# fverdoja/Fast-3D-Pointcloud-Segmentation

Hardware: AMD Instinct MI355X
Metric: Mpoints/sec segmented end-to-end, 1M-pt RGB-D frames (higher is better)
Workload: dtype f32

## Files before the change

### fast-3d-pointcloud-segmentation_amd/csrc/f3ds_hip.hip

```cpp
#include <hip/hip_runtime.h>

#include <algorithm>
#include <cmath>
#include <atomic>
#include <map>
#include <chrono>
#include <cstdio>
#include <cstdlib>
#include <cstring>
#include <string>
#include <type_traits>
#include <mutex>
#include <set>
#include <vector>

#include "../../include/f3ds.h"
#include "f3ds_algo.h"
#include "f3ds_glasbey.h"
#include "f3ds_eval.h"
#include "f3ds_dev.h"
#include "f3ds_levels.h"
#include "f3ds_eval_levels.h"
#include "f3ds_rgbd.h"
#include "f3ds_label_image.h"
#include "f3ds_track.h"
#include "f3ds_regions.h"
#include "f3ds_contacts.h"
#include "f3ds_shapes.h"
#include "f3ds_boxes.h"
#include "f3ds_joints.h"
#include "f3ds_components.h"

using namespace f3ds;

#include "f3ds_kernels.inc"
#include "f3ds_levels.inc"
#include "f3ds_eval_levels.inc"
#include "f3ds_track.inc"
#include "f3ds_regions.inc"
#include "f3ds_contacts.inc"
#include "f3ds_shapes.inc"
#include "f3ds_boxes.inc"
#include "f3ds_joints.inc"
#include "f3ds_components.inc"

namespace {

thread_local std::string g_last_hip_error;
#define HIPCHECK(expr) do { hipError_t e_ = (expr); if (e_ != hipSuccess) { g_last_hip_error = std::string(#expr) + ": " + hipGetErrorString(e_); return F3DS_ERR_HIP; } } while (0)

template <class... Ts> struct ArgPack;
template <> struct ArgPack<> {};
template <class T, class... Ts> struct ArgPack<T, Ts...> { T head; ArgPack<Ts...> tail; };

template <class K, class... Done>
__device__ __forceinline__ void unpack_call(const ArgPack<>&, Done... d) { K{}(d...); }
template <class K, class T, class... Ts, class... Done>
__device__ __forceinline__ void unpack_call(const ArgPack<T, Ts...>& p, Done... d) { unpack_call<K>(p.tail, d..., p.head); }

template <class K, class = void> struct waves_per_simd { static constexpr int v = 1; };
template <class K> struct waves_per_simd<K, std::void_t<decltype(K::WAVES_PER_SIMD)>> { static constexpr int v = K::WAVES_PER_SIMD; };
template <class K, class = void> struct is_latency_kernel { static constexpr bool v = false; };
template <class K> struct is_latency_kernel<K, std::void_t<decltype(K::LATENCY_KERNEL)>> { static constexpr bool v = K::LATENCY_KERNEL; };
template <class K, class Pack>
__global__ __launch_bounds__(K::BLOCK, waves_per_simd<K>::v) void k_batched(const Pack* frames) {
#ifndef F3DS_EXP_NO_LATENCY_PRIO
    if constexpr (is_latency_kernel<K>::v) __builtin_amdgcn_s_setprio(3);
#endif
    const Pack p = frames[f3ds_frame()];
    unpack_call<K>(p);
}

template <class F> struct op_traits;
template <class C, class... Ps> struct op_traits<void (C::*)(Ps...) const> { using pack = ArgPack<std::decay_t<Ps>...>; };
template <class K> using pack_of = typename op_traits<decltype(&K::operator())>::pack;

inline void fill_pack(ArgPack<>&) {}
template <class T, class... Ts, class A, class... As>
inline void fill_pack(ArgPack<T, Ts...>& p, A a, As... as) {
    static_assert(std::is_convertible<A, T>::value && !(std::is_pointer<T>::value && std::is_integral<A>::value),
                  "rec<K>(): an argument does not convert implicitly to the kernel's parameter type (wrong element type, swapped arguments?)");
    p.head = a; fill_pack(p.tail, as...);
}

typedef hipError_t (*LaunchFn)(uint32_t gx, uint32_t nf, uint32_t lds, hipStream_t st, const void* dargs);
template <class K>
hipError_t launch_fn(uint32_t gx, uint32_t nf, uint32_t lds, hipStream_t st, const void* dargs) {
    using Pack = pack_of<K>;
    if (lds > 48u * 1024u) {
        hipError_t e = hipFuncSetAttribute(reinterpret_cast<const void*>(k_batched<K, Pack>), hipFuncAttributeMaxDynamicSharedMemorySize, (int)lds);
        if (e != hipSuccess) return e;
    }
    hipLaunchKernelGGL((k_batched<K, Pack>), dim3(gx ? gx : 1u, nf), dim3(K::BLOCK), lds, st, static_cast<const Pack*>(dargs));
    return hipGetLastError();
}
struct Cmd { LaunchFn fn; uint32_t gx, lds, bytes, off; };

const int g_inc_shift = [] { const char* e = dev_getenv("F3DS_INC_SHIFT"); return e ? atoi(e) : 6; }();

struct Switches {
    bool direct_labels = false, copy_stream = true, copy_duplex = false, split_voxel_accum = false, sweep_tiles = true, merge_spec = true, force_global_merge = false, no_stream_pool = false, sort_pairs = false, host_prof = false, trace_err = false, vox_hash = true, vox_tiles_forced = false, levels_global = false;
    int normals_threads = 0, merge_nw = 0, merge_keys = -1; uint32_t tile_holes = 0, ilist_slack = 32, r_rounds = F3DS_R_ROUNDS, grid_cap = 0, rgc_first_cap = 0, rgj_first_cap = 0; long relabel_lds_cap = -1;
    void read() {
        auto on = [](const char* n) { return dev_getenv(n) != nullptr; };
        auto num = [](const char* n, long dflt) { const char* e = dev_getenv(n); return e ? atol(e) : dflt; };
        direct_labels = num("F3DS_DIRECT_LABELS", 0) != 0; copy_stream = num("F3DS_COPY_STREAM", 1) != 0; copy_duplex = num("F3DS_COPY_STREAM", 1) == 2; split_voxel_accum = on("F3DS_SPLIT_VOXEL_ACCUM"); sweep_tiles = num("F3DS_SWEEP_TILES", 1) != 0; merge_spec = num("F3DS_MERGE_SPEC", 1) != 0;
        force_global_merge = on("F3DS_FORCE_GLOBAL_MERGE"); no_stream_pool = on("F3DS_NO_STREAM_POOL"); sort_pairs = on("F3DS_SORT_PAIRS");
        host_prof = on("F3DS_HOST_PROF"); trace_err = on("F3DS_TRACE_ERR");
        vox_tiles_forced = num("F3DS_VOX_TILES", 1) == 2;
        vox_hash = num("F3DS_VOX_TILES", 1) != 0 && !sort_pairs && !split_voxel_accum;
        normals_threads = (int)num("F3DS_NORMALS_THREADS", 0); tile_holes = (uint32_t)num("F3DS_SWEEP_TILE_HOLES", 0);
        { const long v = num("F3DS_MERGE_NW", 0); merge_nw = v == 4 ? 4 : (v ? 8 : 0); }
        { const char* e = dev_getenv("F3DS_MERGE_KEYS"); merge_keys = !e ? -1 : (!strcmp(e, "lds") ? 2 : (!strcmp(e, "global") ? 1 : 0)); }
        relabel_lds_cap = num("F3DS_RELABEL_LDS_CAP", -1);
        levels_global = num("F3DS_LEVELS_GLOBAL", 0) != 0;
        { const long v = num("F3DS_R_ROUNDS_RUN", F3DS_R_ROUNDS); r_rounds = v >= 1 && v <= F3DS_R_ROUNDS ? (uint32_t)v : (uint32_t)F3DS_R_ROUNDS; }
        { const long v = num("F3DS_ILIST_SLACK", 32); ilist_slack = v >= 1 && v <= 32 ? (uint32_t)v : 32u; }
        { const long v = num("F3DS_GRID_CAP", 0); grid_cap = v >= 1 && v <= 2048 ? (uint32_t)v : 0u; }
        { const long v = num("F3DS_RGC_FIRST_CAP", 0); rgc_first_cap = v >= 1 && v <= 0x7fffffffl ? (uint32_t)v : 0u; }
        { const long v = num("F3DS_RGJ_FIRST_CAP", 0); rgj_first_cap = v >= 1 && v <= 0x7fffffffl ? (uint32_t)v : 0u; }
    }
};
thread_local Switches g_sw;
const int g_merge_shared_res = [] { const char* e = dev_getenv("F3DS_MERGE_SHARED_RES"); return e && atoi(e) == 2 ? 2 : 0; }();

#define F3DS_SCRATCH(X) \
    X(P16, pts)  X(unsigned char, img_depth) X(unsigned char, img_color) X(P16, spts) X(uint64_t, keys0) X(uint64_t, keys1) X(uint32_t, vals0) X(uint32_t, vals1) X(uint32_t, flags) X(uint32_t, incl) X(uint32_t, tiles) X(uint32_t, hist) X(uint32_t, seg_start) X(int, pt_voxel) X(uint32_t, labels) \
    X(uint32_t, vkey) X(uint32_t, vcount) X(float, vf) X(int, nbr) X(int, nbrT) X(uint64_t, hkeys) X(uint32_t, hvals) X(float, boxes) X(uint32_t, ckey) X(uint32_t, cell_start) X(uint64_t, chk) X(uint32_t, chv) X(uint32_t, chvals) X(int, seed_orig) X(uint32_t, keep) X(int, seed_kept) \
    X(uint32_t, owner0) X(uint32_t, ownR) X(float, dist0) X(unsigned char, R) X(float, hc) X(uint32_t, hcount) X(uint32_t, hlo) X(uint32_t, hhi) X(int, ghost_vox) X(unsigned char, ghost_active) X(unsigned char, ghost_done) X(uint32_t, ghost_head) X(uint32_t, ghost_next) \
    X(uint32_t, loff) X(float, rows) X(int, row_voxel) X(float, racc0) X(uint32_t, rcnt0) X(float, rrec0) X(unsigned char, ralive0) X(uint64_t, ehk) X(uint64_t, ekeys0) X(uint64_t, ekeys1) X(uint32_t, evals0) X(uint32_t, evals1) X(uint32_t, ea0) X(uint32_t, eb0) \
    X(uint32_t, ea) X(uint32_t, eb) X(float, ew) X(uint32_t, eku) X(int, ehist) X(unsigned char, ealive) X(uint32_t, ev_epoch) X(uint32_t, ev_key) X(int, ev_prev) X(float, racc) X(uint32_t, rcnt) X(float, rrec) X(unsigned char, ralive) X(uint32_t, rhead) X(uint32_t, rtail) X(uint32_t, lnext) X(uint32_t, parent) X(uint32_t, markA) X(uint32_t, markB) X(uint32_t, tl) X(uint32_t, merges) \
     X(float, r_vf) X(uint32_t, r_owner) X(float, r_dist) X(float, r_hc) X(uint32_t, r_hcount) X(uint32_t, r_hlo) X(uint32_t, r_hhi) X(int, r_gvox) X(unsigned char, r_gact) X(unsigned char, r_gdone) X(uint32_t, r_ghead) X(uint32_t, r_gnext) X(uint32_t, r_tl) X(uint32_t, r_tcnt) X(int, r_seed) X(uint32_t, r_L) \
    X(uint32_t, tstamp) X(uint32_t, tround) X(uint32_t, hdirty) X(uint32_t, htiles) X(uint32_t, htcnt) X(uint32_t, vwl) X(uint32_t, vwl2) X(uint32_t, vtmask) \
     X(uint32_t, glut) X(uint32_t, truth_pts) X(uint32_t, tsum) X(uint32_t, tcol) X(uint32_t, tlab) X(uint32_t, ctab) X(uint32_t, csize) X(uint32_t, eroot) X(uint32_t, eincl) \
     X(uint32_t, hcnt) X(uint32_t, pslot) X(uint32_t, vlist) \
     X(uint32_t, u_src) X(uint32_t, u_voff) X(float, u_xyz) X(uint32_t, u_rgba) X(float, u_cent) X(float, u_nrm) \
    X(float, deltas) X(uint64_t, skeys0) X(uint64_t, skeys1) X(uint32_t, svals0) X(uint32_t, svals1) X(uint32_t, cdf_hist) X(float, cdf) X(uint32_t, root) X(uint32_t, rincl) X(uint32_t, rrank) X(uint2, pool) X(uint32_t, rstart) X(uint32_t, rnleaf) X(uint32_t, rcap) X(uint32_t, tile_n1) X(uint32_t, tile_ord) X(uint32_t, tile_slots) X(uint32_t, ilist) X(uint32_t, istart) X(uint32_t, ilen) X(uint32_t, icap) \
     X(uint32_t, lv_into) X(uint32_t, lv_at) X(uint32_t, lv_pfx) X(float, lv_thr) X(uint32_t, lv_tab) X(uint32_t, lv_nreg) X(uint32_t, lv_out) \
     \
    X(uint64_t, evl_k0) X(uint64_t, evl_k1) X(uint32_t, evl_v0) X(uint32_t, evl_v1) X(uint32_t, evl_flag) X(uint64_t, evl_bkey) X(uint32_t, evl_bcnt) X(uint64_t, evl_ukey) X(uint32_t, evl_ucnt) X(uint32_t, evl_glist) \
    X(uint32_t, evl_ssize) X(unsigned char, evl_used) X(float, evl_hterm) X(float, evl_mterm) X(float, evl_tterm) X(uint32_t, evl_tsize) X(uint32_t, evl_order) X(uint32_t, evl_slot) X(uint32_t, evl_counts) X(uint32_t, evl_out) \
     \
    X(unsigned char, li_depth) X(unsigned char, li_color) X(uint32_t, li_lab) X(unsigned char, li_out) \
     \
     \
    X(uint32_t, trk_end) X(uint32_t, trk_out) X(uint32_t, trk_id) X(uint32_t, trk_tid) \
     \
    X(RgAcc, rgt_acc) \
     \
    X(uint64_t, rgc_k0) X(uint64_t, rgc_k1) X(uint32_t, rgc_v0) X(uint32_t, rgc_v1) X(uint32_t, rgc_rec) X(uint32_t, rgc_flag) X(uint64_t, rgc_ukey) X(uint32_t, rgc_ustart) X(uint32_t, rgc_uend) X(uint32_t, rgc_cnt) \
     \
    X(ShAcc, rgs_acc) \
     \
    X(BxFrame, rgx_frame) X(BxAcc, rgx_acc) X(uint32_t, rgx_head) X(f3ds_region_shape, rgx_shape) \
     \
    X(ShAcc, rgj_sacc) X(uint32_t, rgj_shead) X(f3ds_region_shape, rgj_shape) X(uint64_t, rgj_k0) X(uint64_t, rgj_k1) X(uint32_t, rgj_v0) X(uint32_t, rgj_v1) X(uint32_t, rgj_rec) X(uint32_t, rgj_flag) X(uint64_t, rgj_ukey) X(uint32_t, rgj_ustart) X(uint32_t, rgj_uend) X(uint32_t, rgj_cnt) \
     \
    X(uint32_t, rgk_parent) X(uint32_t, rgk_cnt) X(uint32_t, rgk_flag)
template <class T> struct Scratch { T* p = nullptr; size_t cap = 0; int slot = -1; };
#define F3DS_SCRATCH_SLOT(T, name) S_##name,
#define F3DS_SCRATCH_MEMBER(T, name) Scratch<T> name{nullptr, 0, S_##name};
#define F3DS_SCRATCH_VISIT(T, name) if (const int rc_ = f(name)) return rc_;
enum ScratchSlot { F3DS_SCRATCH(F3DS_SCRATCH_SLOT) N_SCRATCH };

}

struct f3ds_ctx {
    int device = 0;
    hipStream_t own_stream = nullptr;
    hipStream_t stream = nullptr;
    hipEvent_t ev[11] = {};
    DevCounters* d_dc = nullptr;
    DevCounters* h_dc = nullptr;
    GridInfo* d_grid = nullptr;
    GridInfo* h_grid = nullptr;
    SeedGrid* d_sgrid = nullptr;
    std::vector<Cmd> cmds;
    std::vector<unsigned char> blob;
    std::vector<uintptr_t> pend;
    MultiOp ops = {}; uint32_t ops_grid = 0;
    unsigned char* h_args[2] = {nullptr, nullptr}; unsigned char* d_args[2] = {nullptr, nullptr}; size_t args_cap = 0;
    hipEvent_t ev_args[2] = {nullptr, nullptr}; bool args_used[2] = {false, false}; int args_flip = 0;
    hipEvent_t ev_copy[3] = {nullptr, nullptr, nullptr};
    DevCounters* d_dcblk = nullptr; DevCounters* h_dcblk = nullptr; size_t dcblk_cap = 0;
    unsigned char* h_li = nullptr; size_t h_li_cap = 0;
    bool have_frame = false;
    bool live = false;
    int rc = 0;
    f3ds_params prm;
    FrameArgs fa;
    const P16* d_pts = nullptr;
    uint32_t n = 0, V = 0, C = 0, S0 = 0, E = 0, hmask = 0;
    uint64_t *ks = nullptr; uint32_t *vs = nullptr;
    uint64_t *cks = nullptr; uint32_t *cvs = nullptr;
    uint64_t *eks = nullptr;
    f3ds_result res;
    bool merge_in_lds = false;
    int merge_kind = 0;
    uint32_t ev_mult = 64;
    uint32_t pool_mult = 1;
    uint32_t vox_cap = 0;
    bool vox_hashed = false;
    bool vox_dense = false;
    uint32_t vox_dense_wait = 0, vox_dense_penalty = 8;
    uint32_t ilist_mult = 1;
    uint32_t edge_mult = 32;
    bool relabel_lds = true;
    int refined_itr = -1;
    int idxbits = -1;
    uint32_t* user_labels = nullptr;
    MergeDev mdev; MergeLds mlds; float host_lambda = 0.5f;
    F3DS_SCRATCH(F3DS_SCRATCH_MEMBER)
    template <class F> int each_scratch(F&& f) { F3DS_SCRATCH(F3DS_SCRATCH_VISIT) return 0; }
    uint32_t launch_shape[3] = {0, 0, 0};
    std::vector<uint32_t> tsize;
    float cluster_T = 0.0f;
    bool user_mode = false;
    std::vector<uint32_t> user_label, user_row;
};

namespace {

bool referenced_by_pending_calls(const f3ds_ctx* c, const void* mem, size_t cap) {
    const uintptr_t lo = (uintptr_t)mem, hi = lo + cap;
    for (const uintptr_t w : c->pend) if (w >= lo && w < hi) return true;
    for (uint32_t k = 0; k < c->ops.n; ++k) {
        const uintptr_t d = (uintptr_t)c->ops.dst[k], sp = (uintptr_t)c->ops.src[k];
        if ((d >= lo && d < hi) || (sp >= lo && sp < hi)) return true;
    }
    return false;
}
template <class A> inline void note_arg(f3ds_ctx* c, const A& a) {
    if constexpr (std::is_pointer<A>::value) { if (a) c->pend.push_back((uintptr_t)a); }
    else if constexpr (std::is_class<A>::value) {
        static_assert(std::is_trivially_copyable<A>::value, "kernel arguments must be plain data");
        for (size_t off = 0; off + 8 <= sizeof(A); off += 8) { uintptr_t w; memcpy(&w, reinterpret_cast<const unsigned char*>(&a) + off, 8); if (w) c->pend.push_back(w); }
    }
}
std::atomic<size_t> g_scratch_hwm[16][N_SCRATCH];
std::atomic<unsigned long long> g_scratch_allocs{0};
template <class T>
int regrow(Scratch<T>& b, size_t mark) {
    g_scratch_allocs.fetch_add(1, std::memory_order_relaxed);
    if (b.p) { HIPCHECK(hipFree(b.p)); b.p = nullptr; b.cap = 0; }
    const size_t want = mark + mark / 4 + 64;
    HIPCHECK(hipMalloc(&b.p, want));
    b.cap = want;
    return F3DS_OK;
}
template <class T>
int ensure(f3ds_ctx* c, Scratch<T>& b, size_t count, T** out) {
    size_t bytes = count * sizeof(T);
    if (bytes < 256) bytes = 256;
    size_t target = bytes;
    std::atomic<size_t>& hwm = g_scratch_hwm[c->device & 15][b.slot];
    size_t seen = hwm.load(std::memory_order_relaxed);
    while (seen < bytes && !hwm.compare_exchange_weak(seen, bytes, std::memory_order_relaxed)) {}
    if (seen > target && seen <= 4 * bytes) target = seen;
    if (b.cap < bytes) {
        if (b.p && (!c->cmds.empty() || c->ops.n) && referenced_by_pending_calls(c, b.p, b.cap)) {
            fprintf(stderr, "f3ds: internal error: regrowing a buffer that a recorded kernel call refers to\n");
            return F3DS_ERR_LOGIC;
        }
        static const bool trace = dev_getenv("F3DS_TRACE_ALLOC") != nullptr;
        if (trace && b.p) fprintf(stderr, "f3ds: regrow slot %d: cap %zu, request %zu, mark %zu, pending calls %zu\n", b.slot, b.cap, bytes, target, c->cmds.size());
        if (const int rc = regrow(b, target)) return rc;
    }
    *out = b.p;
    return F3DS_OK;
}
int pregrow_scratch(f3ds_ctx* c) {
    return c->each_scratch([c](auto& b) -> int {
        if (!b.p) return F3DS_OK;
        const size_t mark = g_scratch_hwm[c->device & 15][b.slot].load(std::memory_order_relaxed);
        if (b.cap >= mark || mark > 4 * b.cap) return F3DS_OK;
        return regrow(b, mark);
    });
}
#define ENSURE(buf, count, ptr) do { int rc_ = ensure(c, buf, (size_t)(count), &ptr); if (rc_) return rc_; } while (0)

thread_local size_t g_grid_cap = 2048;
thread_local size_t g_wide_cap = 2048;
thread_local int g_batch_frames = 1;
std::atomic<int> g_batch_calls[16];
struct BatchCallCount { int d; explicit BatchCallCount(int dev) : d(dev & 15) { g_batch_calls[d].fetch_add(1, std::memory_order_relaxed); } ~BatchCallCount() { g_batch_calls[d].fetch_sub(1, std::memory_order_relaxed); } };
size_t grid_cap_for_batch(int frames) {
    static const size_t target = dev_getenv("F3DS_GRID_TARGET") ? (size_t)atol(dev_getenv("F3DS_GRID_TARGET")) : 3072;
    if (!target) return 2048;
    size_t cap = target / (size_t)(frames > 0 ? frames : 1);
    return cap < 8 ? 8 : (cap > 2048 ? 2048 : cap);
}
inline void set_launch_shape(f3ds_ctx* const* frames, int nframes) {
    g_grid_cap = g_sw.grid_cap ? (size_t)g_sw.grid_cap : grid_cap_for_batch(nframes);
    g_wide_cap = g_sw.grid_cap ? (size_t)g_sw.grid_cap : 2048;
    g_batch_frames = nframes;
    for (int i = 0; i < nframes; ++i) { frames[i]->launch_shape[0] = (uint32_t)g_grid_cap; frames[i]->launch_shape[1] = (uint32_t)g_wide_cap; frames[i]->launch_shape[2] = (uint32_t)nframes; }
}
inline uint32_t grid_wide(size_t work, int block) {
    size_t g = (work + block - 1) / block;
    return (uint32_t)(g < 1 ? 1 : (g > g_wide_cap ? g_wide_cap : g));
}
inline uint32_t grid_for(size_t work, int block) {
    size_t g = (work + block - 1) / block;
    if (g < 1) g = 1;
    if (g > g_grid_cap) g = g_grid_cap;
    return (uint32_t)g;
}
inline uint32_t pow2_ge(size_t x) { uint32_t p = 1; while (p < x) p <<= 1; return p; }
int bits_for(uint64_t max_value) { int b = 0; while (b < 64 && (max_value >> b)) ++b; return b; }

template <class K, class... As> void rec(f3ds_ctx* c, uint32_t gx, uint32_t lds, As... as);
inline void flush_ops(f3ds_ctx* c) {
    if (!c->ops.n) return;
    const MultiOp m = c->ops; const uint32_t g = c->ops_grid;
    c->ops.n = 0; c->ops_grid = 0;
    rec<d_multi_op>(c, g, 0u, m);
}
template <class K, class... As>
void rec(f3ds_ctx* c, uint32_t gx, uint32_t lds, As... as) {
    if constexpr (!std::is_same<K, d_multi_op>::value) flush_ops(c);
    using Pack = pack_of<K>;
    static_assert(std::is_trivially_copyable<Pack>::value, "kernel arguments must be plain data");
    Pack p;
    memset(&p, 0, sizeof p);
    fill_pack(p, as...);
    (note_arg(c, as), ...);
    Cmd cmd; cmd.fn = &launch_fn<K>; cmd.gx = gx; cmd.lds = lds; cmd.bytes = (uint32_t)sizeof(Pack); cmd.off = (uint32_t)c->blob.size();
    c->blob.resize(c->blob.size() + sizeof(Pack));
    memcpy(c->blob.data() + cmd.off, &p, sizeof(Pack));
    c->cmds.push_back(cmd);
}
inline void rec_op(f3ds_ctx* c, void* dst, const void* src, uint32_t value, size_t bytes) {
    const uint32_t words = (uint32_t)((bytes + 3) / 4);
    if (c->ops.n == (uint32_t)MULTI_OPS) flush_ops(c);
    MultiOp& m = c->ops;
    if (m.n == 0) memset(&m, 0, sizeof m);
    m.dst[m.n] = static_cast<uint32_t*>(dst); m.src[m.n] = static_cast<const uint32_t*>(src); m.val[m.n] = value; m.words[m.n] = words; m.n++;
    const uint32_t g = grid_for(words, 256);
    if (g > c->ops_grid) c->ops_grid = g;
}
inline void rec_fill(f3ds_ctx* c, void* dst, uint32_t value, size_t bytes) { rec_op(c, dst, nullptr, value, bytes); }
inline void rec_copy(f3ds_ctx* c, void* dst, const void* src, size_t bytes) { rec_op(c, dst, src, 0u, bytes); }
inline void reset_recording(f3ds_ctx* c) { c->cmds.clear(); c->blob.clear(); c->pend.clear(); c->ops.n = 0; c->ops_grid = 0; }

struct Batch {
    std::vector<f3ds_ctx*> fr;
    hipStream_t st = nullptr;
    f3ds_ctx* owner = nullptr;
};
inline Batch batch_of(f3ds_ctx* c) {
    Batch b; b.owner = c; b.st = c->stream;
    set_launch_shape(&c, 1); reset_recording(c);
    b.fr.push_back(c);
    return b;
}
int batch_of(f3ds_ctx** ctxs, int nctx, Batch& b) {
    b.owner = ctxs[0]; b.st = ctxs[0]->stream;
    set_launch_shape(ctxs, nctx);
    for (int i = 0; i < nctx; ++i) {
        if (ctxs[i]->stream != b.st) HIPCHECK(hipStreamSynchronize(ctxs[i]->stream));
        reset_recording(ctxs[i]);
        b.fr.push_back(ctxs[i]);
    }
    return F3DS_OK;
}

thread_local double g_t_wait = 0, g_t_launch = 0;
static int trace_err(int code, const char* where, const f3ds_ctx* c) {
    if (code && g_sw.trace_err)
        fprintf(stderr, "f3ds: error %d after %s (V %u, seeds %u, edges %u, chain overflow %d, capacity flag %d)\n", code, where, c->V, c->S0, c->h_dc->n_edges,
                c->h_dc->r_overflow, c->h_dc->ev_overflow);
    return code;
}
static inline double now_ms() { return std::chrono::duration<double, std::milli>(std::chrono::steady_clock::now().time_since_epoch()).count(); }
inline hipError_t timed_sync(hipEvent_t e) { const double t0 = now_ms(); const hipError_t r = hipEventSynchronize(e); g_t_wait += now_ms() - t0; return r; }
inline hipError_t timed_sync(hipStream_t st) { const double t0 = now_ms(); const hipError_t r = hipStreamSynchronize(st); g_t_wait += now_ms() - t0; return r; }
template <class F> int clear_counter(f3ds_ctx* c, hipStream_t st, F DevCounters::*f) { c->h_dc->*f = 0; HIPCHECK(hipMemsetAsync(&(c->d_dc->*f), 0, sizeof(F), st)); return F3DS_OK; }
template <class... Fs> int clear_counters(f3ds_ctx* c, hipStream_t st, Fs DevCounters::*... f) { int rc = F3DS_OK; (void)((rc = clear_counter(c, st, f)) || ...); return rc; }
int flush(Batch& b, hipEvent_t before_launch = nullptr) {
    if (b.fr.empty()) return F3DS_OK;
    for (f3ds_ctx* c : b.fr) flush_ops(c);
    const size_t ncmd = b.fr[0]->cmds.size();
    for (f3ds_ctx* c : b.fr) if (c->cmds.size() != ncmd) return F3DS_ERR_UNSUPPORTED;
    if (ncmd == 0) return F3DS_OK;
    const uint32_t nf = (uint32_t)b.fr.size();
    size_t total = 0;
    std::vector<size_t> off(ncmd);
    for (size_t j = 0; j < ncmd; ++j) { off[j] = total; total += (((size_t)b.fr[0]->cmds[j].bytes * nf) + 63u) & ~(size_t)63u; }
    f3ds_ctx* o = b.owner;
    if (o->args_cap < total) {
        HIPCHECK(hipStreamSynchronize(b.st));
        for (int k = 0; k < 2; ++k) {
            if (o->h_args[k]) HIPCHECK(hipHostFree(o->h_args[k]));
            if (o->d_args[k]) HIPCHECK(hipFree(o->d_args[k]));
            o->h_args[k] = o->d_args[k] = nullptr; o->args_used[k] = false;
        }
        o->args_cap = total * 2;
        for (int k = 0; k < 2; ++k) {
            HIPCHECK(hipHostMalloc(&o->h_args[k], o->args_cap, hipHostMallocDefault));
            HIPCHECK(hipMalloc(&o->d_args[k], o->args_cap));
            if (!o->ev_args[k]) HIPCHECK(hipEventCreateWithFlags(&o->ev_args[k], hipEventDisableTiming));
        }
    }
    const int fl = o->args_flip; o->args_flip ^= 1;
    if (o->args_used[fl]) HIPCHECK(timed_sync(o->ev_args[fl]));
    unsigned char* const h_args = o->h_args[fl]; unsigned char* const d_args = o->d_args[fl];
    const double tl0 = now_ms();
    for (size_t j = 0; j < ncmd; ++j)
        for (uint32_t i = 0; i < nf; ++i) {
            const Cmd& cm = b.fr[i]->cmds[j];
            if (cm.fn != b.fr[0]->cmds[j].fn) return F3DS_ERR_UNSUPPORTED;
            memcpy(h_args + off[j] + (size_t)i * cm.bytes, b.fr[i]->blob.data() + cm.off, cm.bytes);
        }
    HIPCHECK(hipMemcpyAsync(d_args, h_args, total, hipMemcpyHostToDevice, b.st));
    if (before_launch) HIPCHECK(hipEventRecord(before_launch, b.st));
    for (size_t j = 0; j < ncmd; ++j) {
        uint32_t gx = 1, lds = 0;
        for (uint32_t i = 0; i < nf; ++i) { const Cmd& cm = b.fr[i]->cmds[j]; if (cm.gx > gx) gx = cm.gx; if (cm.lds > lds) lds = cm.lds; }
        HIPCHECK(b.fr[0]->cmds[j].fn(gx, nf, lds, b.st, d_args + off[j]));
    }
    HIPCHECK(hipEventRecord(o->ev_args[fl], b.st)); o->args_used[fl] = true;
    for (f3ds_ctx* c : b.fr) reset_recording(c);
    g_t_launch += now_ms() - tl0;
    return F3DS_OK;
}
int flush_sync(Batch& b) {
    int rc = flush(b);
    if (rc) return rc;
    const size_t nf = b.fr.size();
    if (nf == 1) HIPCHECK(hipMemcpyAsync(b.fr[0]->h_dc, b.fr[0]->d_dc, sizeof(DevCounters), hipMemcpyDeviceToHost, b.st));
    else if (nf > 1) {
        f3ds_ctx* o = b.owner;
        if (o->dcblk_cap < nf) {
            HIPCHECK(hipStreamSynchronize(b.st));
            if (o->d_dcblk) HIPCHECK(hipFree(o->d_dcblk));
            if (o->h_dcblk) HIPCHECK(hipHostFree(o->h_dcblk));
            o->dcblk_cap = nf * 2;
            HIPCHECK(hipMalloc(&o->d_dcblk, o->dcblk_cap * sizeof(DevCounters)));
            HIPCHECK(hipHostMalloc(&o->h_dcblk, o->dcblk_cap * sizeof(DevCounters), hipHostMallocDefault));
        }
        for (size_t i = 0; i < nf; ++i) rec<d_dc_gather>(b.fr[i], 1u, 0u, b.fr[i]->d_dc, o->d_dcblk + i);
        if ((rc = flush(b))) return rc;
        HIPCHECK(hipMemcpyAsync(o->h_dcblk, o->d_dcblk, nf * sizeof(DevCounters), hipMemcpyDeviceToHost, b.st));
    }
    HIPCHECK(timed_sync(b.st));
    HIPCHECK(hipGetLastError());
    if (nf > 1) for (size_t i = 0; i < nf; ++i) *b.fr[i]->h_dc = b.owner->h_dcblk[i];
    return F3DS_OK;
}

int scan_u32(f3ds_ctx* c, const uint32_t* in, uint32_t* out, uint32_t n) {
    const uint32_t nt = n ? (n + SCAN_TILE - 1) / SCAN_TILE : 1u;
    uint32_t* tiles;
    ENSURE(c->tiles, nt, tiles);
    rec<d_scan_tiles>(c, nt, 0u, in, out, tiles, n);
    rec<d_scan_single>(c, 1u, 0u, tiles, nt);
    rec<d_scan_add>(c, nt, 0u, out, tiles, n);
    return F3DS_OK;
}
int radix_sort(f3ds_ctx* c, uint64_t* k0, uint32_t* v0, uint64_t* k1, uint32_t* v1, uint32_t n, int total_bits, uint64_t** keys_out, uint32_t** vals_out, int base_shift = 0, const uint32_t* n_dev = nullptr) {
    *keys_out = k0; if (vals_out) *vals_out = v0;
    if (total_bits <= 0) return F3DS_OK;
    const int passes = (total_bits + RS_MAXBITS - 1) / RS_MAXBITS;
    const int per = (total_bits + passes - 1) / passes;
    const uint32_t nb = n ? (n + RS_TILE - 1) / RS_TILE : 1u;
    uint32_t* hist;
    ENSURE(c->hist, (size_t)RS_BINS * nb, hist);
    int shift = 0;
    for (int p = 0; p < passes; ++p) {
        const int bits = (total_bits - shift) < per ? (total_bits - shift) : per;
        rec<d_radix_hist>(c, nb, 0u, k0, n, base_shift + shift, bits, hist, nb, n_dev);
        rec<d_scan_single>(c, 1u, 0u, hist, (uint32_t)((1u << bits) * nb));
        if (v0) rec<d_radix_scatter>(c, nb, 0u, k0, v0, k1, v1, n, base_shift + shift, bits, hist, nb, n_dev);
        else rec<d_radix_scatter_k>(c, nb, 0u, k0, k1, n, base_shift + shift, bits, hist, nb);
        std::swap(k0, k1); std::swap(v0, v1);
        shift += bits;
    }
    *keys_out = k0; if (vals_out) *vals_out = v0;
    return F3DS_OK;
}

int seg_bbox(f3ds_ctx* c) {
    rec<d_init_counters>(c, 1u, 0u, c->d_dc);
    rec<d_bbox>(c, grid_for(c->n, 256 * 8) < 512 ? grid_for(c->n, 256 * 8) : 512u, 0u, c->d_pts, c->n, c->fa, c->d_dc);
    rec<d_grid>(c, 1u, 0u, c->d_dc, c->prm.voxel_res, c->d_grid);
    return F3DS_OK;
}
int seg_sort(f3ds_ctx* c, int sort_bits, int idxbits) {
    const uint32_t n = c->n;
    uint64_t *k0, *k1; uint32_t *v0 = nullptr, *v1 = nullptr, *flags, *incl, *seg_start; int* pt_voxel;
    ENSURE(c->keys0, n, k0); ENSURE(c->keys1, n, k1);
    if (idxbits < 0) { ENSURE(c->vals0, n, v0); ENSURE(c->vals1, n, v1); }
    ENSURE(c->flags, n, flags); ENSURE(c->incl, n, incl); ENSURE(c->seg_start, (size_t)n + 1, seg_start);
    ENSURE(c->pt_voxel, n, pt_voxel);
    c->idxbits = idxbits;
    const int ks = idxbits < 0 ? 0 : idxbits;
    rec<d_keys>(c, grid_for(n, 256), 0u, c->d_pts, n, c->fa, c->d_grid, k0, v0, ks);
    c->vs = nullptr;
    int rc = radix_sort(c, k0, v0, k1, v1, n, sort_bits, &c->ks, &c->vs, ks);
    if (rc) return rc;
    const uint64_t invalid = 1ull << (3 * c->h_dc->depth);
    if (g_sw.split_voxel_accum) {
        rec<d_heads>(c, grid_for(n, 256), 0u, c->ks, n, invalid, flags, ks);
        if ((rc = scan_u32(c, flags, incl, n))) return rc;
        rec<d_segstart>(c, grid_for(n, 256), 0u, c->ks, flags, incl, n, invalid, seg_start, &c->d_dc->n_voxels, &c->d_dc->n_valid, ks);
        return F3DS_OK;
    }
    const uint32_t nt = n ? (n + SCAN_TILE - 1) / SCAN_TILE : 1u;
    uint32_t* tiles; ENSURE(c->tiles, nt, tiles);
    rec<d_seg_count>(c, nt, 0u, c->ks, n, invalid, ks, tiles);
    rec<d_scan_single>(c, 1u, 0u, tiles, nt);
    rec<d_seg_write>(c, nt, 0u, c->ks, n, invalid, ks, tiles, seg_start, &c->d_dc->n_voxels, &c->d_dc->n_valid);
    return F3DS_OK;
}
int seg_vox_tiles(f3ds_ctx* c, int code_bits, int tile_bits) {
    const uint32_t n = c->n;
    const uint32_t ntiles = (n + VT_TILE - 1u) / VT_TILE;
    const uint64_t dcap64 = (uint64_t)ntiles * VT_ENT_MAX;
    if (code_bits + tile_bits + VT_CNT_BITS > 64 || dcap64 > 0x7fffffffull || (uint64_t)ntiles * VT_TAB > 0x7fffffffull) return F3DS_ERR_UNSUPPORTED;
    const uint32_t dcap = (uint32_t)dcap64;
    const uint64_t fin = c->h_dc->n_finite;
    const uint32_t capV = (uint32_t)std::max<uint64_t>(256u, std::min<uint64_t>(fin, dcap));
    c->vox_cap = capV;
    uint64_t *k0, *k1; uint32_t *ploc, *v0, *v1, *part, *vkey, *vcount, *seg_start, *list; uint2* bo_te; float* vf; int* pt_voxel;
    const uint32_t nchunks = (dcap + DS_CHUNK - 1u) / DS_CHUNK;
    ENSURE(c->pslot, n, ploc); ENSURE(c->keys0, dcap, k0); ENSURE(c->keys1, dcap, k1); ENSURE(c->vals0, dcap, v0); ENSURE(c->vals1, dcap, v1);
    { uint32_t* w; ENSURE(c->hcnt, (size_t)ntiles * VT_TAB * 2 + 2u * nchunks, w); bo_te = reinterpret_cast<uint2*>(w); part = w + (size_t)ntiles * VT_TAB * 2; }
    ENSURE(c->vkey, (size_t)capV * 3, vkey); ENSURE(c->vcount, capV, vcount); ENSURE(c->vf, (size_t)capV * 12, vf);
    ENSURE(c->seg_start, (size_t)capV + 1, seg_start); ENSURE(c->vlist, n, list); ENSURE(c->pt_voxel, n, pt_voxel);
    { uint32_t *f, *incl; ENSURE(c->flags, capV, f); ENSURE(c->incl, capV, incl); }
    c->idxbits = -1; c->ks = nullptr; c->vs = nullptr;
    rec<d_tile_keys>(c, std::min<uint32_t>(ntiles, (uint32_t)g_grid_cap * 16u), 0u, c->d_pts, n, c->fa, c->d_grid, ploc, k0, v0, dcap, tile_bits, c->d_dc);
    uint64_t* ks; uint32_t* vs;
    int rc = radix_sort(c, k0, v0, k1, v1, dcap, code_bits + tile_bits, &ks, &vs, VT_CNT_BITS, &c->d_dc->seg_count);
    if (rc) return rc;
    rec<d_desc_part>(c, nchunks, 0u, ks, dcap, tile_bits, part, c->d_dc);
    rec<d_desc_offsets>(c, 1u, 0u, part, dcap, capV, seg_start, c->d_dc);
    rec<d_desc_apply>(c, nchunks, 0u, ks, vs, dcap, capV, tile_bits, c->fa, c->d_grid, part, bo_te, seg_start, vkey, c->d_dc);
    rec<d_tile_place>(c, std::min<uint32_t>(ntiles, (uint32_t)g_grid_cap * 16u), 0u, ploc, n, bo_te, list, pt_voxel, c->d_dc);
    rec<d_voxel_list_accum>(c, std::min<uint32_t>(grid_wide(capV, 256), std::max<uint32_t>(64u, grid_wide(n / 8u, 256))), 0u, c->d_pts, list, seg_start, c->fa, vf, vcount, c->d_dc, capV);
    c->vox_hashed = true;
    return F3DS_OK;
}
int seg_neighbors(f3ds_ctx* c, uint32_t wgs) {
    const uint32_t V = c->V;
    const bool blocks = c->h_dc->depth <= N_BLOCK_DEPTH_MAX;
    const uint32_t cap = blocks ? pow2_ge((size_t)V + 16) : pow2_ge((size_t)V * 2 + 16);
    const size_t words = blocks ? (size_t)cap * 2 : cap;
    uint32_t* hvals = nullptr; int *nbr, *nbrT; uint64_t* hkeys;
    c->hmask = cap - 1;
    ENSURE(c->nbr, (size_t)V * 27, nbr); ENSURE(c->nbrT, (size_t)V * 27, nbrT); ENSURE(c->hkeys, words, hkeys);
    if (!blocks) ENSURE(c->hvals, cap, hvals);
    rec_fill(c, hkeys, 0xFFFFFFFFu, words * 8);
    rec<d_vox_table>(c, wgs, 0u, c->vkey.p, V, c->d_grid, hkeys, hvals, c->hmask);
    rec<d_neighbors>(c, grid_wide((size_t)V * 27, 256), 0u, c->vkey.p, c->d_dc, c->d_grid, c->fa.leaf_order, hkeys, hvals, c->hmask, nbr, nbrT);
    return F3DS_OK;
}
int seg_voxels(f3ds_ctx* c) {
    const uint32_t V = c->V, n = c->n;
    if (c->vox_hashed) return seg_neighbors(c, 1u);
    uint32_t *vkey, *vcount; float *vf;
    ENSURE(c->vkey, (size_t)V * 3, vkey); ENSURE(c->vcount, V, vcount); ENSURE(c->vf, (size_t)V * 12, vf);
    if (g_sw.split_voxel_accum) {
        P16* spts; ENSURE(c->spts, n, spts);
        rec<d_point_gather>(c, grid_wide(n, 256), 0u, c->d_pts, c->vs, c->ks, c->idxbits < 0 ? 0 : c->idxbits, c->incl.p, n, c->d_dc, spts, c->pt_voxel.p);
        rec<d_voxel_accum>(c, grid_wide(V, 256), 0u, spts, c->ks, c->idxbits < 0 ? 0 : c->idxbits, c->seg_start.p, c->d_dc, c->fa, c->d_grid, vkey, vcount, vf);
    } else
        rec<d_voxel_gather_accum>(c, grid_wide(V, 256), 0u, c->d_pts, c->vs, c->ks, c->idxbits < 0 ? 0 : c->idxbits, c->seg_start.p, n, c->d_dc, c->fa, c->d_grid, vkey, vcount, vf, c->pt_voxel.p);
    return seg_neighbors(c, grid_for(V, 4096));
}
int seg_normals(f3ds_ctx* c) {
    const uint32_t nt = (c->V + NT_TILE - 1) / NT_TILE;
    uint32_t *tn1, *tord, *tslots;
    ENSURE(c->tile_n1, nt, tn1); ENSURE(c->tile_ord, (size_t)nt * NT_RING1, tord); ENSURE(c->tile_slots, (size_t)nt * SW_SLOT_WORDS * NT_TILE, tslots);
#ifdef F3DS_NORMALS_LOOP
    static const uint32_t budget = dev_getenv("F3DS_NORMALS_WGS") ? (uint32_t)atoi(dev_getenv("F3DS_NORMALS_WGS")) : 0u;
#else
    static const uint32_t budget = 0u;
#endif
    const uint32_t share = budget ? std::max(2u, budget / (uint32_t)g_batch_frames) : nt;
    const int nthr_env = g_sw.normals_threads;
    const uint32_t holes = g_sw.tile_holes;
    if (nthr_env ? nthr_env == 256 : g_batch_frames >= 16)
        rec<d_normals_t<256>>(c, std::min(nt, share), 0u, c->vf.p, c->nbr.p, c->d_dc, tn1, tord, tslots, holes);
    else
        rec<d_normals_t<384>>(c, std::min(nt, share), 0u, c->vf.p, c->nbr.p, c->d_dc, tn1, tord, tslots, holes);
    return F3DS_OK;
}
int seg_seed_grid(f3ds_ctx* c) {
    const uint32_t V = c->V;
    float* boxes; const float* vf = c->vf.p;
    const uint32_t nchunks = (V + SEED_CHUNK - 1) / SEED_CHUNK;
    ENSURE(c->boxes, (size_t)nchunks * 6, boxes);
    rec<d_chunkbox>(c, nchunks, 0u, vf, c->d_dc, boxes);
    rec<d_seed_grow>(c, 1u, 0u, vf, boxes, c->d_dc, c->prm.seed_res, c->d_sgrid);
    return F3DS_OK;
}
int seg_seed_cells(f3ds_ctx* c, int sort_bits, int max_sdepth) {
    const uint32_t V = c->V;
    uint32_t *ckey, *cell_start, *v0, *v1; uint64_t *k0 = c->keys0.p, *k1 = c->keys1.p;
    ENSURE(c->vals0, V, v0); ENSURE(c->vals1, V, v1);
    ENSURE(c->ckey, (size_t)V * 3, ckey); ENSURE(c->cell_start, (size_t)V + 1, cell_start);
    rec<d_seed_keys>(c, grid_for(V, 256), 0u, c->vf.p, c->d_dc, c->d_sgrid, ckey, k0, v0);
    int rc = radix_sort(c, k0, v0, k1, v1, V, sort_bits, &c->cks, &c->cvs);
    if (rc) return rc;
    const uint64_t climit = max_sdepth >= 21 ? 0xFFFFFFFFFFFFFFFFull : (1ull << (3 * max_sdepth));
    rec<d_heads>(c, grid_for(V, 256), 0u, c->cks, V, climit, c->flags.p, 0);
    if ((rc = scan_u32(c, c->flags.p, c->incl.p, V))) return rc;
    rec<d_segstart>(c, grid_for(V, 256), 0u, c->cks, c->flags.p, c->incl.p, V, climit, cell_start, &c->d_dc->n_cells, &c->d_dc->seg_count, 0);
    return F3DS_OK;
}
int seg_seeds(f3ds_ctx* c) {
    const uint32_t V = c->V, C = c->C;
    uint32_t *sorted_vox, *chvals, *keep; uint64_t* chk; int *seed_orig, *seed_kept;
    const uint32_t ccap = pow2_ge((size_t)C * 2 + 16);
    ENSURE(c->chv, V, sorted_vox); ENSURE(c->chk, ccap, chk); ENSURE(c->chvals, ccap, chvals);
    ENSURE(c->seed_orig, C, seed_orig); ENSURE(c->seed_kept, C, seed_kept); ENSURE(c->keep, C, keep);
    rec_copy(c, sorted_vox, c->cvs, (size_t)V * 4);
    rec_fill(c, chk, 0xFFFFFFFFu, (size_t)ccap * 8);
    const uint32_t* ckey = c->ckey.p; const uint32_t* cell_start = c->cell_start.p; const float* vf = c->vf.p;
    rec<d_cell_hash>(c, grid_for(C, 256), 0u, ckey, sorted_vox, cell_start, c->d_dc, chk, chvals, ccap - 1);
    rec<d_seed_nn>(c, (C + 3u) / 4u, 0u, vf, ckey, sorted_vox, cell_start, c->d_dc, c->d_sgrid, chk, chvals, ccap - 1, seed_orig);
    rec<d_seed_filter>(c, (C + 3u) / 4u, 0u, vf, ckey, sorted_vox, cell_start, c->d_dc, c->d_sgrid, chk, chvals, ccap - 1, seed_orig, a_radius_sq(c->prm.seed_res), a_min_points(c->prm.seed_res, c->prm.voxel_res), keep);
    int rc = scan_u32(c, keep, c->incl.p, C);
    if (rc) return rc;
    rec<d_seed_compact>(c, grid_for(C, 256), 0u, seed_orig, keep, c->incl.p, c->d_dc, seed_kept);
    return F3DS_OK;
}
struct SweepBufs {
    Scratch<uint32_t> *owner; Scratch<float> *dist, *hc; Scratch<uint32_t> *hcount, *hlo, *hhi; Scratch<int>* ghost_vox; Scratch<unsigned char> *ghost_active, *ghost_done; Scratch<uint32_t> *ghost_head, *ghost_next, *htiles, *htcnt;
    const float* vf;
    const int* seeds;
    bool reseed;
};
int seg_sweeps_on(f3ds_ctx* c, const SweepBufs& sb) {
    const uint32_t V = c->V, S0 = c->S0;
    const f3ds_params& prm = c->prm;
    uint32_t *owner0, *ownR, *hcount, *hlo, *hhi, *ghost_head, *ghost_next; float *dist0, *hc; unsigned char *R, *ghost_active, *ghost_done; int* ghost_vox;
    ENSURE(*sb.owner, V, owner0); ENSURE(c->ownR, V, ownR); ENSURE(*sb.dist, V, dist0);
    ENSURE(c->R, V, R); ENSURE(*sb.hc, (size_t)(S0 + 1) * 12, hc); ENSURE(*sb.hcount, S0 + 1, hcount);
    ENSURE(*sb.hlo, S0 + 1, hlo); ENSURE(*sb.hhi, S0 + 1, hhi); ENSURE(*sb.ghost_vox, S0 + 1, ghost_vox);
    ENSURE(*sb.ghost_active, S0 + 1, ghost_active); ENSURE(*sb.ghost_done, S0 + 1, ghost_done);
    ENSURE(*sb.ghost_head, V, ghost_head); ENSURE(*sb.ghost_next, S0 + 1, ghost_next);
    const uint32_t T = (V + 63u) / 64u;
    uint32_t *tiles4, *trr, *hD;
    ENSURE(c->tstamp, (size_t)4 * T, tiles4); ENSURE(c->tround, (size_t)(F3DS_R_ROUNDS - 1) * T, trr); ENSURE(c->hdirty, S0 + 1, hD);
    uint32_t *tl, *tcnt; ENSURE(*sb.htiles, (size_t)(S0 + 1) * HT_CAP, tl); ENSURE(*sb.htcnt, S0 + 1, tcnt);
    uint32_t *wl, *wl2, *tmask; ENSURE(c->vwl, V, wl); ENSURE(c->vwl2, V, wl2); ENSURE(c->vtmask, V, tmask);
    rec_fill(c, tiles4, 0u, (size_t)4 * T * 4);
    rec_fill(c, trr, 0u, (size_t)(F3DS_R_ROUNDS - 1) * T * 4);
    rec_fill(c, hD, 0u, (size_t)(S0 + 1) * 4);
    rec_fill(c, owner0, 0u, (size_t)V * 4);
    rec_fill(c, ghost_head, 0u, (size_t)V * 4);
    rec_fill(c, ghost_next, 0u, (size_t)(S0 + 1) * 4);
    { const float fmax = F3DS_FLT_MAX; uint32_t bits; memcpy(&bits, &fmax, 4); rec_fill(c, dist0, bits, (size_t)V * 4); }
    if (sb.reseed) {
        rec<d_reseed_own>(c, grid_for(S0, 256), 0u, sb.seeds, S0, owner0);
        rec<d_reseed_init>(c, grid_for(S0 + 1, 256), 0u, sb.seeds, S0, owner0, ghost_vox, ghost_active, ghost_done, hlo, hhi, hcount, tl, tcnt);
    } else {
        rec<d_helper_own>(c, grid_for(S0, 256), 0u, sb.seeds, S0, owner0);
        rec<d_helper_init>(c, grid_for(S0 + 1, 256), 0u, sb.seeds, S0, owner0, ghost_vox, ghost_active, ghost_done, hlo, hhi, hcount, hc, tl, tcnt);
    }
    const int* nbrT = c->nbrT.p; const float* vf = sb.vf;
    SweepFrame a;
    a.sv = SweepView{(int)V, nbrT, vf, owner0, dist0, hc, ghost_head, ghost_next, &c->d_dc->n_ghosts, prm.seed_res, prm.w_normal, prm.w_color, prm.w_spatial, c->nbr.p};
    a.R = R; a.ownR = ownR; a.owner_out = owner0; a.dist_out = dist0;
    a.ghost_done = ghost_done; a.ghost_active = ghost_active; a.ghost_vox = ghost_vox; a.ghost_head = ghost_head; a.ghost_next = ghost_next;
    a.hlo = hlo; a.hhi = hhi; a.hcount = hcount; a.hc = hc; a.dc = c->d_dc; a.S0 = S0;
    a.tR0 = tiles4; a.tR1 = tiles4 + T; a.tC0 = tiles4 + 2 * (size_t)T; a.tC1 = tiles4 + 3 * (size_t)T; a.tRr = trr; a.hD = hD; a.T = T; a.tl = tl; a.tcnt = tcnt; a.wl = wl; a.wl2 = wl2; a.tmask = tmask;
    a.thr = a_sweep_thr(V, g_inc_shift);
    if (!g_sw.sweep_tiles) a.tile_n1 = nullptr;
    else a.tile_n1 = c->tile_n1.p;
    a.tile_ord = c->tile_ord.p; a.tile_slots = c->tile_slots.p;
    for (uint32_t t = 0; t < c->res.sweeps; ++t) {
        if (a_sweep_needs_clear(t)) rec_fill(c, R, 0u, V);
        rec<d_sweep_begin>(c, 1u, 0u, a, t);
        const bool can_skip = t >= 2u;
        const bool rounds = g_inc_shift >= 0 && can_skip;
        const uint32_t nrounds = rounds ? g_sw.r_rounds : 0u;
        rec<d_sweep_R_first>(c, grid_for(V, 256), 0u, a, a_sweep_tag(t), t, nrounds);
        for (uint32_t r = 1; r < nrounds; ++r) rec<d_sweep_R_round>(c, grid_for(V, 256), 0u, a, t, r, nrounds);
        for (uint32_t pass = 0; pass < F3DS_R_PASSES; ++pass) rec<d_sweep_R>(c, pass == 0 ? grid_for(V, 256) : 64u, 0u, a, a_sweep_tag(t), t, pass);
        rec<d_sweep_R_tail>(c, 1u, 0u, a, a_sweep_tag(t), t);
        rec<d_sweep_claim>(c, grid_for(V, 256), 0u, a, t);
        rec<d_centroid>(c, grid_for((size_t)S0 * 64u, 256), 0u, a, t);
    }
    return F3DS_OK;
}
int seg_sweeps(f3ds_ctx* c) {
    SweepBufs sb{&c->owner0, &c->dist0, &c->hc, &c->hcount, &c->hlo, &c->hhi, &c->ghost_vox, &c->ghost_active, &c->ghost_done, &c->ghost_head, &c->ghost_next, &c->htiles, &c->htcnt, c->vf.p, c->seed_kept.p, false};
    return seg_sweeps_on(c, sb);
}
int seg_supervoxels(f3ds_ctx* c) {
    const uint32_t V = c->V, S0 = c->S0;
    uint32_t *loff, *rcnt0, *ev0, *ev1; float *rows, *racc0, *rrec0; int* row_voxel; unsigned char* ralive0; uint64_t *ehk, *ek0, *ek1;
    ENSURE(c->loff, S0 + 2, loff);
    int rc = scan_u32(c, c->hcount.p, loff + 1, S0 + 1);
    if (rc) return rc;
    rec_fill(c, loff, 0u, 4);
    ENSURE(c->rows, ((size_t)V + S0 + 1) * 12, rows); ENSURE(c->row_voxel, (size_t)V + S0 + 1, row_voxel);
    ENSURE(c->racc0, (size_t)(S0 + 1) * 12, racc0); ENSURE(c->rcnt0, S0 + 1, rcnt0); ENSURE(c->rrec0, (size_t)(S0 + 1) * 16, rrec0);
    ENSURE(c->ralive0, S0 + 1, ralive0);
    rec_fill(c, ralive0, 0u, S0 + 1);
    rec_fill(c, rcnt0, 0u, (size_t)(S0 + 1) * 4);
    rec<d_sv_fill>(c, S0 ? (S0 + 3u) / 4u : 1u, 0u,
                   c->vf.p, c->owner0.p, S0, c->hlo.p, c->hhi.p, c->ghost_vox.p, c->ghost_active.p, c->hcount.p, loff, c->hc.p, rows, row_voxel, racc0, rcnt0, rrec0, ralive0, c->d_dc, c->htiles.p, c->htcnt.p, V);
    const uint32_t ecap = (uint32_t)std::min<uint64_t>((uint64_t)S0 * c->edge_mult + 1024u, 0x7fffffffu);
    const uint32_t ehcap = pow2_ge((size_t)ecap * 2);
    ENSURE(c->ehk, ehcap, ehk);
    ENSURE(c->ekeys0, ecap, ek0); ENSURE(c->ekeys1, ecap, ek1); ENSURE(c->evals0, ecap, ev0); ENSURE(c->evals1, ecap, ev1);
    rec_fill(c, ehk, 0xFFFFFFFFu, (size_t)ehcap * 8);
    rec<d_edges>(c, grid_for(V, 256), 0u, V, S0, c->nbrT.p, c->owner0.p, ehk, ehcap - 1, ek0, ecap, c->d_dc);
    rec<d_edges_ghost>(c, grid_for(S0, 256), 0u, V, S0, c->ghost_vox.p, c->ghost_active.p, c->nbrT.p, c->owner0.p, ehk, ehcap - 1, ek0, ecap, c->d_dc);
    return F3DS_OK;
}
int seg_edge_sort(f3ds_ctx* c, int sort_bits) {
    const uint32_t E = c->E, S0 = c->S0;
    uint32_t *ea0, *eb0; ENSURE(c->ea0, E, ea0); ENSURE(c->eb0, E, eb0);
    uint32_t* evs;
    { uint32_t* h; ENSURE(c->hist, (size_t)RS_BINS * (((size_t)E * 2 + RS_TILE - 1) / RS_TILE + 1), h); }
    rec<d_iota>(c, grid_for(E, 256), 0u, c->evals0.p, E);
    int rc = radix_sort(c, c->ekeys0.p, c->evals0.p, c->ekeys1.p, c->evals1.p, E, sort_bits, &c->eks, &evs);
    if (rc) return rc;
    rec<d_edge_init>(c, grid_for(E, 256), 0u, c->eks, E, S0, ea0, eb0);
    return F3DS_OK;
}
bool merge_il_layout(uint32_t E, uint32_t S0, int nw, int res, MergeLds* xl) {
    memset(xl, 0, sizeof *xl);
    if ((uint64_t)E * (res == 2 ? 10u : 2u) > (1u << 22)) return false;
    const MergeIlLayout L = merge_il_offsets(E, nw, res);
    xl->Ecap = L.Ecap; xl->NGcap = L.NGcap; xl->lds_bytes = L.total; xl->keys_in_lds = res;
    xl->spec = g_sw.merge_spec ? 1 : 0;
    return L.total <= MC_LDS_LIMIT && S0 <= 65534u;
}
enum MergeKind { MK_GLOBAL = 0, MK_IL = 1 };
inline int mk_waves(int kind) { return (kind - MK_IL) >= 2 ? 4 : 8; }
inline int mk_res(int kind) { return (kind - MK_IL) % 2 ? 0 : 2; }
int choose_merge_kind(const std::vector<f3ds_ctx*>& fr, bool force_global) {
    if (force_global || g_sw.force_global_merge) return MK_GLOBAL;
    const bool e_keys = g_sw.merge_keys >= 0;
    const bool shared = fr.size() >= 16 && g_batch_calls[fr[0]->device & 15].load(std::memory_order_relaxed) >= 2;
    const int nw = g_sw.merge_nw ? (g_sw.merge_nw == 8 ? 8 : 4) : (shared ? 4 : 8);
    const int first = e_keys ? (g_sw.merge_keys == 2 ? 2 : 0) : (shared ? g_merge_shared_res : 2);
    for (int res = first; res >= (e_keys ? first : 0); res -= 2) {
        bool ok = true;
        for (f3ds_ctx* c : fr) { MergeLds t; if (!merge_il_layout(c->E, c->S0, nw, res, &t)) { ok = false; break; } }
        if (ok) return MK_IL + (nw == 8 ? 0 : 2) + (res == 2 ? 0 : 1);
    }
    return MK_GLOBAL;
}
int seg_cluster_front(f3ds_ctx* c, const f3ds_params* prm, int kind) {
    const bool use_lds = kind != MK_GLOBAL;
    const uint32_t S0 = c->S0, E = c->E;
    float lambda = 0.5f; int bins = 500;
    if (prm->merging == F3DS_MANUAL_LAMBDA && prm->lambda != 0) { if (prm->lambda < 0 || prm->lambda > 1) return F3DS_ERR_RANGE; lambda = prm->lambda; }
    if (prm->merging == F3DS_EQUALIZATION && prm->bins != 0) { if (prm->bins < 0) return F3DS_ERR_RANGE; bins = (short)prm->bins; }
    if (prm->merging < 0 || prm->merging > 2 || prm->color_metric < 0 || prm->color_metric > 1 || prm->geom_metric < 0 || prm->geom_metric > 1) return F3DS_ERR_ARG;
    MergeDev m;
    memset(&m, 0, sizeof m);
    m.E = E; m.S0 = S0; m.threshold = prm->threshold; m.dc = c->d_dc;
    { const uint64_t cap = (uint64_t)E * c->ev_mult + 4096u; m.ev_cap = cap > 0x7fffffffull ? 0x7fffffffu : (uint32_t)cap; }
    ENSURE(c->ea, E, m.ea); ENSURE(c->eb, E, m.eb); ENSURE(c->ew, ((size_t)E + 2047) & ~(size_t)2047, m.ew);  ENSURE(c->eku, ((size_t)E + 2047) & ~(size_t)2047, m.eku);
    ENSURE(c->ehist, E, m.ehist); ENSURE(c->ealive, E, m.ealive);
    ENSURE(c->ev_epoch, m.ev_cap, m.ev_epoch); ENSURE(c->ev_key, m.ev_cap, m.ev_key); ENSURE(c->ev_prev, m.ev_cap, m.ev_prev);
    ENSURE(c->racc, (size_t)(S0 + 1) * 12, m.racc); ENSURE(c->rrec, (size_t)(S0 + 1) * 16, m.rrec);
    ENSURE(c->rcnt, S0 + 1, m.rcnt); ENSURE(c->ralive, S0 + 1, m.ralive);
    ENSURE(c->rhead, S0 + 1, m.rhead); ENSURE(c->rtail, S0 + 1, m.rtail); ENSURE(c->lnext, S0 + 1, m.lnext);
    ENSURE(c->parent, S0 + 1, m.parent); ENSURE(c->markA, S0 + 1, m.markA); ENSURE(c->markB, S0 + 1, m.markB);
    ENSURE(c->tl, E, m.tl); ENSURE(c->merges, (size_t)(S0 + 1) * 3, m.merges);
    m.loff = c->loff.p; m.llen = c->hcount.p; m.rows = c->rows.p;
    float* deltas; ENSURE(c->deltas, (size_t)E * 2, deltas);
    rec_copy(c, m.racc, c->racc0.p, (size_t)(S0 + 1) * 12 * 4);
    rec_copy(c, m.rrec, c->rrec0.p, (size_t)(S0 + 1) * 16 * 4);
    rec_copy(c, m.rcnt, c->rcnt0.p, (size_t)(S0 + 1) * 4);
    rec_copy(c, m.ralive, c->ralive0.p, (size_t)(S0 + 1));
    rec_copy(c, m.ea, c->ea0.p, (size_t)E * 4);
    rec_copy(c, m.eb, c->eb0.p, (size_t)E * 4);
    MergeLds xl;
    merge_il_layout(E, S0, use_lds ? mk_waves(kind) : 8, use_lds ? mk_res(kind) : 0, &xl);
    uint32_t logS = 1; while ((1u << logS) < S0 + 2u) ++logS;
    xl.pool_cap = (S0 + 1u) * (4u * logS + 8u) * c->pool_mult;
    ENSURE(c->pool, xl.pool_cap, xl.pool); ENSURE(c->rstart, S0 + 1, xl.rstart); ENSURE(c->rnleaf, S0 + 1, xl.rnleaf);
    ENSURE(c->rcap, S0 + 1, xl.rcap);
    if (use_lds) {
        const uint64_t bound = 2ull * E + (uint64_t)(S0 ? S0 - 1u : 0u) * (MC_TL_CAP + MC_TL_CAP / 2u + 4u) + 1024u;
        uint64_t cap = 2ull * E + (uint64_t)g_sw.ilist_slack * E * c->ilist_mult + (g_sw.ilist_slack < 32u ? 16u : 1024u);
        if (cap > bound) cap = bound;
        xl.ilist_cap = cap > 0x7fffffffull ? 0x7fffffffu : (uint32_t)cap;
        ENSURE(c->ilist, xl.ilist_cap, xl.ilist); ENSURE(c->istart, S0 + 1, xl.istart); ENSURE(c->ilen, S0 + 1, xl.ilen); ENSURE(c->icap, S0 + 1, xl.icap);
    }
    if (use_lds) rec<d_inc_build>(c, 1u, 0u, E, S0, m.ea, m.eb, xl.istart, xl.ilen, xl.icap, xl.ilist);
    xl.stop_key = (prm->threshold != prm->threshold) ? 0u : n_weight_key(prm->threshold);
    c->merge_in_lds = use_lds; c->merge_kind = kind;
    rec<d_region_reset>(c, grid_for(S0 + 1, 256), 0u, S0, c->hcount.p, m.rhead, m.rtail, m.lnext, m.parent, m.markA, m.markB, xl.pool, xl.rstart, xl.rnleaf, xl.rcap, c->loff.p);
    m.mp.color_metric = prm->color_metric; m.mp.geom_metric = prm->geom_metric; m.mp.merging = prm->merging; m.mp.lambda = lambda; m.mp.bins = bins;
    uint64_t *sk0 = nullptr, *sk1 = nullptr; uint32_t *sv0 = nullptr, *sv1 = nullptr;
    if (prm->merging == F3DS_ADAPTIVE_LAMBDA) {
        ENSURE(c->skeys0, (size_t)E * 2, sk0); ENSURE(c->skeys1, (size_t)E * 2, sk1);
        ENSURE(c->svals0, (size_t)E * 2, sv0); ENSURE(c->svals1, (size_t)E * 2, sv1);
    }
    rec<d_edge_deltas>(c, grid_for(E, 256), 0u, E, m.ea, m.eb, m.rrec, prm->color_metric, prm->geom_metric, deltas, sk0, sv0);
    if (prm->merging == F3DS_ADAPTIVE_LAMBDA) {
        uint64_t* ks; uint32_t* vs;
        int rc = radix_sort(c, sk0, sv0, sk1, sv1, E * 2u, 33, &ks, &vs);
        if (rc) return rc;
        rec<d_lambda>(c, 1u, 0u, E, deltas, vs, c->d_dc);
    } else if (prm->merging == F3DS_EQUALIZATION) {
        uint32_t* hist; float* cdf;
        ENSURE(c->cdf_hist, (size_t)2 * (bins > 0 ? bins : 1), hist); ENSURE(c->cdf, (size_t)2 * (bins > 0 ? bins : 1), cdf);
        rec_fill(c, hist, 0u, (size_t)2 * (bins > 0 ? bins : 1) * 4);
        rec<d_cdf_hist>(c, grid_for((size_t)E * 2, 256), 0u, E, deltas, bins, hist, c->d_dc);
        rec<d_cdf_scan>(c, 1u, 0u, E, bins, hist, cdf);
        m.mp.cdf_c = cdf; m.mp.cdf_g = cdf + bins;
    }
    rec<d_edge_weights>(c, grid_for(E, 256), 0u, m, deltas);
    c->mdev = m; c->mlds = xl; c->host_lambda = lambda;
    return F3DS_OK;
}
int seg_merge(f3ds_ctx* c) {
#ifdef F3DS_WHATIF
    if (const char* e = dev_getenv("F3DS_FAKE_MERGE")) {
        unsigned us = 30000, waves = 1; sscanf(e, "%u,%u", &us, &waves);
        const char* l = dev_getenv("F3DS_FAKE_MERGE_LDS");
        rec<d_fake_merge>(c, 1u, l ? (uint32_t)atoi(l) * 1024u : c->mlds.lds_bytes, c->mdev, (uint32_t)us, (uint32_t)waves);
        return F3DS_OK;
    }
#endif
    switch (c->merge_kind) {
        case MK_IL + 0: rec<d_merge_il_t<8, 2>>(c, 1u, c->mlds.lds_bytes, c->mdev, c->mlds); break;
        case MK_IL + 1: rec<d_merge_il_t<8, 0>>(c, 1u, c->mlds.lds_bytes, c->mdev, c->mlds); break;
        case MK_IL + 2: rec<d_merge_il_t<4, 2>>(c, 1u, c->mlds.lds_bytes, c->mdev, c->mlds); break;
        case MK_IL + 3: rec<d_merge_il_t<4, 0>>(c, 1u, c->mlds.lds_bytes, c->mdev, c->mlds); break;
        default: rec<d_merge>(c, 1u, 0u, c->mdev);
    }
    return F3DS_OK;
}
int seg_labels(f3ds_ctx* c) {
    const uint32_t S0 = c->S0, n = c->n;
    const MergeDev& m = c->mdev;
    uint32_t *root, *rincl, *d_labels;
    ENSURE(c->root, S0 + 1, root); ENSURE(c->rincl, S0 + 1, rincl);
    if (c->user_labels) d_labels = c->user_labels;
    else ENSURE(c->labels, n, d_labels);
// ... 79 lines not shown
int li_begin(f3ds_ctx** ctxs, int nctx, Batch* b) {
    g_sw.read();
    HIPCHECK(hipSetDevice(ctxs[0]->device));
    return batch_of(ctxs, nctx, *b);
}
struct LiImages { const unsigned char* depth; const unsigned char* color; const uint32_t* labels; };
int li_upload(f3ds_ctx* const* ctxs, int nctx, Batch& b, const RgbdLayout& lay, const void* const* depth, const void* const* color, const uint32_t* const* labels, int inputs_on_device,
              LiImages* im) {
    for (int i = 0; i < nctx; ++i) im[i] = LiImages{static_cast<const unsigned char*>(depth[i]), color ? static_cast<const unsigned char*>(color[i]) : nullptr, labels[i]};
    if (inputs_on_device) return F3DS_OK;
    hipStream_t up = g_sw.copy_stream ? copy_stream_of(b.owner->device) : nullptr;
    for (int i = 0; i < nctx; ++i) {
        f3ds_ctx* c = ctxs[i];
        unsigned char *ud, *uc = nullptr; uint32_t* ul;
        ENSURE(c->li_depth, lay.depth_bytes, ud); ENSURE(c->li_lab, lay.n, ul);
        if (color) ENSURE(c->li_color, lay.color_bytes, uc);
        HIPCHECK(hipMemcpyAsync(ud, depth[i], lay.depth_bytes, hipMemcpyHostToDevice, up ? up : b.st));
        if (color) HIPCHECK(hipMemcpyAsync(uc, color[i], lay.color_bytes, hipMemcpyHostToDevice, up ? up : b.st));
        HIPCHECK(hipMemcpyAsync(ul, labels[i], lay.n * 4, hipMemcpyHostToDevice, up ? up : b.st));
        im[i] = LiImages{ud, uc, ul};
    }
    if (up) { if (const int urc = await_uploads(b, up)) return urc; }
    return F3DS_OK;
}
int li_upload(f3ds_ctx* c, Batch& b, const RgbdLayout& lay, const void* depth, const void* color, const uint32_t* labels, int inputs_on_device, LiImages* im) {
    return li_upload(&c, 1, b, lay, &depth, color ? &color : nullptr, &labels, inputs_on_device, im);
}
struct LiStage {
    f3ds_ctx* o = nullptr; unsigned char* out = nullptr; std::vector<LiSlot> slot; size_t first_bytes = 0, total = 0;
    uint32_t* head(int i) const { return reinterpret_cast<uint32_t*>(out + (size_t)i * LI_HEAD_BYTES); }
    const uint32_t* h_head(int i) const { return reinterpret_cast<const uint32_t*>(o->h_li + (size_t)i * LI_HEAD_BYTES); }
};
int li_out_buffers(f3ds_ctx* c, int nctx, const size_t* fixed, const size_t* stage_rows, size_t row_bytes, size_t first_rows, LiStage* s) {
    s->o = c; s->slot.resize((size_t)nctx);
    s->total = li_stage_layout((size_t)nctx, fixed, stage_rows, row_bytes, first_rows, s->slot.data(), &s->first_bytes);
    ENSURE(c->li_out, s->total, s->out);
    if (c->h_li_cap < s->total) {
        if (c->h_li) { HIPCHECK(hipHostFree(c->h_li)); c->h_li = nullptr; c->h_li_cap = 0; }
        HIPCHECK(hipHostMalloc(&c->h_li, s->total + s->total / 4, hipHostMallocDefault));
        c->h_li_cap = s->total + s->total / 4;
    }
    return F3DS_OK;
}
int li_download_heads(const LiStage& s, Batch& b) {
    HIPCHECK(hipMemcpyAsync(s.o->h_li, s.out, s.first_bytes, hipMemcpyDeviceToHost, b.st));
    HIPCHECK(timed_sync(b.st));
    HIPCHECK(hipGetLastError());
    return F3DS_OK;
}
int li_rows_behind(const LiStage& s, Batch& b, int nctx, size_t row_bytes, const size_t* count, void* const* rows) {
    bool more = false;
    for (int i = 0; i < nctx; ++i) {
        const LiSlot& sl = s.slot[(size_t)i];
        if (count[i] <= sl.first) continue;
        const size_t off = sl.rows_at + sl.first * row_bytes;
        HIPCHECK(hipMemcpyAsync(s.o->h_li + off, s.out + off, (count[i] - sl.first) * row_bytes, hipMemcpyDeviceToHost, b.st));
        more = true;
    }
    if (more) HIPCHECK(timed_sync(b.st));
    for (int i = 0; i < nctx; ++i) if (count[i]) memcpy(rows[i], s.o->h_li + s.slot[(size_t)i].rows_at, count[i] * row_bytes);
    return F3DS_OK;
}
enum FrameNeed { NEED_NOTHING = 0, NEED_FRAME = 1, NEED_VOXEL_GRID = 2 , NEED_REFINED = 4 };
int on_frame(f3ds_ctx* c, int need = NEED_FRAME) {
    if (!c) return F3DS_ERR_ARG;
    if (((need & NEED_FRAME) && !c->have_frame) || ((need & NEED_VOXEL_GRID) && c->user_mode) || ((need & NEED_REFINED) && c->refined_itr < 0)) return F3DS_ERR_LOGIC;
    HIPCHECK(hipSetDevice(c->device));
    HIPCHECK(hipStreamSynchronize(c->stream));
    return F3DS_OK;
}
struct Capped {
    size_t cap; bool any; size_t k = 0;
    bool room() const { return k < cap; }
    void next() { ++k; }
    int finish(size_t* n_out) const { if (n_out) *n_out = k; return (k > cap && any) ? F3DS_ERR_CAPACITY : F3DS_OK; }
};
inline bool all_fit(size_t n, size_t cap, bool any, size_t* n_out, int* rc) {
    if (n_out) *n_out = n;
    *rc = (any && cap < n) ? F3DS_ERR_CAPACITY : F3DS_OK;
    return any && cap >= n;
}
inline void put3(float* dst, size_t k, const float* src) { if (dst) { dst[3 * k] = src[0]; dst[3 * k + 1] = src[1]; dst[3 * k + 2] = src[2]; } }

static uint32_t* pinned_device_alias(uint32_t* host) {
    hipPointerAttribute_t at;
    memset(&at, 0, sizeof at);
    if (hipPointerGetAttributes(&at, host) != hipSuccess) { (void)hipGetLastError(); return nullptr; }
    if (at.type != hipMemoryTypeHost || !at.devicePointer) return nullptr;
    return static_cast<uint32_t*>(at.devicePointer);
}

int run_cluster(Batch& b, const f3ds_params* prm, uint32_t* const* labels_of, const std::vector<int>& index_of, int labels_on_device, bool force_global = false) {
    const int kind = choose_merge_kind(b.fr, force_global);
    const bool all_lds = kind != MK_GLOBAL;
    int rc = for_frames(b, [&](f3ds_ctx* c) { return seg_cluster_front(c, prm, kind); });
    if (rc || (rc = flush(b))) return rc;
    stage_mark(b, 5);
    if ((rc = for_frames(b, seg_merge)) || (rc = flush(b))) return rc;
    stage_mark(b, 6);
    for (size_t i = 0; i < b.fr.size(); ++i) {
        uint32_t* out = labels_of ? labels_of[index_of[i]] : nullptr;
        if (out && !labels_on_device && g_sw.direct_labels) out = pinned_device_alias(out);
        else if (!labels_on_device) out = nullptr;
        b.fr[i]->user_labels = out;
    }
    {
        const uint32_t cap = g_sw.relabel_lds_cap >= 0 ? (uint32_t)g_sw.relabel_lds_cap : RL_LDS_CAP;
        bool fits = true;
        for (f3ds_ctx* c : b.fr) if (c->S0 + 1u > cap) fits = false;
        for (f3ds_ctx* c : b.fr) c->relabel_lds = fits;
    }
    if ((rc = for_frames(b, seg_labels)) || (rc = flush(b))) return rc;
    stage_mark(b, 7);
    {
        bool want = false;
        for (size_t i = 0; i < b.fr.size(); ++i) if (labels_of && labels_of[index_of[i]] && !b.fr[i]->user_labels && b.fr[i]->n) want = true;
        hipStream_t dl = nullptr;
        if (want && !labels_on_device && (rc = download_begin(b, &dl))) return rc;
        for (size_t i = 0; i < b.fr.size(); ++i) {
            f3ds_ctx* c = b.fr[i];
            uint32_t* out = labels_of ? labels_of[index_of[i]] : nullptr;
            if (out && !c->user_labels && c->n) HIPCHECK(hipMemcpyAsync(out, c->labels.p, (size_t)c->n * 4, hipMemcpyDeviceToHost, dl ? dl : b.st));
            c->user_labels = nullptr;
        }
        if ((rc = download_queued(b, dl)) || (rc = flush_sync(b)) || (rc = download_wait(b, dl))) return rc;
    }
    {
        bool again = false;
        for (f3ds_ctx* c : b.fr) {
            if (c->h_dc->ev_overflow == 1 && c->ev_mult < 16384u) { c->ev_mult *= 4u; again = true; }
            if (c->h_dc->ev_overflow == 2 && c->pool_mult < 64u) { c->pool_mult *= 4u; again = true; }
            if (c->h_dc->ev_overflow == 4 && c->ilist_mult < 4096u) { c->ilist_mult *= 4u; again = true; }
        }
        if (again) {
            if (g_sw.trace_err) fprintf(stderr, "f3ds: merge stage of %zu frames runs again with more history / leaf-pool room\n", b.fr.size());
            for (f3ds_ctx* c : b.fr) if ((rc = clear_counters(c, b.st, &DevCounters::error, &DevCounters::ev_overflow))) return rc;
            return run_cluster(b, prm, labels_of, index_of, labels_on_device, force_global);
        }
    }
    if (all_lds) {
        bool again = false;
        for (f3ds_ctx* c : b.fr) if (c->h_dc->error == F3DS_ERR_UNSUPPORTED) again = true;
        if (again) {
            if (g_sw.trace_err) fprintf(stderr, "f3ds: merge stage of %zu frames runs again with the global-memory kernel\n", b.fr.size());
            for (f3ds_ctx* c : b.fr) if ((rc = clear_counters(c, b.st, &DevCounters::error))) return rc;
            return run_cluster(b, prm, labels_of, index_of, labels_on_device, true);
        }
    }
    for (f3ds_ctx* c : b.fr) {
        if (c->h_dc->error) return trace_err(c->h_dc->error, "merge", c);
        c->res.n_merges = c->h_dc->n_merges; c->res.n_regions = c->h_dc->n_regions;
        c->res.lambda = prm->merging == F3DS_ADAPTIVE_LAMBDA ? (c->E ? c->h_dc->lambda : __builtin_nanf("")) : c->host_lambda;
        c->prm.color_metric = prm->color_metric; c->prm.geom_metric = prm->geom_metric; c->prm.merging = prm->merging;
        c->prm.lambda = prm->lambda; c->prm.bins = prm->bins; c->prm.threshold = prm->threshold;
        c->cluster_T = prm->threshold;
        c->have_frame = true;
    }
    return F3DS_OK;
}

}

extern "C" {

const char* f3ds_last_hip_error(void) { return g_last_hip_error.c_str(); }

int f3ds_device_count(void) {
    int n = 0;
    if (hipGetDeviceCount(&n) != hipSuccess) return 0;
    return n;
}

int f3ds_create(int device, f3ds_ctx** out) {
    if (!out) return F3DS_ERR_ARG;
    *out = nullptr;
    int n = 0;
    if (hipGetDeviceCount(&n) != hipSuccess || n <= 0) return F3DS_ERR_NO_DEVICE;
    if (device < 0 || device >= n) return F3DS_ERR_ARG;
    HIPCHECK(hipSetDevice(device));
    f3ds_ctx* c = new f3ds_ctx;
    c->device = device;
    if (const char* e = dev_getenv("F3DS_EDGE_MULT")) { const int v = atoi(e); if (v >= 1 && v <= 32) c->edge_mult = (uint32_t)v; }
    const int rc = [c]() -> int {
        HIPCHECK(hipStreamCreateWithFlags(&c->own_stream, hipStreamNonBlocking));
        c->stream = c->own_stream;
        for (auto& e : c->ev) HIPCHECK(hipEventCreate(&e));
        HIPCHECK(hipMalloc(&c->d_dc, sizeof(DevCounters)));
        HIPCHECK(hipHostMalloc(&c->h_dc, sizeof(DevCounters), hipHostMallocDefault));
        HIPCHECK(hipMalloc(&c->d_grid, sizeof(GridInfo)));
        HIPCHECK(hipHostMalloc(&c->h_grid, sizeof(GridInfo), hipHostMallocDefault));
        HIPCHECK(hipMalloc(&c->d_sgrid, sizeof(SeedGrid)));
        return F3DS_OK;
    }();
    if (rc) { c->stream = c->own_stream; f3ds_destroy(c); return rc; }
    memset(c->h_grid, 0, sizeof(GridInfo));
    memset(&c->res, 0, sizeof c->res);
    *out = c;
    return F3DS_OK;
}

void f3ds_destroy(f3ds_ctx* c) {
    if (!c) return;
    (void)hipSetDevice(c->device);
    if (c->stream) (void)hipStreamSynchronize(c->stream);
    c->each_scratch([](auto& b) { if (b.p) (void)hipFree(b.p); return 0; });
    if (c->d_dc) (void)hipFree(c->d_dc);
    if (c->h_dc) (void)hipHostFree(c->h_dc);
    if (c->d_grid) (void)hipFree(c->d_grid);
    if (c->h_grid) (void)hipHostFree(c->h_grid);
    if (c->d_sgrid) (void)hipFree(c->d_sgrid);
    for (int k = 0; k < 2; ++k) { if (c->h_args[k]) (void)hipHostFree(c->h_args[k]); if (c->d_args[k]) (void)hipFree(c->d_args[k]); if (c->ev_args[k]) (void)hipEventDestroy(c->ev_args[k]); }
    for (auto& e : c->ev_copy) if (e) (void)hipEventDestroy(e);
    if (c->d_dcblk) (void)hipFree(c->d_dcblk);
    if (c->h_dcblk) (void)hipHostFree(c->h_dcblk);
    if (c->h_li) (void)hipHostFree(c->h_li);
    for (auto& e : c->ev) if (e) (void)hipEventDestroy(e);
    if (c->own_stream) (void)hipStreamDestroy(c->own_stream);
    delete c;
}

int f3ds_set_stream(f3ds_ctx* c, void* hip_stream) {
    if (!c) return F3DS_ERR_ARG;
    c->stream = hip_stream ? (hipStream_t)hip_stream : c->own_stream;
    return F3DS_OK;
}

int f3ds_segment(f3ds_ctx* c, const void* points, size_t n_, int points_on_device, const f3ds_params* prm, uint32_t* point_labels,
                 int labels_on_device, f3ds_result* result) {
    const void* pp[1] = {points}; const size_t cnt[1] = {n_}; uint32_t* lp[1] = {point_labels};
    return f3ds_segment_batch(&c, 1, pp, cnt, points_on_device, prm, lp, labels_on_device, result);
}

}
namespace {
template <class Source>
int segment_batch_from(f3ds_ctx** ctxs, int nctx, Source&& source, int sources_on_device, const f3ds_params* prm, uint32_t* const* point_labels, int labels_on_device,
                              f3ds_result* results) {
    const int points_on_device = sources_on_device;
    const auto t0 = std::chrono::steady_clock::now();
    g_t_wait = 0; g_t_launch = 0;
    g_sw.read();
    HIPCHECK(hipSetDevice(ctxs[0]->device));
    BatchCallCount in_flight(ctxs[0]->device);
    Batch b;
    b.owner = ctxs[0]; b.st = ctxs[0]->stream;
    BatchStreamLease lease;
    if (nctx > 1 && ctxs[0]->stream == ctxs[0]->own_stream && !g_sw.no_stream_pool) { hipStream_t ps = lease.acquire(ctxs[0]->device); if (ps) b.st = ps; }
    set_launch_shape(ctxs, nctx);
    std::vector<int> index_of;
    const int max_depth = (int)(1.8f * prm->seed_res / prm->voxel_res);
    const uint32_t sweeps = max_depth > 1 ? (uint32_t)(max_depth - 1) : 0u;
    stage_mark(b, 0);
    hipStream_t up_stream = (!points_on_device && g_sw.copy_stream) ? copy_stream_of(ctxs[0]->device) : nullptr;
    bool uploaded = false;
    for (int i = 0; i < nctx; ++i) {
        f3ds_ctx* c = ctxs[i];
        reset_recording(c);
        c->have_frame = false; c->live = true; c->rc = 0; c->refined_itr = -1;
        c->user_mode = false; c->user_label.clear(); c->user_row.clear();
        { const int prc = pregrow_scratch(c); if (prc) return prc; }
        c->prm = *prm; c->V = c->C = c->S0 = c->E = 0;
        c->fa = FrameArgs{prm->use_transform, prm->fold_negative_z, prm->leaf_order, prm->voxel_res, prm->seed_res, prm->w_color, prm->w_spatial, prm->w_normal};
        { const int src_rc = source(c, i, up_stream ? up_stream : b.st, uploaded); if (src_rc) return src_rc; }
        memset(&c->res, 0, sizeof c->res);
        c->res.n_points = c->n; c->res.sweeps = sweeps;
        b.fr.push_back(c); index_of.push_back(i);
    }
    if (up_stream && uploaded) { const int urc = await_uploads(b, up_stream); if (urc) return urc; }
    auto drop_dead = [&](auto&& dead) -> int {
        std::vector<f3ds_ctx*> keep; std::vector<int> keep_idx;
        for (size_t i = 0; i < b.fr.size(); ++i) {
            f3ds_ctx* c = b.fr[i];
            if (dead(c)) { int rc = finish_empty(c, b.st, point_labels ? point_labels[index_of[i]] : nullptr, labels_on_device); if (rc) return rc; }
            else { keep.push_back(c); keep_idx.push_back(index_of[i]); }
        }
        b.fr.swap(keep); index_of.swap(keep_idx);
        return F3DS_OK;
    };
    int rc;
    if ((rc = for_frames(b, seg_bbox)) || (rc = flush_sync(b))) return rc;
    for (f3ds_ctx* c : b.fr) {
        c->res.n_finite = c->h_dc->n_finite;
        if (c->h_dc->error) return c->h_dc->error;
        c->res.octree_depth = (uint32_t)c->h_dc->depth;
    }
    if ((rc = drop_dead([](f3ds_ctx* c) { return c->h_dc->grid_empty || c->n == 0; }))) return rc;
    int maxd = 0;
    for (f3ds_ctx* c : b.fr) if (c->h_dc->depth > maxd) maxd = c->h_dc->depth;
    bool hashed = g_sw.vox_hash && (nctx >= 4 || g_sw.vox_tiles_forced);
    for (f3ds_ctx* c : b.fr) {
        c->vox_hashed = false;
        if (c->vox_dense && hashed) { if (c->vox_dense_wait) c->vox_dense_wait--; else c->vox_dense = false; }
    }
    for (f3ds_ctx* c : b.fr) if (c->vox_dense) hashed = false;
    if (hashed) {
        uint32_t maxtiles = 1;
        for (f3ds_ctx* c : b.fr) maxtiles = std::max(maxtiles, (c->n + VT_TILE - 1u) / VT_TILE);
        const int tile_bits = bits_for((uint64_t)maxtiles - 1u);
        rc = for_frames(b, [&](f3ds_ctx* c) { return seg_vox_tiles(c, 3 * maxd, tile_bits); });
        if (rc == F3DS_ERR_UNSUPPORTED) {
            for (f3ds_ctx* c : b.fr) { reset_recording(c); c->vox_hashed = false; }
            hashed = false;
        } else if (rc || (rc = flush_sync(b))) return rc;
        if (hashed && g_sw.trace_err) for (f3ds_ctx* c : b.fr) fprintf(stderr, "f3ds: tile path: most voxels in a tile %u, descriptors %u, leaves %u, lists sorted %u\n", c->h_dc->vox_max_tile, c->h_dc->seg_count, c->h_dc->n_voxels, c->h_dc->vox_disorder);
        if (hashed) for (f3ds_ctx* c : b.fr) if (c->h_dc->ev_overflow == 6 || c->h_dc->ev_overflow == 7) {
            if (g_sw.trace_err) fprintf(stderr, "f3ds: tile path refused a frame: %s (descriptors %u, leaves %u)\n", c->h_dc->ev_overflow == 6 ? "a voxel with too many points" : "a tile with too many voxels", c->h_dc->seg_count, c->h_dc->n_voxels);
            c->vox_dense = true; c->vox_dense_wait = c->vox_dense_penalty; c->vox_dense_penalty = std::min(2u * c->vox_dense_penalty, 1024u); hashed = false;
        }
        if (!hashed) {
            if (g_sw.trace_err) fprintf(stderr, "f3ds: voxelisation of %zu frames runs again on the sort path (an unorganised cloud or dense voxels)\n", b.fr.size());
            for (f3ds_ctx* c : b.fr) {
                c->vox_hashed = false;
                if ((rc = clear_counters(c, b.st, &DevCounters::error, &DevCounters::ev_overflow, &DevCounters::n_voxels, &DevCounters::seg_count))) return rc;
            }
        }
    }
    if (!hashed) {
        uint32_t maxn = 1;
        for (f3ds_ctx* c : b.fr) if (c->n > maxn) maxn = c->n;
        int idxbits = bits_for((uint64_t)maxn - 1u);
        if (3 * maxd + 1 + idxbits > 64 || g_sw.sort_pairs) idxbits = -1;
        if ((rc = for_frames(b, [&](f3ds_ctx* c) { return seg_sort(c, 3 * maxd + 1, idxbits); })) || (rc = flush_sync(b))) return rc;
    }
    for (f3ds_ctx* c : b.fr) { if (c->h_dc->error) return trace_err(c->h_dc->error, "voxelisation", c); c->V = c->h_dc->n_voxels; c->res.n_voxels = c->V; }
    if ((rc = drop_dead([](f3ds_ctx* c) { return c->V == 0; }))) return rc;
    stage_mark(b, 1);
    if ((rc = for_frames(b, seg_voxels)) || (rc = flush(b))) return rc;
    if ((rc = for_frames(b, seg_normals)) || (rc = flush(b, b.owner->ev[9]))) return rc;
    stage_mark(b, 10);
    if ((rc = for_frames(b, seg_seed_grid)) || (rc = flush(b))) return rc;
    stage_mark(b, 2);
    if ((rc = flush_sync(b))) return rc;
    int maxsd = 0;
    for (f3ds_ctx* c : b.fr) { if (c->h_dc->error) return c->h_dc->error; if (c->h_dc->sdepth > maxsd) maxsd = c->h_dc->sdepth; }
    if ((rc = for_frames(b, [&](f3ds_ctx* c) { return seg_seed_cells(c, 3 * maxsd, maxsd); })) || (rc = flush_sync(b))) return rc;
    for (f3ds_ctx* c : b.fr) { c->C = c->h_dc->n_cells; c->res.n_seed_cells = c->C; }
    if ((rc = for_frames(b, seg_seeds)) || (rc = flush_sync(b))) return rc;
    for (f3ds_ctx* c : b.fr) { c->S0 = c->h_dc->n_seeds; c->res.n_seeds = c->S0; if (c->S0 >= 0x3FFFFFFFu) return F3DS_ERR_UNSUPPORTED; }
    stage_mark(b, 3);
    if ((rc = for_frames(b, seg_sweeps)) || (rc = flush(b))) return rc;
    stage_mark(b, 4);
    if ((rc = for_frames(b, seg_supervoxels)) || (rc = flush_sync(b))) return rc;
    for (int attempt = 0; attempt < 6; ++attempt) {
        bool again = false;
        for (f3ds_ctx* c : b.fr) if (c->h_dc->ev_overflow == 3 && c->edge_mult < (1u << 14)) { c->edge_mult *= 4u; again = true; }
        if (!again) break;
        if (g_sw.trace_err) fprintf(stderr, "f3ds: adjacency pass of %zu frames runs again with more list room\n", b.fr.size());
        for (f3ds_ctx* c : b.fr) if ((rc = clear_counters(c, b.st, &DevCounters::error, &DevCounters::ev_overflow, &DevCounters::n_edges, &DevCounters::n_alive))) return rc;
        if ((rc = for_frames(b, seg_supervoxels)) || (rc = flush_sync(b))) return rc;
    }
    uint64_t maxkey = 1;
    for (f3ds_ctx* c : b.fr) {
        if (c->h_dc->error) return trace_err(c->h_dc->error, "supervoxels/adjacency", c);
        if (c->h_dc->r_overflow) return trace_err(F3DS_ERR_UNSUPPORTED, "sweeps (R chain)", c);
        c->E = c->h_dc->n_edges; c->res.n_edges = c->E; c->res.n_supervoxels = c->h_dc->n_alive;
        const uint64_t k = (uint64_t)(c->S0 + 1) * (c->S0 + 1);
        if (k > maxkey) maxkey = k;
    }
    if ((rc = for_frames(b, [&](f3ds_ctx* c) { return seg_edge_sort(c, bits_for(maxkey)); }))) return rc;
    if ((rc = run_cluster(b, prm, point_labels, index_of, labels_on_device))) return rc;
    HIPCHECK(hipStreamSynchronize(b.st));
    float stage[8] = {0, 0, 0, 0, 0, 0, 0, 0};
    stage_times(b.owner, 0, 7, stage);
    if (!b.fr.empty()) { float ms = 0; if (hipEventElapsedTime(&ms, b.owner->ev[9], b.owner->ev[10]) == hipSuccess) stage[7] = ms; }
    const float ms = (float)std::chrono::duration<double, std::milli>(std::chrono::steady_clock::now() - t0).count();
    if (g_sw.host_prof) fprintf(stderr, "batch of %d: %.1f ms total, %.1f waiting for the GPU, %.1f packing + launching, %.1f recording / host logic; stages %.0f %.0f %.0f %.0f %.0f %.0f %.0f ms; %llu scratch allocations so far\n", nctx, ms, g_t_wait, g_t_launch, ms - g_t_wait - g_t_launch, stage[0], stage[1], stage[2], stage[3], stage[4], stage[5], stage[6], g_scratch_allocs.load());
    for (int i = 0; i < nctx; ++i) {
        f3ds_ctx* c = ctxs[i];
        for (int k = 0; k < 8; ++k) c->res.ms_stage[k] = stage[k];
        c->res.ms_total = ms;
        if (results) results[i] = c->res;
    }
    return F3DS_OK;
}

}
extern "C" {

int f3ds_segment_batch(f3ds_ctx** ctxs, int nctx, const void* const* points, const size_t* counts, int points_on_device, const f3ds_params* prm,
                       uint32_t* const* point_labels, int labels_on_device, f3ds_result* results) {
    if (!ctxs || nctx <= 0 || !points || !counts || !prm) return F3DS_ERR_ARG;
    if (!(prm->voxel_res > 0) || !(prm->seed_res > 0)) return F3DS_ERR_ARG;
    for (int i = 0; i < nctx; ++i) if (!ctxs[i] || (!points[i] && counts[i]) || counts[i] > 0x7fffffffull || ctxs[i]->device != ctxs[0]->device) return F3DS_ERR_ARG;
    auto source = [&](f3ds_ctx* c, int i, hipStream_t copy, bool& uploaded) -> int {
        c->n = (uint32_t)counts[i];
        if (points_on_device) c->d_pts = static_cast<const P16*>(points[i]);
        else {
            P16* up; ENSURE(c->pts, c->n ? c->n : 1, up);
            if (c->n) { HIPCHECK(hipMemcpyAsync(up, points[i], (size_t)c->n * 16, hipMemcpyHostToDevice, copy)); uploaded = true; }
            c->d_pts = up;
        }
        return F3DS_OK;
    };
    return segment_batch_from(ctxs, nctx, source, points_on_device, prm, point_labels, labels_on_device, results);
}

int f3ds_segment_rgbd_batch(f3ds_ctx** ctxs, int nctx, const f3ds_rgbd_format* fmt, const void* const* depth, const void* const* color, int images_on_device,
                            const f3ds_params* prm, uint32_t* const* point_labels, int labels_on_device, f3ds_result* results) {
    if (!ctxs || nctx <= 0 || !fmt || !depth || !color || !prm) return F3DS_ERR_ARG;
    if (!(prm->voxel_res > 0) || !(prm->seed_res > 0)) return F3DS_ERR_ARG;
    f3ds::RgbdLayout lay;
    if (const int rc = f3ds::rgbd_layout(fmt, &lay)) return rc;
    for (int i = 0; i < nctx; ++i) if (!ctxs[i] || !depth[i] || !color[i] || ctxs[i]->device != ctxs[0]->device) return F3DS_ERR_ARG;
    const RgbdArgs args{fmt->width, (uint32_t)lay.n, lay.depth_pitch, lay.color_pitch, fmt->depth_type == F3DS_DEPTH_F32 ? 1 : 0, fmt->color_format, fmt->depth_scale, fmt->fx, fmt->fy, fmt->cx, fmt->cy};
    auto source = [&](f3ds_ctx* c, int i, hipStream_t copy, bool& uploaded) -> int {
        c->n = (uint32_t)lay.n;
        P16* records; ENSURE(c->pts, c->n, records);
        const unsigned char* d_depth = static_cast<const unsigned char*>(depth[i]);
        const unsigned char* d_color = static_cast<const unsigned char*>(color[i]);
        if (!images_on_device) {
            unsigned char *ud, *uc; ENSURE(c->img_depth, lay.depth_bytes, ud); ENSURE(c->img_color, lay.color_bytes, uc);
            HIPCHECK(hipMemcpyAsync(ud, depth[i], lay.depth_bytes, hipMemcpyHostToDevice, copy));
            HIPCHECK(hipMemcpyAsync(uc, color[i], lay.color_bytes, hipMemcpyHostToDevice, copy));
            uploaded = true; d_depth = ud; d_color = uc;
        }
        rec<d_deproject>(c, grid_for(c->n, 256), 0u, d_depth, d_color, args, records);
        c->d_pts = records;
        return F3DS_OK;
    };
    return segment_batch_from(ctxs, nctx, source, images_on_device, prm, point_labels, labels_on_device, results);
}
int f3ds_segment_rgbd(f3ds_ctx* c, const f3ds_rgbd_format* fmt, const void* depth, const void* color, int images_on_device, const f3ds_params* prm, uint32_t* point_labels,
                      int labels_on_device, f3ds_result* result) {
    const void* dp[1] = {depth}; const void* cp[1] = {color}; uint32_t* lp[1] = {point_labels};
    return f3ds_segment_rgbd_batch(&c, 1, fmt, dp, cp, images_on_device, prm, lp, labels_on_device, result);
}

int f3ds_get_points(f3ds_ctx* c, void* points16, size_t cap, int dst_on_device, size_t* n_out) {
    if (!c || (!points16 && !n_out)) return F3DS_ERR_ARG;
    if (!c->d_pts || c->d_pts != c->pts.p) return F3DS_ERR_LOGIC;
    int rc;
    if (!all_fit(c->n, cap, points16 != nullptr, n_out, &rc)) return rc;
    HIPCHECK(hipSetDevice(c->device));
    if (c->n) HIPCHECK(hipMemcpy(points16, c->pts.p, (size_t)c->n * 16, dst_on_device ? hipMemcpyDeviceToDevice : hipMemcpyDeviceToHost));
    return F3DS_OK;
}

int f3ds_recluster(f3ds_ctx* c, const f3ds_params* prm, uint32_t* point_labels, int labels_on_device, f3ds_result* result) {
    if (!c || !prm) return F3DS_ERR_ARG;
    if (!c->have_frame) return F3DS_ERR_LOGIC;
    const auto t0 = std::chrono::steady_clock::now();
    g_sw.read();
    HIPCHECK(hipSetDevice(c->device));
    Batch b = batch_of(c);
    { const int crc = clear_counters(c, c->stream, &DevCounters::error); if (crc) return crc; }
    stage_mark(b, 4);
    std::vector<int> idx{0}; uint32_t* lp[1] = {point_labels};
    int rc = run_cluster(b, prm, lp, idx, labels_on_device);
    if (rc) return rc;
    HIPCHECK(hipStreamSynchronize(b.st));
    stage_times(c, 4, 7, c->res.ms_stage);
    c->res.ms_total = (float)std::chrono::duration<double, std::milli>(std::chrono::steady_clock::now() - t0).count();
    if (result) *result = c->res;
    return F3DS_OK;
}

int f3ds_cluster_supervoxels(f3ds_ctx* c, const f3ds_supervoxel_set* sv, const uint32_t* pairs, size_t n_pairs, const f3ds_params* prm, uint32_t* region_of_sv,
                             uint32_t* voxel_labels, f3ds_result* result) {
    if (!c || !sv || !prm || (n_pairs && !pairs)) return F3DS_ERR_ARG;
    const uint32_t S = sv->n_supervoxels;
    if (S && (!sv->label || !sv->voxel_offset || !sv->voxel_xyz || !sv->voxel_rgba || !sv->centroid_xyz || !sv->normal)) return F3DS_ERR_ARG;
    if (S >= 0x3FFFFFFFu) return F3DS_ERR_UNSUPPORTED;
    const auto t0 = std::chrono::steady_clock::now();
    g_sw.read();
    HIPCHECK(hipSetDevice(c->device));
    std::vector<uint32_t> row(S + 1u, 0u), lab(S + 1u, 0u), hof(S, 0u);
    {
        std::vector<uint32_t> order(S);
        for (uint32_t i = 0; i < S; ++i) order[i] = i;
        std::sort(order.begin(), order.end(), [&](uint32_t a, uint32_t b) { return sv->label[a] < sv->label[b]; });
        for (uint32_t r = 0; r < S; ++r) {
            if (r && sv->label[order[r]] == sv->label[order[r - 1]]) return F3DS_ERR_ARG;
            row[r + 1] = order[r]; lab[r + 1] = sv->label[order[r]]; hof[order[r]] = r + 1u;
        }
    }
    if (S && sv->voxel_offset[0] != 0u) return F3DS_ERR_ARG;
    for (uint32_t i = 0; i < S; ++i) if (sv->voxel_offset[i + 1] <= sv->voxel_offset[i]) return F3DS_ERR_ARG;
    const uint32_t Vt = S ? sv->voxel_offset[S] : 0u;
    if ((uint64_t)Vt + S + 1u > 0x7fffffffull) return F3DS_ERR_UNSUPPORTED;
    std::vector<uint32_t> ea, eb;
    {
        std::vector<std::pair<uint32_t, uint32_t>> ed;
        std::set<std::pair<uint32_t, uint32_t>> seen;
        for (size_t k = 0; k < n_pairs; ++k) {
            const uint32_t p = pairs[2 * k], q = pairs[2 * k + 1];
            if (p > q) continue;
            uint32_t hh[2];
            for (int w = 0; w < 2; ++w) {
                const uint32_t l = w ? q : p;
                const auto it = std::lower_bound(lab.begin() + 1, lab.end(), l);
                if (it == lab.end() || *it != l) return F3DS_ERR_OUT_OF_RANGE;
                hh[w] = (uint32_t)(it - lab.begin());
            }
            if (hh[0] == hh[1] || !seen.insert({hh[0], hh[1]}).second) return F3DS_ERR_ARG;
            ed.push_back({hh[0], hh[1]});
        }
        std::stable_sort(ed.begin(), ed.end(), [](const std::pair<uint32_t, uint32_t>& a, const std::pair<uint32_t, uint32_t>& b) { return a.first < b.first; });
        if (ed.size() > 0x7fffffffull) return F3DS_ERR_UNSUPPORTED;
        ea.resize(ed.size()); eb.resize(ed.size());
        for (size_t k = 0; k < ed.size(); ++k) { ea[k] = ed[k].first; eb[k] = ed[k].second; }
    }
    const uint32_t E = (uint32_t)ea.size();
    reset_recording(c);
    c->have_frame = false; c->live = true; c->rc = 0; c->refined_itr = -1;
    { const int prc = pregrow_scratch(c); if (prc) return prc; }
    c->prm = *prm; c->n = Vt; c->V = c->C = 0; c->S0 = S; c->E = E; c->d_pts = nullptr;
    memset(&c->res, 0, sizeof c->res);
    c->res.n_voxels = Vt; c->res.n_seeds = S; c->res.n_supervoxels = S; c->res.n_edges = E;
    c->user_mode = true; c->user_label = lab; c->user_row = row;
    if (S == 0) {
        c->user_mode = false; c->user_label.clear(); c->user_row.clear(); c->live = false;
        if (result) *result = c->res;
        return F3DS_OK;
    }
    Batch b = batch_of(c);
    uint32_t *d_src, *d_voff, *d_rgba, *loff, *hcount, *owner, *rcnt0, *ea0, *eb0; float *d_xyz, *d_cent, *d_nrm, *rows, *racc0, *rrec0, *hc; int *row_voxel, *pt_voxel; unsigned char* ralive0;
    ENSURE(c->u_src, S + 1u, d_src); ENSURE(c->u_voff, S + 1u, d_voff); ENSURE(c->u_xyz, (size_t)Vt * 3, d_xyz); ENSURE(c->u_rgba, Vt, d_rgba);
    ENSURE(c->u_cent, (size_t)S * 3, d_cent); ENSURE(c->u_nrm, (size_t)S * 3, d_nrm);
    ENSURE(c->loff, S + 2u, loff); ENSURE(c->hcount, S + 1u, hcount); ENSURE(c->owner0, Vt, owner); ENSURE(c->pt_voxel, Vt, pt_voxel);
    ENSURE(c->rows, ((size_t)Vt + S + 1) * 12, rows); ENSURE(c->row_voxel, (size_t)Vt + S + 1, row_voxel);
    ENSURE(c->racc0, (size_t)(S + 1) * 12, racc0); ENSURE(c->rcnt0, S + 1u, rcnt0); ENSURE(c->rrec0, (size_t)(S + 1) * 16, rrec0);
    ENSURE(c->ralive0, S + 1u, ralive0); ENSURE(c->hc, (size_t)(S + 1) * 12, hc);
    ENSURE(c->ea0, E, ea0); ENSURE(c->eb0, E, eb0);
    std::vector<uint32_t> h_loff(S + 2u, 0u), h_cnt(S + 1u, 0u);
    for (uint32_t h = 1; h <= S; ++h) { h_loff[h] = sv->voxel_offset[row[h]]; h_cnt[h] = sv->voxel_offset[row[h] + 1] - sv->voxel_offset[row[h]]; }
    h_loff[S + 1] = Vt;
    const hipStream_t st = b.st;
    HIPCHECK(hipMemcpyAsync(d_src, row.data(), (size_t)(S + 1) * 4, hipMemcpyHostToDevice, st));
    HIPCHECK(hipMemcpyAsync(d_voff, sv->voxel_offset, (size_t)(S + 1) * 4, hipMemcpyHostToDevice, st));
    HIPCHECK(hipMemcpyAsync(d_xyz, sv->voxel_xyz, (size_t)Vt * 12, hipMemcpyHostToDevice, st));
    HIPCHECK(hipMemcpyAsync(d_rgba, sv->voxel_rgba, (size_t)Vt * 4, hipMemcpyHostToDevice, st));
    HIPCHECK(hipMemcpyAsync(d_cent, sv->centroid_xyz, (size_t)S * 12, hipMemcpyHostToDevice, st));
    HIPCHECK(hipMemcpyAsync(d_nrm, sv->normal, (size_t)S * 12, hipMemcpyHostToDevice, st));
    HIPCHECK(hipMemcpyAsync(loff, h_loff.data(), (size_t)(S + 2) * 4, hipMemcpyHostToDevice, st));
    HIPCHECK(hipMemcpyAsync(hcount, h_cnt.data(), (size_t)(S + 1) * 4, hipMemcpyHostToDevice, st));
    if (E) { HIPCHECK(hipMemcpyAsync(ea0, ea.data(), (size_t)E * 4, hipMemcpyHostToDevice, st)); HIPCHECK(hipMemcpyAsync(eb0, eb.data(), (size_t)E * 4, hipMemcpyHostToDevice, st)); }
    stage_mark(b, 4);
    rec<d_init_counters>(c, 1u, 0u, c->d_dc);
    rec_fill(c, ralive0, 0u, S + 1u);
    rec_fill(c, rcnt0, 0u, (size_t)(S + 1) * 4);
    rec_fill(c, racc0, 0u, 48); rec_fill(c, rrec0, 0u, 64); rec_fill(c, hc, 0u, 48);
    rec<d_iota>(c, grid_for(Vt, 256), 0u, reinterpret_cast<uint32_t*>(pt_voxel), Vt);
    rec<d_sv_user_fill>(c, S, 0u, S, d_src, d_voff, d_xyz, d_rgba, d_cent, d_nrm, rows, row_voxel, owner, racc0, rcnt0, rrec0, ralive0, hc, c->d_dc);
    int rc = flush(b);
    if (rc) return rc;
    uint32_t* lp[1] = {voxel_labels}; std::vector<int> idx{0};
    if ((rc = run_cluster(b, prm, lp, idx, 0))) return rc;
    HIPCHECK(hipStreamSynchronize(b.st));
    stage_times(c, 4, 7, c->res.ms_stage);
    if (region_of_sv) {
        std::vector<uint32_t> root(S + 1u);
        HIPCHECK(hipMemcpy(root.data(), c->root.p, (size_t)(S + 1) * 4, hipMemcpyDeviceToHost));
        for (uint32_t i = 0; i < S; ++i) region_of_sv[i] = lab[root[hof[i]]];
    }
    c->live = false;
    c->res.ms_total = (float)std::chrono::duration<double, std::milli>(std::chrono::steady_clock::now() - t0).count();
    if (result) *result = c->res;
    return F3DS_OK;
}

}

namespace {
template <class T>
int fetch(f3ds_ctx* c, const Scratch<T>& b, size_t count, std::vector<T>& out) {
    out.resize(count);
    if (count) HIPCHECK(hipMemcpy(out.data(), b.p, count * sizeof(T), hipMemcpyDeviceToHost));
    return F3DS_OK;
}
inline uint32_t label_out(const f3ds_ctx* c, uint32_t h) { return c->user_mode && h < c->user_label.size() ? c->user_label[h] : h; }
int region_leaves(f3ds_ctx* c, std::vector<unsigned char>& ralive, std::vector<std::vector<uint2>>& leaves) {
    const uint32_t S0 = c->S0;
    std::vector<uint32_t> rhead, lnext, loff, llen, rstart, rnleaf; std::vector<uint2> pool;
    int rc;
    if ((rc = fetch(c, c->ralive, S0 + 1, ralive)) || (rc = fetch(c, c->rhead, S0 + 1, rhead)) || (rc = fetch(c, c->lnext, S0 + 1, lnext)) ||
        (rc = fetch(c, c->loff, S0 + 2, loff)) || (rc = fetch(c, c->hcount, S0 + 1, llen)))
        return rc;
    if (c->merge_in_lds && ((rc = fetch(c, c->pool, c->pool.cap / 8, pool)) || (rc = fetch(c, c->rstart, S0 + 1, rstart)) || (rc = fetch(c, c->rnleaf, S0 + 1, rnleaf)))) return rc;
    leaves.assign(S0 + 1, {});
    for (uint32_t h = 1; h <= S0; ++h) {
        if (!ralive[h]) continue;
        if (c->merge_in_lds) leaves[h].assign(pool.begin() + rstart[h], pool.begin() + rstart[h] + rnleaf[h]);
        else for (uint32_t leaf = rhead[h]; leaf; leaf = lnext[leaf]) leaves[h].push_back(make_uint2(loff[leaf], llen[leaf]));
    }
    return F3DS_OK;
}
inline size_t rows_in_use(const f3ds_ctx* c, const std::vector<uint32_t>& loff) { return c->user_mode ? c->n : loff[c->S0 + 1]; }
}

extern "C" int f3ds_get_regions(f3ds_ctx* c, uint32_t* label, uint32_t* n_voxels, float* centroid_xyz, float* normal, float* mean_rgb, size_t cap, size_t* n_out) {
    if (const int frc = on_frame(c)) return frc;
    const uint32_t S0 = c->S0;
    std::vector<unsigned char> ralive; std::vector<uint32_t> rcnt; std::vector<float> rrec;
    int rc;
    if ((rc = fetch(c, c->ralive, S0 + 1, ralive)) || (rc = fetch(c, c->rcnt, S0 + 1, rcnt)) || (rc = fetch(c, c->rrec, (size_t)(S0 + 1) * 16, rrec))) return rc;
    Capped out{cap, label || n_voxels || centroid_xyz || normal || mean_rgb};
    for (uint32_t h = 1; h <= S0; ++h) {
        if (!ralive[h]) continue;
        if (out.room()) {
            const float* r = &rrec[(size_t)h * 16];
            if (label) label[out.k] = label_out(c, h);
            if (n_voxels) n_voxels[out.k] = rcnt[h];
            put3(centroid_xyz, out.k, r); put3(normal, out.k, r + 3); put3(mean_rgb, out.k, r + 6);
        }
        out.next();
    }
    return out.finish(n_out);
// ... 1270 lines not shown
```

### fast-3d-pointcloud-segmentation_amd/csrc/f3ds_kernels.inc

```


namespace {

struct P16 { float x, y, z; uint32_t rgba; };

struct DevCounters {
    unsigned long long n_finite;
    uint32_t bbox[6];
    uint32_t bbox_any;
    uint32_t n_valid;
    uint32_t n_voxels;
    uint32_t n_cells;
    uint32_t n_seeds;
    uint32_t n_edges;
    uint32_t n_alive;
    uint32_t n_merges;
    uint32_t n_regions;
    uint32_t n_events;
    int error;
    int r_overflow;
    float lambda;
    uint32_t seg_count;
    uint32_t n_ghosts;
    int depth;
    int grid_empty;
    int sdepth;
    uint32_t n_changed;
    uint32_t sweep_full;
    uint32_t sweep_marks;
    int ev_overflow;
    uint32_t sweep_pre;
    uint32_t pad_to_line_[1];
    uint32_t rq[F3DS_R_PASSES + 1];
    uint32_t vox_disorder;
    uint32_t vox_max_tile;
#ifdef F3DS_CEN_STATS
    uint32_t cen_stats[8];
#endif
    uint32_t sweep_stats[4];
    uint32_t sweep_idle;
};

static_assert(offsetof(DevCounters, rq) == 128, "rq[] on a 128-byte line of its own");
__device__ inline SweepCtl sweep_ctl(DevCounters* dc) { return SweepCtl{&dc->n_changed, &dc->sweep_full, &dc->sweep_pre, &dc->sweep_marks, &dc->sweep_idle}; }
constexpr uint64_t HASH_EMPTY = 0xFFFFFFFFFFFFFFFFull;

__host__ __device__ inline uint64_t hash64(uint64_t x) {
    x ^= x >> 33; x *= 0xff51afd7ed558ccdULL; x ^= x >> 33; x *= 0xc4ceb9fe1a85ec53ULL; x ^= x >> 33;
    return x;
}
__device__ inline uint32_t enc_f32(float f) {
    uint32_t b = __float_as_uint(f);
    return (b & 0x80000000u) ? ~b : (b | 0x80000000u);
}
__host__ __device__ inline float dec_f32(uint32_t e) {
    uint32_t b = (e & 0x80000000u) ? (e & 0x7fffffffu) : ~e;
    float f; memcpy(&f, &b, 4); return f;
}

__device__ __forceinline__ void f3ds_vblock(uint32_t* frame, uint32_t* vbx) {
    const uint32_t gx = gridDim.x, nf = gridDim.y;
    const uint32_t full = nf & ~7u;
    if (blockIdx.y < full) {
        const uint32_t lin = blockIdx.y * gx + blockIdx.x;
        const uint32_t g = lin / (8u * gx), r = lin - g * 8u * gx;
        *frame = g * 8u + (r & 7u); *vbx = r >> 3;
    } else { *frame = blockIdx.y; *vbx = blockIdx.x; }
}
__device__ __forceinline__ uint32_t f3ds_vbx() { uint32_t f, x; f3ds_vblock(&f, &x); return x; }
__device__ __forceinline__ uint32_t f3ds_frame() { uint32_t f, x; f3ds_vblock(&f, &x); return f; }
#define BIX (f3ds_vbx())

__device__ inline int lane_id() { return (int)(threadIdx.x & 63u); }
__device__ inline uint64_t lanemask_lt() { return (1ull << lane_id()) - 1ull; }
__device__ inline void wave_lds_sync() {
    __builtin_amdgcn_fence(__ATOMIC_RELEASE, "wavefront");
    __builtin_amdgcn_wave_barrier();
    __builtin_amdgcn_fence(__ATOMIC_ACQUIRE, "wavefront");
}

constexpr int SCAN_THREADS = 256;
constexpr int SCAN_ITEMS = 8;
constexpr int SCAN_TILE = SCAN_THREADS * SCAN_ITEMS;

__device__ inline uint32_t wave_incl_scan(uint32_t v) {
#pragma unroll
    for (int d = 1; d < 64; d <<= 1) {
        uint32_t t = __shfl_up(v, d, 64);
        if (lane_id() >= d) v += t;
    }
    return v;
}
template <int BLOCK>
__device__ inline uint32_t block_incl_scan(uint32_t v, uint32_t* total) {
    __shared__ uint32_t wsum[BLOCK / 64];
    __shared__ uint32_t wtot;
    uint32_t inc = wave_incl_scan(v);
    const int w = threadIdx.x >> 6;
    __syncthreads();
    if (lane_id() == 63) wsum[w] = inc;
    __syncthreads();
    if (threadIdx.x == 0) {
        uint32_t run = 0;
        for (int i = 0; i < BLOCK / 64; ++i) { uint32_t t = wsum[i]; wsum[i] = run; run += t; }
        wtot = run;
    }
    __syncthreads();
    *total = wtot;
    return inc + wsum[w];
}

struct d_scan_single {
    static constexpr bool LATENCY_KERNEL = true;
    static constexpr int BLOCK = 256;
    __device__ void operator()(uint32_t* data, uint32_t m) const {
        uint32_t carry = 0;
        for (uint32_t base = 0; base < m; base += 4096u) {
            const uint32_t i0 = base + threadIdx.x * 16u;
            uint32_t v[16];
            if (i0 + 15u < m) {
#pragma unroll
                for (int q = 0; q < 4; ++q) { const uint4 x = *reinterpret_cast<const uint4*>(data + i0 + 4 * q); v[4 * q] = x.x; v[4 * q + 1] = x.y; v[4 * q + 2] = x.z; v[4 * q + 3] = x.w; }
            } else {
#pragma unroll
                for (int k = 0; k < 16; ++k) v[k] = i0 + k < m ? data[i0 + k] : 0u;
            }
            uint32_t sum = 0;
#pragma unroll
            for (int k = 0; k < 16; ++k) sum += v[k];
            uint32_t tot;
            const uint32_t inc = block_incl_scan<256>(sum, &tot);
            uint32_t run = carry + inc - sum;
            if (i0 + 15u < m) {
#pragma unroll
                for (int q = 0; q < 4; ++q) {
                    uint4 x; x.x = run; x.y = run + v[4 * q]; x.z = x.y + v[4 * q + 1]; x.w = x.z + v[4 * q + 2]; run = x.w + v[4 * q + 3];
                    *reinterpret_cast<uint4*>(data + i0 + 4 * q) = x;
                }
            } else {
#pragma unroll
                for (int k = 0; k < 16; ++k) if (i0 + k < m) { data[i0 + k] = run; run += v[k]; }
            }
            carry += tot;
        }
    }
};
struct d_scan_tiles {
    static constexpr int BLOCK = SCAN_THREADS;
    __device__ void operator()(const uint32_t* in, uint32_t* out, uint32_t* tile_sums, uint32_t n) const {
        if (BIX > 0 && BIX * SCAN_TILE >= n) return;
        const uint32_t base = BIX * SCAN_TILE + threadIdx.x * SCAN_ITEMS;
        uint32_t v[SCAN_ITEMS];
        uint32_t s = 0;
    #pragma unroll
        for (int i = 0; i < SCAN_ITEMS; ++i) { v[i] = (base + i < n) ? in[base + i] : 0u; s += v[i]; }
        uint32_t tot;
        uint32_t inc = block_incl_scan<SCAN_THREADS>(s, &tot);
        uint32_t run = inc - s;
    #pragma unroll
        for (int i = 0; i < SCAN_ITEMS; ++i) { run += v[i]; if (base + i < n) out[base + i] = run; }
        if (threadIdx.x == 0) tile_sums[BIX] = tot;
    }
};
struct d_scan_add {
    static constexpr int BLOCK = SCAN_THREADS;
    __device__ void operator()(uint32_t* out, const uint32_t* tile_offsets, uint32_t n) const {
        if (BIX > 0 && BIX * SCAN_TILE >= n) return;
        const uint32_t base = BIX * SCAN_TILE + threadIdx.x * SCAN_ITEMS;
        const uint32_t off = tile_offsets[BIX];
    #pragma unroll
        for (int i = 0; i < SCAN_ITEMS; ++i) if (base + i < n) out[base + i] += off;
    }
};

constexpr int RS_THREADS = 256;
constexpr int RS_WAVES = RS_THREADS / 64;
constexpr int RS_STRIPS = 16;
constexpr int RS_TILE = RS_THREADS * RS_STRIPS;
constexpr int RS_MAXBITS = 9;
constexpr int RS_BINS = 1 << RS_MAXBITS;

struct d_radix_hist {
    static constexpr int BLOCK = RS_THREADS;
    __device__ void operator()(const uint64_t* keys, uint32_t n, int shift, int bits, uint32_t* hist,
                                                         uint32_t nblocks, const uint32_t* n_dev) const {
        if (BIX >= nblocks) return;
        if (n_dev) { const uint32_t nd = *n_dev; n = nd < n ? nd : n; }
        __shared__ uint32_t lh[RS_BINS];
        for (int i = threadIdx.x; i < RS_BINS; i += RS_THREADS) lh[i] = 0;
        __syncthreads();
        const uint32_t mask = (1u << bits) - 1u;
        const uint32_t wbase = BIX * RS_TILE + (threadIdx.x >> 6) * (64 * RS_STRIPS);
    #pragma unroll
        for (int s = 0; s < RS_STRIPS; ++s) {
            uint32_t i = wbase + s * 64 + lane_id();
            if (i < n) atomicAdd(&lh[(uint32_t)(keys[i] >> shift) & mask], 1u);
        }
        __syncthreads();
        for (uint32_t d = threadIdx.x; d < (1u << bits); d += RS_THREADS) hist[d * nblocks + BIX] = lh[d];
    }
};
struct d_radix_scatter {
    static constexpr int BLOCK = RS_THREADS;
    __device__ void operator()(const uint64_t* keys, const uint32_t* vals, uint64_t* keys_out,
                                                            uint32_t* vals_out, uint32_t n, int shift, int bits,
                                                            const uint32_t* hist_scanned, uint32_t nblocks, const uint32_t* n_dev) const {
        if (BIX >= nblocks) return;
        if (n_dev) { const uint32_t nd = *n_dev; n = nd < n ? nd : n; }
        __shared__ uint32_t wcount[RS_WAVES][RS_BINS];
        const uint32_t mask = (1u << bits) - 1u;
        const int w = threadIdx.x >> 6;
        for (int i = threadIdx.x; i < RS_WAVES * RS_BINS; i += RS_THREADS) (&wcount[0][0])[i] = 0;
        __syncthreads();
        const uint32_t wbase = BIX * RS_TILE + w * (64 * RS_STRIPS);
        uint64_t k[RS_STRIPS];
    #pragma unroll
        for (int s = 0; s < RS_STRIPS; ++s) {
            uint32_t i = wbase + s * 64 + lane_id();
            k[s] = i < n ? keys[i] : 0ull;
            if (i < n) atomicAdd(&wcount[w][(uint32_t)(k[s] >> shift) & mask], 1u);
        }
        __syncthreads();
        for (uint32_t d = threadIdx.x; d < (1u << bits); d += RS_THREADS) {
            uint32_t run = hist_scanned[d * nblocks + BIX];
            for (int ww = 0; ww < RS_WAVES; ++ww) { uint32_t t = wcount[ww][d]; wcount[ww][d] = run; run += t; }
        }
        __syncthreads();
    #pragma unroll
        for (int s = 0; s < RS_STRIPS; ++s) {
            uint32_t i = wbase + s * 64 + lane_id();
            const bool valid = i < n;
            const uint32_t d = (uint32_t)(k[s] >> shift) & mask;
            uint64_t peers = __ballot(valid);
            for (int b = 0; b < bits; ++b) {
                uint64_t m = __ballot(valid && ((d >> b) & 1u));
                peers &= ((d >> b) & 1u) ? m : ~m;
            }
            uint32_t pos = 0;
            if (valid) pos = wcount[w][d] + (uint32_t)__popcll(peers & lanemask_lt());
            __builtin_amdgcn_wave_barrier();
            if (valid && (peers & lanemask_lt()) == 0ull) wcount[w][d] += (uint32_t)__popcll(peers);
            __builtin_amdgcn_wave_barrier();
            if (valid) { keys_out[pos] = k[s]; vals_out[pos] = vals[i]; }
        }
    }
};


struct d_radix_scatter_k {
    static constexpr int BLOCK = RS_THREADS;
    __device__ void operator()(const uint64_t* keys, uint64_t* keys_out, uint32_t n, int shift, int bits, const uint32_t* hist_scanned, uint32_t nblocks) const {
        if (BIX >= nblocks) return;
        __shared__ uint32_t wcount[RS_WAVES][RS_BINS];
        const uint32_t mask = (1u << bits) - 1u;
        const int w = threadIdx.x >> 6;
        for (int i = threadIdx.x; i < RS_WAVES * RS_BINS; i += RS_THREADS) (&wcount[0][0])[i] = 0;
        __syncthreads();
        const uint32_t wbase = BIX * RS_TILE + w * (64 * RS_STRIPS);
        uint64_t k[RS_STRIPS];
    #pragma unroll
        for (int s = 0; s < RS_STRIPS; ++s) {
            uint32_t i = wbase + s * 64 + lane_id();
            k[s] = i < n ? keys[i] : 0ull;
            if (i < n) atomicAdd(&wcount[w][(uint32_t)(k[s] >> shift) & mask], 1u);
        }
        __syncthreads();
        for (uint32_t d = threadIdx.x; d < (1u << bits); d += RS_THREADS) {
            uint32_t run = hist_scanned[d * nblocks + BIX];
            for (int ww = 0; ww < RS_WAVES; ++ww) { uint32_t t = wcount[ww][d]; wcount[ww][d] = run; run += t; }
        }
        __syncthreads();
    #pragma unroll
        for (int s = 0; s < RS_STRIPS; ++s) {
            uint32_t i = wbase + s * 64 + lane_id();
            const bool valid = i < n;
            const uint32_t d = (uint32_t)(k[s] >> shift) & mask;
            uint64_t peers = __ballot(valid);
            for (int b = 0; b < bits; ++b) {
                uint64_t m = __ballot(valid && ((d >> b) & 1u));
                peers &= ((d >> b) & 1u) ? m : ~m;
            }
            uint32_t pos = 0;
            if (valid) pos = wcount[w][d] + (uint32_t)__popcll(peers & lanemask_lt());
            __builtin_amdgcn_wave_barrier();
            if (valid && (peers & lanemask_lt()) == 0ull) wcount[w][d] += (uint32_t)__popcll(peers);
            __builtin_amdgcn_wave_barrier();
            if (valid) keys_out[pos] = k[s];
        }
    }
};

struct FrameArgs {
    int use_transform, fold_negative_z, leaf_order;
    float voxel_res, seed_res, w_color, w_spatial, w_normal;
};

__device__ inline P16 load_point(const P16* pts, size_t i) {
    const uint4 q = reinterpret_cast<const uint4*>(pts)[i];
    P16 p;
    p.x = __uint_as_float(q.x); p.y = __uint_as_float(q.y); p.z = __uint_as_float(q.z); p.rgba = q.w;
    return p;
}

__device__ inline bool vt_blocks(int depth) { return depth <= N_BLOCK_DEPTH_MAX; }
constexpr uint32_t BT_EMPTY = 0xFFFFFFFFu;
struct __attribute__((aligned(16))) BtEntry { uint32_t key, base; unsigned long long vacant; };
static_assert(sizeof(BtEntry) == 16, "one 16-byte load per probe");
template <class T> __device__ inline bool vt_cas(T* p, T* expect, T v, bool agent) {
    return agent ? __hip_atomic_compare_exchange_strong(p, expect, v, __ATOMIC_RELAXED, __ATOMIC_RELAXED, __HIP_MEMORY_SCOPE_AGENT)
                 : __hip_atomic_compare_exchange_strong(p, expect, v, __ATOMIC_RELAXED, __ATOMIC_RELAXED, __HIP_MEMORY_SCOPE_WORKGROUP);
}
__device__ inline void vt_insert(uint64_t* hkeys, uint32_t* hvals, uint32_t hmask, bool agent, unsigned x, unsigned y, unsigned z, uint32_t v) {
    const unsigned long long pk = (unsigned long long)n_pack_key(x, y, z);
    uint32_t h = (uint32_t)hash64((uint64_t)pk) & hmask;
    for (;;) {
        unsigned long long expect = HASH_EMPTY;
        if (vt_cas((unsigned long long*)&hkeys[h], &expect, pk, agent) || expect == pk) { hvals[h] = v; return; }
        h = (h + 1u) & hmask;
    }
}
__device__ inline int vt_find(const uint64_t* hkeys, const uint32_t* hvals, uint32_t hmask, unsigned x, unsigned y, unsigned z) {
    const uint64_t pk = n_pack_key(x, y, z);
    uint32_t h = (uint32_t)hash64(pk) & hmask;
    for (;;) {
        const uint64_t k = hkeys[h];
        if (k == pk) return (int)hvals[h];
        if (k == HASH_EMPTY) return -1;
        h = (h + 1u) & hmask;
    }
}
__device__ inline BtEntry* bt_entry(BtEntry* tab, uint32_t tmask, bool agent, uint32_t bk) {
    uint32_t h = (uint32_t)hash64((uint64_t)bk) & tmask;
    for (;;) {
        uint32_t expect = BT_EMPTY;
        if (vt_cas(&tab[h].key, &expect, bk, agent) || expect == bk) return &tab[h];
        h = (h + 1u) & tmask;
    }
}
__device__ inline int bt_find(const BtEntry* tab, uint32_t tmask, int leaf_order, unsigned x, unsigned y, unsigned z) {
    const uint32_t bk = n_block_key(x, y, z);
    uint32_t h = (uint32_t)hash64((uint64_t)bk) & tmask;
    for (;;) {
        const uint4 e = reinterpret_cast<const uint4*>(tab)[h];
        if (e.x == bk) return n_block_ordinal(e.y, ~(((uint64_t)e.w << 32) | (uint64_t)e.z), n_block_cell(x, y, z), leaf_order);
        if (e.x == BT_EMPTY) return -1;
        h = (h + 1u) & tmask;
    }
}
struct RgbdArgs {
    uint32_t width, n;
    uint32_t depth_pitch, color_pitch;
    int depth_f32, color_format;
    float depth_scale, fx, fy, cx, cy;
};
template <class T> __device__ inline T load_unaligned(const unsigned char* p) { T t; __builtin_memcpy(&t, p, sizeof(T)); return t; }
template <bool DEPTH_F32, int COLOR>
__device__ inline void deproject_loop(const unsigned char* depth, const unsigned char* color, const RgbdArgs& a, P16* out) {
    const uint32_t stride = gridDim.x * blockDim.x;
    const uint32_t sv = stride / a.width, su = stride - sv * a.width;
    uint32_t i = BIX * blockDim.x + threadIdx.x;
    uint32_t v = i / a.width, u = i - v * a.width;
    for (; i < a.n; i += stride) {
        const unsigned char* drow = depth + (size_t)v * a.depth_pitch;
        const unsigned char* crow = color + (size_t)v * a.color_pitch;
        float z = 0.0f;
        bool valid;
        if constexpr (DEPTH_F32) valid = n_depth_to_z(reinterpret_cast<const float*>(drow)[u], a.depth_scale, z);
        else valid = n_depth_to_z(reinterpret_cast<const uint16_t*>(drow)[u], a.depth_scale, z);
        uint32_t rgba;
        if constexpr (COLOR == 0) { const unsigned char* p = crow + 3u * (size_t)u; rgba = n_color_word(p[0], p[1], p[2], 255u); }
        else {
            const uint32_t w = load_unaligned<uint32_t>(crow + 4u * (size_t)u);
            rgba = COLOR == 1 ? n_color_word(w & 255u, (w >> 8) & 255u, (w >> 16) & 255u, w >> 24) : w;
        }
        float x, y, zo;
        n_deproject(u, v, valid, z, a.fx, a.fy, a.cx, a.cy, x, y, zo);
        reinterpret_cast<uint4*>(out)[i] = make_uint4(__float_as_uint(x), __float_as_uint(y), __float_as_uint(zo), rgba);
        u += su; v += sv;
        if (u >= a.width) { u -= a.width; ++v; }
    }
}
struct d_deproject {
    static constexpr int BLOCK = 256;
    __device__ void operator()(const unsigned char* depth, const unsigned char* color, RgbdArgs a, P16* out) const {
        if (a.depth_f32) {
            if (a.color_format == 0) deproject_loop<true, 0>(depth, color, a, out);
            else if (a.color_format == 1) deproject_loop<true, 1>(depth, color, a, out);
            else deproject_loop<true, 2>(depth, color, a, out);
        } else {
            if (a.color_format == 0) deproject_loop<false, 0>(depth, color, a, out);
            else if (a.color_format == 1) deproject_loop<false, 1>(depth, color, a, out);
            else deproject_loop<false, 2>(depth, color, a, out);
        }
    }
};
struct d_bbox {
    static constexpr int BLOCK = 256;
    __device__ void operator()(const P16* pts, uint32_t n, FrameArgs fa, DevCounters* dc) const {
        float mn[3] = {F3DS_FLT_MAX, F3DS_FLT_MAX, F3DS_FLT_MAX}, mx[3] = {-F3DS_FLT_MAX, -F3DS_FLT_MAX, -F3DS_FLT_MAX};
        uint32_t nfin = 0, any = 0;
        for (uint32_t i = BIX * blockDim.x + threadIdx.x; i < n; i += gridDim.x * blockDim.x) {
            P16 p = load_point(pts, i);
            float x = p.x, y = p.y, z = p.z;
            n_prelude(z, fa.fold_negative_z);
            if (n_finite3(x, y, z)) nfin++;
            n_transform(x, y, z, fa.use_transform);
            if (!n_finite3(x, y, z)) continue;
            any = 1;
            if (x < mn[0]) mn[0] = x;
            if (y < mn[1]) mn[1] = y;
            if (z < mn[2]) mn[2] = z;
            if (x > mx[0]) mx[0] = x;
            if (y > mx[1]) mx[1] = y;
            if (z > mx[2]) mx[2] = z;
        }
    #pragma unroll
        for (int d = 32; d >= 1; d >>= 1) {
            for (int a = 0; a < 3; ++a) {
                float t = __shfl_xor(mn[a], d, 64); if (t < mn[a]) mn[a] = t;
                t = __shfl_xor(mx[a], d, 64); if (t > mx[a]) mx[a] = t;
            }
            nfin += __shfl_xor(nfin, d, 64);
            any |= __shfl_xor(any, d, 64);
        }
        __shared__ float smn[4][3], smx[4][3];
        __shared__ uint32_t sfin[4], sany[4];
        const int w = threadIdx.x >> 6;
        if (lane_id() == 0) { for (int a = 0; a < 3; ++a) { smn[w][a] = mn[a]; smx[w][a] = mx[a]; } sfin[w] = nfin; sany[w] = any; }
        __syncthreads();
        if (threadIdx.x == 0) {
            for (int ww = 1; ww < 4; ++ww) {
                for (int a = 0; a < 3; ++a) { if (smn[ww][a] < mn[a]) mn[a] = smn[ww][a]; if (smx[ww][a] > mx[a]) mx[a] = smx[ww][a]; }
                nfin += sfin[ww]; any |= sany[ww];
            }
            if (any) {
                for (int a = 0; a < 3; ++a) { atomicMin(&dc->bbox[a], enc_f32(mn[a])); atomicMax(&dc->bbox[3 + a], enc_f32(mx[a])); }
                atomicOr(&dc->bbox_any, 1u);
            }
            if (nfin) atomicAdd(&dc->n_finite, (unsigned long long)nfin);
        }
    }
};
struct d_grid {
    static constexpr bool LATENCY_KERNEL = true;
    static constexpr int BLOCK = 64;
    __device__ void operator()(DevCounters* dc, float voxel_res, GridInfo* g) const {
        if (threadIdx.x || BIX) return;
        GridInfo t;
        if (!dc->bbox_any) {
            for (int a = 0; a < 3; ++a) { t.min[a] = 0; t.max[a] = 0; }
            t.res = (double)voxel_res; t.depth = 0; t.max_key = 0; t.error = 0; t.empty = 1;
        } else {
            float mn[3], mx[3];
            for (int a = 0; a < 3; ++a) { mn[a] = dec_f32(dc->bbox[a]); mx[a] = dec_f32(dc->bbox[3 + a]); }
            n_grid_from_bbox(mn, mx, voxel_res, t);
            if (t.error) dc->error = t.error;
        }
        *g = t;
        dc->depth = t.depth; dc->grid_empty = t.empty;
    }
};
struct d_keys {
    static constexpr int BLOCK = 256;
    __device__ void operator()(const P16* pts, uint32_t n, FrameArgs fa, const GridInfo* gp, uint64_t* keys, uint32_t* vals, int idxbits) const {
        const GridInfo g = *gp;
        const uint64_t invalid = 1ull << (3 * g.depth);
        for (uint32_t i = BIX * blockDim.x + threadIdx.x; i < n; i += gridDim.x * blockDim.x) {
            P16 p = load_point(pts, i);
            float x = p.x, y = p.y, z = p.z;
            n_prelude(z, fa.fold_negative_z);
            uint64_t key = invalid;
            if (n_finite3(x, y, z) && !g.empty) {
                unsigned k[3];
                n_point_key(g, x, y, z, fa.use_transform, k);
                key = n_morton(k[0], k[1], k[2], g.depth);
                if (fa.leaf_order == 1) key = (~key) & (invalid - 1ull);
            }
            if (vals) { keys[i] = key; vals[i] = i; } else keys[i] = (key << idxbits) | (uint64_t)i;
        }
    }
};
struct d_heads {
    static constexpr int BLOCK = 256;
    __device__ void operator()(const uint64_t* keys, uint32_t n, uint64_t limit, uint32_t* flags, int shift) const {
        for (uint32_t i = BIX * blockDim.x + threadIdx.x; i < n; i += gridDim.x * blockDim.x) {
            uint64_t k = keys[i] >> shift;
            flags[i] = (k < limit && (i == 0 || (keys[i - 1] >> shift) != k)) ? 1u : 0u;
        }
    }
};
struct d_segstart {
    static constexpr int BLOCK = 256;
    __device__ void operator()(const uint64_t* keys, const uint32_t* flags, const uint32_t* incl, uint32_t n, uint64_t limit,
                                                 uint32_t* seg_start, uint32_t* nseg_out, uint32_t* nvalid_out, int shift) const {
        for (uint32_t i = BIX * blockDim.x + threadIdx.x; i < n; i += gridDim.x * blockDim.x) {
            if (flags[i]) seg_start[incl[i] - 1u] = i;
            if ((keys[i] >> shift) < limit && (i + 1 == n || (keys[i + 1] >> shift) >= limit)) { seg_start[incl[i]] = i + 1u; *nseg_out = incl[i]; *nvalid_out = i + 1u; }
        }
    }
};
__device__ inline uint32_t seg_heads_of_thread(const uint64_t* keys, uint32_t n, uint64_t limit, int shift, uint32_t base, uint64_t k[SCAN_ITEMS + 1], uint32_t* head_mask) {
    uint64_t prev = (base > 0u && base - 1u < n) ? keys[base - 1u] >> shift : ~0ull;
    uint32_t cnt = 0, mask = 0;
#pragma unroll
    for (int i = 0; i <= SCAN_ITEMS; ++i) k[i] = base + (uint32_t)i < n ? keys[base + (uint32_t)i] >> shift : ~0ull;
#pragma unroll
    for (int i = 0; i < SCAN_ITEMS; ++i) {
        const bool head = base + (uint32_t)i < n && k[i] < limit && (base + (uint32_t)i == 0u || prev != k[i]);
        if (head) { cnt++; mask |= 1u << i; }
        prev = k[i];
    }
    *head_mask = mask;
    return cnt;
}
struct d_seg_count {
    static constexpr int BLOCK = SCAN_THREADS;
    __device__ void operator()(const uint64_t* keys, uint32_t n, uint64_t limit, int shift, uint32_t* tile_sums) const {
        if (BIX > 0 && BIX * SCAN_TILE >= n) return;
        uint64_t k[SCAN_ITEMS + 1]; uint32_t mask, tot;
        const uint32_t cnt = seg_heads_of_thread(keys, n, limit, shift, BIX * SCAN_TILE + threadIdx.x * SCAN_ITEMS, k, &mask);
        block_incl_scan<SCAN_THREADS>(cnt, &tot);
        if (threadIdx.x == 0) tile_sums[BIX] = tot;
    }
};
struct d_seg_write {
    static constexpr int BLOCK = SCAN_THREADS;
    __device__ void operator()(const uint64_t* keys, uint32_t n, uint64_t limit, int shift, const uint32_t* tile_offsets, uint32_t* seg_start, uint32_t* nseg_out, uint32_t* nvalid_out) const {
        if (BIX > 0 && BIX * SCAN_TILE >= n) return;
        const uint32_t base = BIX * SCAN_TILE + threadIdx.x * SCAN_ITEMS;
        uint64_t k[SCAN_ITEMS + 1]; uint32_t mask, tot;
        const uint32_t cnt = seg_heads_of_thread(keys, n, limit, shift, base, k, &mask);
        uint32_t run = tile_offsets[BIX] + block_incl_scan<SCAN_THREADS>(cnt, &tot) - cnt;
#pragma unroll
        for (int i = 0; i < SCAN_ITEMS; ++i) {
            const uint32_t pos = base + (uint32_t)i;
            if (mask & (1u << i)) seg_start[run++] = pos;
            if (pos < n && k[i] < limit && (pos + 1u == n || k[i + 1] >= limit)) { seg_start[run] = pos + 1u; *nseg_out = run; *nvalid_out = pos + 1u; }
        }
    }
};
struct d_point_gather {
    static constexpr int BLOCK = 256;
    __device__ void operator()(const P16* pts, const uint32_t* vals, const uint64_t* keys, int idxbits, const uint32_t* incl, uint32_t n, const DevCounters* dc, P16* spts,
                               int* pt_voxel) const {
        const uint32_t nv = dc->n_valid;
        for (uint32_t i = BIX * blockDim.x + threadIdx.x; i < n; i += gridDim.x * blockDim.x) {
            const uint32_t idx = vals ? vals[i] : (uint32_t)(keys[i] & ((1ull << idxbits) - 1ull));
            if (i < nv) {
                const P16 p = load_point(pts, idx);
                *reinterpret_cast<float4*>(spts + i) = make_float4(p.x, p.y, p.z, __uint_as_float(p.rgba));
                pt_voxel[idx] = (int)(incl[i] - 1u);
            } else pt_voxel[idx] = -1;
        }
    }
};
struct d_voxel_accum {
    static constexpr int BLOCK = 256;
    __device__ void operator()(const P16* spts, const uint64_t* keys, int keyshift, const uint32_t* seg_start,
                                                    const DevCounters* dc, FrameArgs fa, const GridInfo* gp, uint32_t* vkey, uint32_t* vcount,
                                                    float* vf) const {
        const uint32_t V = dc->n_voxels;
        const int depth = gp->depth;
        for (uint32_t v = BIX * blockDim.x + threadIdx.x; v < V; v += gridDim.x * blockDim.x) {
            const uint32_t s = seg_start[v], e = seg_start[v + 1];
            float sx = 0, sy = 0, sz = 0, sr = 0, sg = 0, sb = 0;
            for (uint32_t i = s; i < e; ++i) {
                P16 p = load_point(spts, i);
                float z = p.z; n_prelude(z, fa.fold_negative_z);
                sx += p.x; sy += p.y; sz += z;
                sr += (float)((p.rgba >> 16) & 255u); sg += (float)((p.rgba >> 8) & 255u); sb += (float)(p.rgba & 255u);
            }
            const uint32_t cnt = e - s;
            const float c = (float)cnt;
            float4* row = reinterpret_cast<float4*>(vf + (size_t)v * 12);
            row[0] = make_float4(sx / c, sy / c, sz / c, sr / c);
            row[1] = make_float4(sg / c, sb / c, 0.0f, 0.0f);
            row[2] = make_float4(0.0f, 0.0f, 0.0f, 0.0f);
            vcount[v] = cnt;
            uint64_t code = keys[s] >> keyshift;
            if (fa.leaf_order == 1) code = (~code) & ((1ull << (3 * depth)) - 1ull);
            unsigned k[3];
            n_demorton(code, depth, k);
            vkey[v * 3] = k[0]; vkey[v * 3 + 1] = k[1]; vkey[v * 3 + 2] = k[2];
        }
    }
};
constexpr uint32_t VG_CHUNK = 1024;
struct d_voxel_gather_accum {
    static constexpr int BLOCK = 256;
    __device__ void operator()(const P16* pts, const uint32_t* vals, const uint64_t* keys, int keyshift, const uint32_t* seg_start, uint32_t n,
                               const DevCounters* dc, FrameArgs fa, const GridInfo* gp, uint32_t* vkey, uint32_t* vcount,
                               float* vf, int* pt_voxel) const {
        __shared__ __attribute__((aligned(16))) uint4 buf[VG_CHUNK];
        __shared__ uint32_t ibuf[VG_CHUNK], vbuf[VG_CHUNK];
        const uint32_t V = dc->n_voxels, nv = dc->n_valid;
        const int depth = gp->depth;
        const uint64_t imask = (1ull << keyshift) - 1ull;
        const uint32_t tid = threadIdx.x;
        for (uint32_t i = nv + BIX * blockDim.x + tid; i < n; i += gridDim.x * blockDim.x) pt_voxel[vals ? vals[i] : (uint32_t)(keys[i] & imask)] = -1;
        for (uint32_t vb = BIX * 256u; vb < V; vb += gridDim.x * 256u) {
            const uint32_t v = vb + tid;
            const bool mine = v < V;
            const uint32_t s = mine ? seg_start[v] : 0u, e = mine ? seg_start[v + 1] : 0u;
            const uint32_t p0 = seg_start[vb], p1 = seg_start[vb + 256u < V ? vb + 256u : V];
            float sx = 0, sy = 0, sz = 0, sr = 0, sg = 0, sb = 0;
            for (uint32_t c0 = p0; c0 < p1; c0 += VG_CHUNK) {
                const uint32_t c1 = p1 - c0 < VG_CHUNK ? p1 : c0 + VG_CHUNK;
                uint32_t idx[VG_CHUNK / 256];
        #pragma unroll
                for (uint32_t j = 0; j < VG_CHUNK / 256; ++j) { const uint32_t i = c0 + j * 256u + tid; const uint32_t ii = i < c1 ? i : c1 - 1u; idx[j] = vals ? vals[ii] : (uint32_t)(keys[ii] & imask); }
                uint4 q[VG_CHUNK / 256];
        #pragma unroll
                for (uint32_t j = 0; j < VG_CHUNK / 256; ++j) q[j] = reinterpret_cast<const uint4*>(pts)[idx[j]];
        #pragma unroll
                for (uint32_t j = 0; j < VG_CHUNK / 256; ++j) { buf[j * 256u + tid] = q[j]; ibuf[j * 256u + tid] = idx[j]; }
                __syncthreads();
                const uint32_t a = s > c0 ? s : c0, b = e < c1 ? e : c1;
                for (uint32_t i = a; i < b; ++i) {
                    const uint4 w = buf[i - c0];
                    float z = __uint_as_float(w.z); n_prelude(z, fa.fold_negative_z);
                    sx += __uint_as_float(w.x); sy += __uint_as_float(w.y); sz += z;
                    sr += (float)((w.w >> 16) & 255u); sg += (float)((w.w >> 8) & 255u); sb += (float)(w.w & 255u);
                    vbuf[i - c0] = v;
                }
                __syncthreads();
        #pragma unroll
                for (uint32_t j = 0; j < VG_CHUNK / 256; ++j) { const uint32_t pp = j * 256u + tid; if (c0 + pp < c1) pt_voxel[ibuf[pp]] = (int)vbuf[pp]; }
                __syncthreads();
            }
            if (!mine) continue;
            const uint32_t cnt = e - s;
            const float c = (float)cnt;
            float4* row = reinterpret_cast<float4*>(vf + (size_t)v * 12);
            row[0] = make_float4(sx / c, sy / c, sz / c, sr / c);
            row[1] = make_float4(sg / c, sb / c, 0.0f, 0.0f);
            row[2] = make_float4(0.0f, 0.0f, 0.0f, 0.0f);
            vcount[v] = cnt;
            uint64_t code = keys[s] >> keyshift;
            if (fa.leaf_order == 1) code = (~code) & ((1ull << (3 * depth)) - 1ull);
            unsigned k[3];
            n_demorton(code, depth, k);
            vkey[v * 3] = k[0]; vkey[v * 3 + 1] = k[1]; vkey[v * 3 + 2] = k[2];
        }
    }
};

#ifndef F3DS_VT_TILE
#define F3DS_VT_TILE 4096
#endif
constexpr uint32_t VT_TILE = F3DS_VT_TILE;
constexpr uint32_t VT_TAB = VT_TILE / 2;
constexpr int VT_CNT_BITS = 14;
static_assert(VT_TILE < (1u << VT_CNT_BITS), "a tile's point count must fit the count field");
constexpr uint32_t VT_ENT_MAX = VT_TAB * 5 / 8;
constexpr uint32_t VL_MAX_RUN = 256;
constexpr uint32_t VOX_NONE = 0xFFFFFFFFu;
__device__ inline void run_of_lane(bool valid, uint32_t w0, uint32_t w1, bool* head, int* head_lane, uint32_t* run_len) {
    const int lane = lane_id();
    const uint32_t p0 = __shfl_up(w0, 1, 64), p1 = __shfl_up(w1, 1, 64);
    const bool pv = __shfl_up((int)valid, 1, 64) != 0;
    const bool h = valid && (lane == 0 || !pv || p0 != w0 || p1 != w1);
    const uint64_t hm = __ballot(h), vm = __ballot(valid);
    const uint64_t le = lane == 63 ? ~0ull : ((2ull << lane) - 1ull);
    const int hl = valid ? 63 - __builtin_clzll(hm & le) : lane;
    const uint64_t above = hl == 63 ? 0ull : ~((2ull << hl) - 1ull);
    const uint64_t stop = (hm | ~vm) & above;
    *head = h; *head_lane = hl; *run_len = (uint32_t)((stop ? __builtin_ctzll(stop) : 64) - hl);
}
struct d_tile_keys {
    static constexpr int BLOCK = 256;
    __device__ void operator()(const P16* pts, uint32_t n, FrameArgs fa, const GridInfo* gp, uint32_t* ploc, uint64_t* dkeys, uint32_t* dvals,
                               uint32_t dcap, int tile_bits, DevCounters* dc) const {
        __shared__ unsigned long long tkey[VT_TAB];
        __shared__ uint32_t tcnt[VT_TAB];
        __shared__ uint32_t tbits[2][VT_TAB / 32];
        __shared__ uint32_t s_ent, s_base, s_over[2], s_dis;
        const GridInfo g = *gp;
        const uint64_t code_mask = (1ull << (3 * g.depth)) - 1ull;
        const int lane = lane_id();
        const uint32_t tid = threadIdx.x;
        const uint32_t ntiles = (n + VT_TILE - 1u) / VT_TILE;
        for (uint32_t tile = BIX; tile < ntiles; tile += gridDim.x) {
            for (uint32_t e = tid; e < VT_TAB; e += 256u) { tkey[e] = HASH_EMPTY; tcnt[e] = 0u; }
            if (tid < VT_TAB / 32u) { tbits[0][tid] = 0u; tbits[1][tid] = 0u; }
            if (tid == 0) { s_ent = 0u; s_over[0] = 0u; s_over[1] = 0u; s_dis = 0u; }
            __syncthreads();
            const uint32_t t0 = tile * VT_TILE, t1 = n - t0 < VT_TILE ? n : t0 + VT_TILE;
            constexpr uint32_t VT_PF = 4;
            uint32_t it4 = 0u;
            for (uint32_t base4 = t0; base4 < t1 && !s_over[(it4 + 1u) & 1u]; base4 += 256u * VT_PF, ++it4) {
              uint4 q[VT_PF];
        #pragma unroll
              for (uint32_t j = 0; j < VT_PF; ++j) { const uint32_t i = base4 + j * 256u + tid; q[j] = reinterpret_cast<const uint4*>(pts)[i < t1 ? i : t1 - 1u]; }
        #pragma unroll
              for (uint32_t j = 0; j < VT_PF; ++j) {
                const uint32_t base = base4 + j * 256u;
                if (base >= t1) break;
                const uint32_t i = base + tid;
                const uint32_t step = (base - t0) >> 8;
                uint64_t pk = HASH_EMPTY;
                if (i < t1) {
                    float x = __uint_as_float(q[j].x), y = __uint_as_float(q[j].y), z = __uint_as_float(q[j].z);
                    n_prelude(z, fa.fold_negative_z);
                    if (n_finite3(x, y, z) && !g.empty) { unsigned k[3]; n_point_key(g, x, y, z, fa.use_transform, k); pk = n_pack_key(k[0], k[1], k[2]); }
                }
                const bool valid = pk != HASH_EMPTY;
                bool head; int hl; uint32_t len;
                run_of_lane(valid, (uint32_t)pk, (uint32_t)(pk >> 32), &head, &hl, &len);
                uint32_t ent = VOX_NONE, roff = 0;
                if (head) {
                    uint32_t e = (uint32_t)hash64(pk) & (VT_TAB - 1u);
                    for (uint32_t probes = 0; probes < VT_TAB; ++probes) {
                        const unsigned long long old = atomicCAS(&tkey[e], (unsigned long long)HASH_EMPTY, (unsigned long long)pk);
                        if (old == HASH_EMPTY) { if (atomicAdd(&s_ent, 1u) >= VT_ENT_MAX) s_over[it4 & 1u] = 1u; ent = e; break; }
                        if (old == pk) { ent = e; break; }
                        e = (e + 1u) & (VT_TAB - 1u);
                    }
                    if (ent != VOX_NONE) {
                        roff = atomicAdd(&tcnt[ent], len);
                        const uint32_t bit = 1u << (ent & 31u);
                        if (atomicOr(&tbits[step & 1u][ent >> 5], bit) & bit) s_dis = 1u;
                    } else s_over[it4 & 1u] = 1u;
                }
                if (tid < VT_TAB / 32u) tbits[(step + 1u) & 1u][tid] = 0u;
                ent = __shfl(ent, hl, 64); roff = __shfl(roff, hl, 64);
                if (i < t1) ploc[i] = (valid && ent != VOX_NONE) ? (ent << 16) | (roff + (uint32_t)(lane - hl)) : VOX_NONE;
                __syncthreads();
              }
            }
            __syncthreads();
            if (tid == 0) { atomicMax(&dc->vox_max_tile, s_ent); if (s_dis) dc->vox_disorder = 1u; }
            if (s_over[0] | s_over[1]) { if (tid == 0) { dc->error = F3DS_ERR_UNSUPPORTED; dc->ev_overflow = 7; } return; }
            if (tid == 0) s_base = s_ent ? atomicAdd(&dc->seg_count, s_ent) : 0u;
            __syncthreads();
            const uint32_t dbase = s_base;
            if (tid == 0) s_ent = 0u;
            __syncthreads();
            for (uint32_t e0 = 0; e0 < VT_TAB; e0 += 256u) {
                const uint32_t e = e0 + tid;
                const unsigned long long pk = tkey[e];
                const bool live = pk != HASH_EMPTY;
                const uint64_t lm = __ballot(live);
                if (!lm) continue;
                uint32_t wb = 0;
                if (lane == __builtin_ctzll(lm)) wb = atomicAdd(&s_ent, (uint32_t)__popcll(lm));
                wb = __shfl(wb, __builtin_ctzll(lm), 64);
                if (live) {
                    const uint32_t d = dbase + wb + (uint32_t)__popcll(lm & lanemask_lt());
                    if (d < dcap) {
                        uint64_t code = n_morton((unsigned)(pk >> 42) & 0x1FFFFFu, (unsigned)(pk >> 21) & 0x1FFFFFu, (unsigned)pk & 0x1FFFFFu, g.depth);
                        if (fa.leaf_order == 1) code = (~code) & code_mask;
                        dkeys[d] = (((code << tile_bits) | (uint64_t)tile) << VT_CNT_BITS) | (uint64_t)tcnt[e];
                        dvals[d] = tile * VT_TAB + e;
                    } else { dc->error = F3DS_ERR_UNSUPPORTED; dc->ev_overflow = 7; }
                }
            }
            __syncthreads();
        }
    }
};
constexpr uint32_t DS_IT = 8;
constexpr uint32_t DS_CHUNK = 256u * DS_IT;
struct DescThread { uint64_t code[DS_IT]; uint32_t te[DS_IT], cnt[DS_IT]; uint32_t headmask, nheads, npts; };
__device__ inline void desc_load(const uint64_t* dkeys, const uint32_t* dvals, uint32_t D, int tile_bits, uint32_t db, DescThread& t, bool want_te) {
    const int sh = tile_bits + VT_CNT_BITS;
    uint64_t prev = (db > 0u && db - 1u < D) ? dkeys[db - 1u] >> sh : ~0ull;
#pragma unroll
    for (uint32_t k = 0; k < DS_IT; ++k) {
        const uint32_t d = db + k;
        const uint64_t key = d < D ? dkeys[d] : 0ull;
        t.code[k] = key >> sh; t.cnt[k] = d < D ? (uint32_t)key & ((1u << VT_CNT_BITS) - 1u) : 0u;
        t.te[k] = (want_te && d < D) ? dvals[d] : 0u;
    }
    t.headmask = 0u; t.nheads = 0u; t.npts = 0u;
#pragma unroll
    for (uint32_t k = 0; k < DS_IT; ++k) {
        const uint32_t d = db + k;
        const bool head = d < D && (d == 0u || prev != t.code[k]);
        prev = t.code[k];
        if (head) { t.headmask |= 1u << k; t.nheads++; }
        t.npts += t.cnt[k];
    }
}
__device__ inline void block_excl_scan2(uint32_t a, uint32_t b, uint32_t* ea, uint32_t* eb, uint32_t* ta, uint32_t* tb) {
    __shared__ uint32_t s_a[4], s_b[4];
    const uint32_t lane = (uint32_t)lane_id(), w = threadIdx.x >> 6;
    uint32_t ia = a, ib = b;
#pragma unroll
    for (int k = 1; k < 64; k <<= 1) { const uint32_t x = __shfl_up(ia, k, 64), y = __shfl_up(ib, k, 64); if ((int)lane >= k) { ia += x; ib += y; } }
    __syncthreads();
    if (lane == 63u) { s_a[w] = ia; s_b[w] = ib; }
    __syncthreads();
    uint32_t ba = 0, bb = 0, sa = 0, sb = 0;
#pragma unroll
    for (uint32_t k = 0; k < 4u; ++k) { if (k < w) { ba += s_a[k]; bb += s_b[k]; } sa += s_a[k]; sb += s_b[k]; }
    *ea = ba + ia - a; *eb = bb + ib - b; *ta = sa; *tb = sb;
}
struct d_desc_part {
    static constexpr int BLOCK = 256;
    __device__ void operator()(const uint64_t* dkeys, uint32_t dcap, int tile_bits, uint32_t* part, const DevCounters* dc) const {
        if (dc->ev_overflow) return;
        const uint32_t D = dc->seg_count < dcap ? dc->seg_count : dcap;
        const uint32_t nchunks = (dcap + DS_CHUNK - 1u) / DS_CHUNK;
        for (uint32_t b = BIX; b < nchunks; b += gridDim.x) {
            DescThread t;
            desc_load(dkeys, nullptr, D, tile_bits, b * DS_CHUNK + threadIdx.x * DS_IT, t, false);
            uint32_t eh, ec, th, tc;
            block_excl_scan2(t.nheads, t.npts, &eh, &ec, &th, &tc);
            if (threadIdx.x == 0) { part[2u * b] = th; part[2u * b + 1u] = tc; }
            __syncthreads();
        }
    }
};
struct d_desc_offsets {
    static constexpr bool LATENCY_KERNEL = true;
    static constexpr int BLOCK = 256;
    __device__ void operator()(uint32_t* part, uint32_t dcap, uint32_t capV, uint32_t* seg_start, DevCounters* dc) const {
        if (BIX || dc->ev_overflow) return;
        const uint32_t nchunks = (dcap + DS_CHUNK - 1u) / DS_CHUNK;
        uint32_t ch = 0, cc = 0;
        for (uint32_t b0 = 0; b0 < nchunks; b0 += 256u) {
            const uint32_t b = b0 + threadIdx.x;
            const uint32_t h = b < nchunks ? part[2u * b] : 0u, c = b < nchunks ? part[2u * b + 1u] : 0u;
            uint32_t eh, ec, th, tc;
            block_excl_scan2(h, c, &eh, &ec, &th, &tc);
            if (b < nchunks) { part[2u * b] = ch + eh; part[2u * b + 1u] = cc + ec; }
            ch += th; cc += tc;
            __syncthreads();
        }
        if (threadIdx.x == 0) {
            dc->n_voxels = ch; dc->n_valid = cc;
            if (ch <= capV) seg_start[ch] = cc; else { dc->error = F3DS_ERR_UNSUPPORTED; dc->ev_overflow = 7; }
        }
    }
};
struct d_desc_apply {
    static constexpr int BLOCK = 256;
    __device__ void operator()(const uint64_t* dkeys, const uint32_t* dvals, uint32_t dcap, uint32_t capV, int tile_bits, FrameArgs fa, const GridInfo* gp,
                               const uint32_t* part, uint2* bo_te, uint32_t* seg_start, uint32_t* vkey, const DevCounters* dc) const {
        if (dc->ev_overflow) return;
        const uint32_t D = dc->seg_count < dcap ? dc->seg_count : dcap;
        const int depth = gp->depth;
        const uint32_t nchunks = (D + DS_CHUNK - 1u) / DS_CHUNK;
        for (uint32_t b = BIX; b < nchunks; b += gridDim.x) {
            const uint32_t db = b * DS_CHUNK + threadIdx.x * DS_IT;
            DescThread t;
            desc_load(dkeys, dvals, D, tile_bits, db, t, true);
            uint32_t eh, ec, th, tc;
            block_excl_scan2(t.nheads, t.npts, &eh, &ec, &th, &tc);
            uint32_t ord = part[2u * b] + eh;
            uint32_t pos = part[2u * b + 1u] + ec;
        #pragma unroll
            for (uint32_t k = 0; k < DS_IT; ++k) {
                if (db + k >= D) break;
                if (t.headmask & (1u << k)) {
                    if (ord < capV) {
                        seg_start[ord] = pos;
                        uint64_t c2 = t.code[k];
                        if (fa.leaf_order == 1) c2 = (~c2) & ((1ull << (3 * depth)) - 1ull);
                        unsigned k3[3];
                        n_demorton(c2, depth, k3);
                        vkey[ord * 3] = k3[0]; vkey[ord * 3 + 1] = k3[1]; vkey[ord * 3 + 2] = k3[2];
                    }
                    ord++;
                }
                bo_te[t.te[k]] = make_uint2(pos, ord - 1u);
                pos += t.cnt[k];
            }
            __syncthreads();
        }
    }
};
struct d_tile_place {
    static constexpr int BLOCK = 256;
    __device__ void operator()(const uint32_t* ploc, uint32_t n, const uint2* bo_te, uint32_t* list, int* pt_voxel, const DevCounters* dc) const {
        __shared__ uint2 tab[VT_TAB];
        if (dc->ev_overflow) return;
        const uint32_t ntiles = (n + VT_TILE - 1u) / VT_TILE;
        for (uint32_t tile = BIX; tile < ntiles; tile += gridDim.x) {
            const uint32_t t0 = tile * VT_TILE, t1 = n - t0 < VT_TILE ? n : t0 + VT_TILE;
            constexpr uint32_t PF = 4;
            uint32_t pl[PF];
    #pragma unroll
            for (uint32_t j = 0; j < PF; ++j) { const uint32_t i = t0 + j * 256u + threadIdx.x; pl[j] = i < t1 ? ploc[i] : VOX_NONE; }
            __syncthreads();
            for (uint32_t e = threadIdx.x; e < VT_TAB; e += 256u) tab[e] = bo_te[(size_t)tile * VT_TAB + e];
            __syncthreads();
            for (uint32_t i0 = t0; i0 < t1; i0 += 256u * PF) {
                uint32_t nx[PF];
    #pragma unroll
                for (uint32_t j = 0; j < PF; ++j) { const uint32_t i = i0 + (PF + j) * 256u + threadIdx.x; nx[j] = i < t1 ? ploc[i] : VOX_NONE; }
    #pragma unroll
                for (uint32_t j = 0; j < PF; ++j) {
                    const uint32_t i = i0 + j * 256u + threadIdx.x;
                    if (i >= t1) continue;
                    if (pl[j] == VOX_NONE) { pt_voxel[i] = -1; continue; }
                    const uint2 bo = tab[pl[j] >> 16];
                    list[bo.x + (pl[j] & 0xFFFFu)] = i;
                    pt_voxel[i] = (int)bo.y;
                }
    #pragma unroll
                for (uint32_t j = 0; j < PF; ++j) pl[j] = nx[j];
            }
        }
    }
};
struct d_vox_table {
    static constexpr bool LATENCY_KERNEL = true;
    static constexpr int BLOCK = 1024;
    __device__ void operator()(const uint32_t* vkey, uint32_t V, const GridInfo* gp, uint64_t* hkeys, uint32_t* hvals, uint32_t hmask) const {
        const bool blocks = vt_blocks(gp->depth);
        const bool agent = gridDim.x > 1u;
        BtEntry* const tab = reinterpret_cast<BtEntry*>(hkeys);
        const uint32_t lane = (uint32_t)lane_id();
        constexpr uint32_t PF = 4;
        for (uint32_t s0 = BIX * (BLOCK * PF); s0 < V; s0 += gridDim.x * (BLOCK * PF)) {
            unsigned k[PF][3]; uint32_t prev[PF];
    #pragma unroll
            for (uint32_t j = 0; j < PF; ++j) { const uint32_t v = s0 + j * BLOCK + threadIdx.x, vv = v < V ? v : 0u; k[j][0] = vkey[vv * 3]; k[j][1] = vkey[vv * 3 + 1]; k[j][2] = vkey[vv * 3 + 2]; }
            if (!blocks) {
    #pragma unroll
                for (uint32_t j = 0; j < PF; ++j) { const uint32_t v = s0 + j * BLOCK + threadIdx.x; if (v < V) vt_insert(hkeys, hvals, hmask, agent, k[j][0], k[j][1], k[j][2], v); }
                continue;
            }
    #pragma unroll
            for (uint32_t j = 0; j < PF; ++j) {
                const uint32_t v = s0 + j * BLOCK + threadIdx.x;
                prev[j] = lane == 0u && v > 0u && v < V ? n_block_key(vkey[(v - 1u) * 3], vkey[(v - 1u) * 3 + 1], vkey[(v - 1u) * 3 + 2]) : BT_EMPTY;
            }
    #pragma unroll
            for (uint32_t j = 0; j < PF; ++j) {
                const uint32_t v = s0 + j * BLOCK + threadIdx.x;
                const bool in = v < V;
                const uint32_t bk = n_block_key(k[j][0], k[j][1], k[j][2]);
                const uint32_t up = __shfl_up(bk, 1, 64);
                const bool head = in && bk != (lane ? up : prev[j]);
                const uint64_t cuts = __ballot(head || !in);
                const uint64_t ahead = (cuts >> 1) >> lane;
                unsigned long long m = in ? 1ull << n_block_cell(k[j][0], k[j][1], k[j][2]) : 0ull;
    #pragma unroll
                for (uint32_t d = 1; d < 64u; d <<= 1) {
                    const unsigned long long o = __shfl_down(m, d, 64);
                    if (lane + d < 64u && !(ahead & ((1ull << d) - 1ull))) m |= o;
                }
                if (in && (head || lane == 0u)) {
                    BtEntry* const e = bt_entry(tab, hmask, agent, bk);
                    if (agent) __hip_atomic_fetch_and(&e->vacant, ~m, __ATOMIC_RELAXED, __HIP_MEMORY_SCOPE_AGENT);
                    else __hip_atomic_fetch_and(&e->vacant, ~m, __ATOMIC_RELAXED, __HIP_MEMORY_SCOPE_WORKGROUP);
                    if (head) e->base = v;
                }
            }
        }
    }
};
struct d_voxel_list_accum {
    static constexpr int BLOCK = 256;
    __device__ void operator()(const P16* pts, uint32_t* list, const uint32_t* seg_start, FrameArgs fa, float* vf, uint32_t* vcount, DevCounters* dc, uint32_t capV) const {
        __shared__ __attribute__((aligned(16))) uint4 buf[VG_CHUNK];
        if (dc->ev_overflow) return;
        const uint32_t V = dc->n_voxels < capV ? dc->n_voxels : capV;
        const bool disorder = dc->vox_disorder != 0u;
        const uint32_t tid = threadIdx.x;
        for (uint32_t vb = BIX * 256u; vb < V; vb += gridDim.x * 256u) {
            const uint32_t v = vb + tid;
            const bool mine = v < V;
            const uint32_t s = mine ? seg_start[v] : 0u, e = mine ? seg_start[v + 1] : 0u;
            const uint32_t p0 = seg_start[vb], p1 = seg_start[vb + 256u < V ? vb + 256u : V];
            if (__syncthreads_or(e - s > VL_MAX_RUN)) { if (tid == 0) { dc->error = F3DS_ERR_UNSUPPORTED; dc->ev_overflow = 6; } return; }
            if (disorder) {
                for (uint32_t a = s + 1u; a < e; ++a) {
                    const uint32_t x = list[a];
                    uint32_t b = a;
                    while (b > s && list[b - 1u] > x) { list[b] = list[b - 1u]; --b; }
                    if (b != a) list[b] = x;
                }
                __threadfence_block();
                __syncthreads();
            }
            float sx = 0, sy = 0, sz = 0, sr = 0, sg = 0, sb = 0;
            for (uint32_t c0 = p0; c0 < p1; c0 += VG_CHUNK) {
                const uint32_t c1 = p1 - c0 < VG_CHUNK ? p1 : c0 + VG_CHUNK;
                uint32_t idx[VG_CHUNK / 256];
        #pragma unroll
                for (uint32_t j = 0; j < VG_CHUNK / 256; ++j) { const uint32_t i = c0 + j * 256u + tid; idx[j] = list[i < c1 ? i : c1 - 1u]; }
                uint4 q[VG_CHUNK / 256];
        #pragma unroll
                for (uint32_t j = 0; j < VG_CHUNK / 256; ++j) q[j] = reinterpret_cast<const uint4*>(pts)[idx[j]];
        #pragma unroll
                for (uint32_t j = 0; j < VG_CHUNK / 256; ++j) buf[j * 256u + tid] = q[j];
                __syncthreads();
                const uint32_t a = s > c0 ? s : c0, b = e < c1 ? e : c1;
                for (uint32_t i = a; i < b; ++i) {
                    const uint4 w = buf[i - c0];
                    float z = __uint_as_float(w.z); n_prelude(z, fa.fold_negative_z);
                    sx += __uint_as_float(w.x); sy += __uint_as_float(w.y); sz += z;
                    sr += (float)((w.w >> 16) & 255u); sg += (float)((w.w >> 8) & 255u); sb += (float)(w.w & 255u);
                }
                __syncthreads();
            }
            if (!mine) continue;
            const float c = (float)(e - s);
            vcount[v] = e - s;
            float4* row = reinterpret_cast<float4*>(vf + (size_t)v * 12);
            row[0] = make_float4(sx / c, sy / c, sz / c, sr / c);
            row[1] = make_float4(sg / c, sb / c, 0.0f, 0.0f);
            row[2] = make_float4(0.0f, 0.0f, 0.0f, 0.0f);
        }
    }
};
__device__ inline int hash_find(const uint64_t* hkeys, const uint32_t* hvals, uint32_t hmask, uint64_t pk) {
    uint32_t h = (uint32_t)hash64(pk) & hmask;
    for (;;) {
        uint64_t k = hkeys[h];
        if (k == pk) return (int)hvals[h];
        if (k == HASH_EMPTY) return -1;
        h = (h + 1u) & hmask;
    }
}

struct d_neighbors {
    static constexpr int BLOCK = 256;
    __device__ void operator()(const uint32_t* vkey, const DevCounters* dc, const GridInfo* gp, int leaf_order, const uint64_t* hkeys,
                                                  const uint32_t* hvals, uint32_t hmask, int* nbr, int* nbrT) const {
        __shared__ int tr[27][65];
        const uint32_t V = dc->n_voxels;
        const unsigned max_key = gp->max_key;
        const bool blocks = vt_blocks(gp->depth);
        const BtEntry* const tab = reinterpret_cast<const BtEntry*>(hkeys);
        for (uint32_t vb = BIX * 64u; vb < V; vb += gridDim.x * 64u) {
            const uint32_t nv = V - vb < 64u ? V - vb : 64u, np = nv * 27u;
            for (uint32_t tl = threadIdx.x; tl < np; tl += 256u) {
                const uint32_t vl = tl / 27u, s = tl - vl * 27u, v = vb + vl;
                const int d[3] = {(int)(s / 9u) - 1, (int)((s / 3u) % 3u) - 1, (int)(s % 3u) - 1};
                bool ok = true; unsigned k[3];
                for (int a = 0; a < 3; ++a) {
                    long long q = (long long)vkey[v * 3 + a] + d[a];
                    if (q < 0 || q > (long long)max_key) ok = false;
                    k[a] = (unsigned)q;
                }
                const int u = !ok ? -1 : blocks ? bt_find(tab, hmask, leaf_order, k[0], k[1], k[2]) : vt_find(hkeys, hvals, hmask, k[0], k[1], k[2]);
                nbr[(size_t)vb * 27u + tl] = u;
                tr[s][vl] = u;
            }
            __syncthreads();
            for (uint32_t r = threadIdx.x; r < 27u * 64u; r += 256u) {
                const uint32_t s = r >> 6, vl = r & 63u;
                if (vl < nv) nbrT[(size_t)s * V + vb + vl] = tr[s][vl];
            }
            __syncthreads();
        }
    }
};
constexpr int NT_TILE = 128;
constexpr int NT_HCAP = 2048;
#ifndef F3DS_NT_SLOTS
#define F3DS_NT_SLOTS 896
#endif
#ifndef F3DS_NT_RING1
#define F3DS_NT_RING1 448
#endif
constexpr int NT_SLOTS = F3DS_NT_SLOTS;
constexpr int NT_RING1 = F3DS_NT_RING1;
constexpr uint16_t NT_NONE = 0xFFFFu;
constexpr uint32_t NT_HNONE = 0x3FFu;
constexpr uint32_t NT_ORD_LIMIT = (1u << 22) - 2u;
static_assert(NT_SLOTS < 1023, "slot numbers share a word with the ordinal");
constexpr uint16_t NT_ZERO = NT_SLOTS;
constexpr uint32_t SW_TILE_NONE = 0xFFFFFFFFu;
constexpr int SW_SLOT_BITS = 9;
constexpr int SW_SLOT_WORDS = (27 * SW_SLOT_BITS + 31) / 32;
static_assert(NT_RING1 < (1 << SW_SLOT_BITS), "a list position must fit its bit field");
__device__ __forceinline__ void sw_slots_pack(const uint32_t pos[27], uint32_t w[SW_SLOT_WORDS]) {
#pragma unroll
    for (int k = 0; k < SW_SLOT_WORDS; ++k) w[k] = 0u;
#pragma unroll
    for (int j = 0; j < 27; ++j) {
        const int bit = j * SW_SLOT_BITS, wi = bit >> 5, sh = bit & 31;
        w[wi] |= pos[j] << sh;
        if (sh + SW_SLOT_BITS > 32) w[wi + 1] |= pos[j] >> (32 - sh);
    }
}
__device__ __forceinline__ uint32_t sw_slot(const uint32_t w[SW_SLOT_WORDS], int j) {
    const int bit = j * SW_SLOT_BITS, wi = bit >> 5, sh = bit & 31;
    uint32_t x = w[wi] >> sh;
    if (sh + SW_SLOT_BITS > 32) x |= w[wi + 1] << (32 - sh);
    return x & ((1u << SW_SLOT_BITS) - 1u);
}
__device__ inline void cov_add(float acc[9], const float4 q) {
    acc[0] += q.x * q.x; acc[1] += q.x * q.y; acc[2] += q.x * q.z;
    acc[3] += q.y * q.y; acc[4] += q.y * q.z; acc[5] += q.z * q.z;
    acc[6] += q.x; acc[7] += q.y; acc[8] += q.z;
}
__device__ __forceinline__ uint32_t lds_addr(const float* p);
typedef float f3ds_f2 __attribute__((ext_vector_type(2)));
typedef float f3ds_f4 __attribute__((ext_vector_type(4)));
struct CovPairs {
    f3ds_f2 a0, a1, a2, a3; float sz;
    __device__ void zero() { a0 = a1 = a2 = a3 = f3ds_f2{0.0f, 0.0f}; sz = 0.0f; }
    __device__ void add(const f3ds_f4 q) {
        const f3ds_f2 xy = q.xy, zy = q.zw;
        a0 += xy * q.xx;
        a1 += xy * q.zz;
        a2 += zy * zy;
        a3 += xy;
        sz += q.z;
    }
    __device__ void store(float acc[9]) const { acc[0] = a0.x; acc[1] = a0.y; acc[2] = a1.x; acc[3] = a2.y; acc[4] = a1.y; acc[5] = a2.x; acc[6] = a3.x; acc[7] = a3.y; acc[8] = sz; }
};
template <int NTT>
struct d_normals_t {
    static constexpr int BLOCK = NTT;
    static constexpr int PT = (NT_RING1 * 27 + NTT - 1) / NTT;
    static constexpr int PR = PT % 9 == 0 ? 9 : (PT % 8 == 0 ? 8 : (PT % 6 == 0 ? 6 : (PT % 4 == 0 ? 4 : (PT % 3 == 0 ? 3 : (PT % 2 == 0 ? 2 : 1)))));
#ifndef F3DS_NORMALS_WPS
#define F3DS_NORMALS_WPS 3
#endif
#ifndef F3DS_NORMALS_WPS256
#define F3DS_NORMALS_WPS256 3
#endif
    static constexpr int WAVES_PER_SIMD = NTT > 256 ? F3DS_NORMALS_WPS : F3DS_NORMALS_WPS256;
    __device__ static uint32_t hslot(uint32_t ord) { return (ord * 2654435761u) >> 21; }
    __device__ void one_tile(const uint32_t bix, float* vf, const int* nbr, const DevCounters* dc, uint32_t* tile_n1, uint32_t* tile_ord, uint32_t* tile_slots, uint32_t holes) const {
        __shared__ uint32_t hw[NT_HCAP];
        __shared__ __attribute__((aligned(16))) float4 xyz[NT_SLOTS + 1];
        __shared__ uint32_t sord[NT_SLOTS];
        __shared__ uint16_t rows[NT_RING1 + 1][28];
        __shared__ uint32_t n_slots, overflow;
        __shared__ uint16_t tme[NT_TILE];
        const uint32_t KB = lds_addr(reinterpret_cast<const float*>(xyz)) >> 4;
        const uint32_t V = dc->n_voxels;
        const uint32_t v0 = bix * NT_TILE;
        if (v0 >= V) return;
        const uint32_t nt = V - v0 < (uint32_t)NT_TILE ? V - v0 : (uint32_t)NT_TILE;
#ifdef F3DS_MERGE_PROF
        unsigned long long tp[8], tq = __builtin_amdgcn_s_memtime(); int tpi = 0;
        unsigned long long tx_[12] = {0, 0, 0, 0, 0, 0, 0, 0, 0, 0, 0, 0}, tq2 = tq;
#define NPH() do { const unsigned long long n_ = __builtin_amdgcn_s_memtime(); tp[tpi++] = n_ - tq; tq = n_; } while (0)
#define NPX(i) do { const unsigned long long n_ = __builtin_amdgcn_s_memtime(); tx_[i] = n_ - tq2; tq2 = n_; } while (0)
#else
#define NPH() do { } while (0)
#define NPX(i) do { } while (0)
#endif
        for (int i = threadIdx.x; i < NT_HCAP; i += NTT) hw[i] = 0u;
        if (threadIdx.x == 0) { n_slots = 0; overflow = V >= NT_ORD_LIMIT ? 1u : 0u; xyz[NT_ZERO] = make_float4(0.0f, 0.0f, 0.0f, 0.0f); }
        __syncthreads();
        auto insert_key_from = [&](uint32_t ord, uint32_t h, uint32_t old) -> uint32_t {
            for (int probes = 0; probes < NT_HCAP; ++probes) {
                if (old == 0u) old = atomicCAS(&hw[h], 0u, ((ord + 1u) << 10) | NT_HNONE);
                if (old == 0u || (old >> 10) == ord + 1u) return h;
                h = (h + 1u) & (NT_HCAP - 1);
                old = hw[h];
            }
            overflow = 1;
            return 0u;
        };
        auto lookup = [&](uint32_t ord) -> uint16_t {
            uint32_t h = hslot(ord);
            for (;;) {
                const uint32_t k = hw[h];
                if ((k >> 10) == ord + 1u) return (k & NT_HNONE) == NT_HNONE ? NT_NONE : (uint16_t)(k & NT_HNONE);
                if (k == 0u) return NT_NONE;
                h = (h + 1u) & (NT_HCAP - 1);
            }
        };
        NPH();
        {
            constexpr int R1 = (NT_TILE * 27 + NTT - 1) / NTT;
            int u1[R1];
#pragma unroll
            for (int j = 0; j < R1; ++j) {
                const uint32_t t = threadIdx.x + (uint32_t)j * NTT;
                const uint32_t tt = t < nt * 27u ? t : 0u;
                u1[j] = nbr[(size_t)v0 * 27 + tt];
            }
            uint32_t h1[R1], o1[R1];
#pragma unroll
            for (int j = 0; j < R1; ++j) { h1[j] = hslot((uint32_t)u1[j]); o1[j] = hw[h1[j]]; }
            NPX(0);
#pragma unroll
            for (int j = 0; j < R1; ++j) {
                const uint32_t t = threadIdx.x + (uint32_t)j * NTT;
                if (t < nt * 27u && u1[j] >= 0 && (o1[j] >> 10) != (uint32_t)u1[j] + 1u) insert_key_from((uint32_t)u1[j], h1[j], o1[j]);
            }
        }
        NPX(1);
        __syncthreads();
        NPX(2);
        constexpr int NI = (NT_HCAP + NTT - 1) / NTT;
        {
            uint32_t key[NI]; uint64_t mask[NI]; uint32_t total = 0;
#pragma unroll
            for (int r = 0; r < NI; ++r) {
                const int i = r * NTT + (int)threadIdx.x;
                key[r] = i < NT_HCAP ? hw[i] : 0u;
                mask[r] = __ballot(key[r] != 0u);
                total += (uint32_t)__popcll(mask[r]);
            }
            uint32_t first = 0;
            if (lane_id() == 0 && total) first = atomicAdd(&n_slots, total);
            first = (uint32_t)__builtin_amdgcn_readfirstlane((int)first);
#pragma unroll
            for (int r = 0; r < NI; ++r) {
                const int i = r * NTT + (int)threadIdx.x;
                if (key[r]) { const uint32_t sl = first + (uint32_t)__popcll(mask[r] & lanemask_lt()); if (sl < NT_RING1) { hw[i] = (key[r] & ~NT_HNONE) | sl; sord[sl] = (key[r] >> 10) - 1u; } else overflow = 1; }
                first += (uint32_t)__popcll(mask[r]);
            }
        }
        NPX(3);
        __syncthreads();
        NPH();
        NPX(4);
        const uint32_t n1 = n_slots < NT_RING1 ? n_slots : NT_RING1;
        if (threadIdx.x < nt && !overflow) tme[threadIdx.x] = lookup(v0 + threadIdx.x);
        if (!overflow) {
            int u2c[PT];
            const uint32_t lim = n1 * 27u;
#pragma unroll
            for (int j = 0; j < PT; ++j) {
                u2c[j] = -1;
                if ((uint32_t)j * NTT < lim) {
                    const uint32_t t = threadIdx.x + (uint32_t)j * NTT;
                    const uint32_t tt = t < lim ? t : lim - 1u;
                    const uint32_t i = tt / 27u, sl = tt - i * 27u;
                    u2c[j] = nbr[(size_t)sord[i] * 27 + sl];
                }
            }
            constexpr int G = PR;
            { int any_ = 0;
#pragma unroll
              for (int j = 0; j < PT; ++j) any_ |= u2c[j];
              asm volatile("" :: "v"(any_)); }
            NPX(5);
#pragma unroll
            for (int j0 = 0; j0 < PT; j0 += G) {
                uint32_t h2[G], o2[G];
#pragma unroll
                for (int g = 0; g < G; ++g) {
                    const uint32_t t = threadIdx.x + (uint32_t)(j0 + g) * NTT;
                    if (t >= lim) u2c[j0 + g] = -1;
                    h2[g] = hslot((uint32_t)u2c[j0 + g]); o2[g] = hw[h2[g]];
                }
#pragma unroll
                for (int g = 0; g < G; ++g) {
                    uint32_t pos = 0xFFFFu;
                    if (u2c[j0 + g] >= 0) pos = (o2[g] >> 10) == (uint32_t)u2c[j0 + g] + 1u ? h2[g] : insert_key_from((uint32_t)u2c[j0 + g], h2[g], o2[g]);
                    const uint32_t t = threadIdx.x + (uint32_t)(j0 + g) * NTT;
                    if (t < lim) { const uint32_t i = t / 27u, sl = t - i * 27u; rows[i][sl] = (uint16_t)pos; }
                }
            }
        }
        NPX(6);
        __syncthreads();
        NPX(7);
        if (!overflow) {
            uint32_t key[NI]; uint64_t mask[NI]; uint32_t total = 0;
#pragma unroll
            for (int r = 0; r < NI; ++r) {
                const int i = r * NTT + (int)threadIdx.x;
                const uint32_t kw = i < NT_HCAP ? hw[i] : 0u;
                key[r] = (kw & NT_HNONE) == NT_HNONE ? kw : 0u;
                mask[r] = __ballot(key[r] != 0u);
                total += (uint32_t)__popcll(mask[r]);
            }
            uint32_t first = 0;
            if (lane_id() == 0 && total) first = atomicAdd(&n_slots, total);
            first = (uint32_t)__builtin_amdgcn_readfirstlane((int)first);
#pragma unroll
            for (int r = 0; r < NI; ++r) {
                const int i = r * NTT + (int)threadIdx.x;
                if (key[r]) { const uint32_t sl = first + (uint32_t)__popcll(mask[r] & lanemask_lt()); if (sl < NT_SLOTS) { hw[i] = (key[r] & ~NT_HNONE) | sl; sord[sl] = (key[r] >> 10) - 1u; } else overflow = 1; }
                first += (uint32_t)__popcll(mask[r]);
            }
        }
        NPX(8);
        __syncthreads();
        NPH();
        NPX(9);
        if (overflow) {
            if (threadIdx.x == 0) tile_n1[bix] = SW_TILE_NONE;
            const uint32_t v = v0 + threadIdx.x;
            if (threadIdx.x < nt) {
                float acc[9] = {0, 0, 0, 0, 0, 0, 0, 0, 0};
                unsigned cnt = 1;
                const float4 self = *reinterpret_cast<const float4*>(vf + (size_t)v * 12);
                cov_add(acc, self);
                for (int s = 0; s < 27; ++s) {
                    const int u = nbr[(size_t)v * 27 + s];
                    if (u < 0) continue;
                    cov_add(acc, *reinterpret_cast<const float4*>(vf + (size_t)u * 12)); cnt++;
                    for (int s2 = 0; s2 < 27; ++s2) {
                        const int u2 = nbr[(size_t)u * 27 + s2];
                        if (u2 >= 0) { cov_add(acc, *reinterpret_cast<const float4*>(vf + (size_t)u2 * 12)); cnt++; }
                    }
                }
                const float vp[3] = {self.x, self.y, self.z};
                float n4[4];
                n_plane_normal(acc, cnt, vp, n4);
                float* nout = vf + (size_t)v * 12 + 6;
                nout[0] = n4[0]; nout[1] = n4[1]; nout[2] = n4[2];
            }
            return;
// ... 2811 lines not shown
```

Baseline: 3703.

## Fuse tile placement into key kernel and sort voxel descriptor keys only

The per-point placement pass moves into the tile-key kernel. Each tile now writes compact 16-bit tile-local point lists built in LDS, in place of a global per-point slot array and a separate placement kernel. The descriptor sort packs the tile list offset into the key so the radix sort moves keys only with no value arrays. The voxel accumulation kernel then finds each point through a binary search over descriptor positions and writes pt_voxel itself. The aim is to cut global traffic and one launch, at the cost of extra LDS work, key bits and search logic.

New measurement: 3695. No clear change (-0.2%).

```diff
diff --git a/fast-3d-pointcloud-segmentation_amd/csrc/f3ds_hip.hip b/fast-3d-pointcloud-segmentation_amd/csrc/f3ds_hip.hip
--- a/fast-3d-pointcloud-segmentation_amd/csrc/f3ds_hip.hip
+++ b/fast-3d-pointcloud-segmentation_amd/csrc/f3ds_hip.hip
@@ -133,7 +133,7 @@
      X(float, r_vf) X(uint32_t, r_owner) X(float, r_dist) X(float, r_hc) X(uint32_t, r_hcount) X(uint32_t, r_hlo) X(uint32_t, r_hhi) X(int, r_gvox) X(unsigned char, r_gact) X(unsigned char, r_gdone) X(uint32_t, r_ghead) X(uint32_t, r_gnext) X(uint32_t, r_tl) X(uint32_t, r_tcnt) X(int, r_seed) X(uint32_t, r_L) \
     X(uint32_t, tstamp) X(uint32_t, tround) X(uint32_t, hdirty) X(uint32_t, htiles) X(uint32_t, htcnt) X(uint32_t, vwl) X(uint32_t, vwl2) X(uint32_t, vtmask) \
      X(uint32_t, glut) X(uint32_t, truth_pts) X(uint32_t, tsum) X(uint32_t, tcol) X(uint32_t, tlab) X(uint32_t, ctab) X(uint32_t, csize) X(uint32_t, eroot) X(uint32_t, eincl) \
-     X(uint32_t, hcnt) X(uint32_t, pslot) X(uint32_t, vlist) \
+     X(uint32_t, hcnt) X(uint32_t, tlist) X(uint32_t, dfirst) X(uint2, dpos) \
      X(uint32_t, u_src) X(uint32_t, u_voff) X(float, u_xyz) X(uint32_t, u_rgba) X(float, u_cent) X(float, u_nrm) \
     X(float, deltas) X(uint64_t, skeys0) X(uint64_t, skeys1) X(uint32_t, svals0) X(uint32_t, svals1) X(uint32_t, cdf_hist) X(float, cdf) X(uint32_t, root) X(uint32_t, rincl) X(uint32_t, rrank) X(uint2, pool) X(uint32_t, rstart) X(uint32_t, rnleaf) X(uint32_t, rcap) X(uint32_t, tile_n1) X(uint32_t, tile_ord) X(uint32_t, tile_slots) X(uint32_t, ilist) X(uint32_t, istart) X(uint32_t, ilen) X(uint32_t, icap) \
      X(uint32_t, lv_into) X(uint32_t, lv_at) X(uint32_t, lv_pfx) X(float, lv_thr) X(uint32_t, lv_tab) X(uint32_t, lv_nreg) X(uint32_t, lv_out) \
@@ -201,6 +201,7 @@
     uint32_t pool_mult = 1;
     uint32_t vox_cap = 0;
     bool vox_hashed = false;
+    bool vox_keys_only = false;
     bool vox_dense = false;
     uint32_t vox_dense_wait = 0, vox_dense_penalty = 8;
     uint32_t ilist_mult = 1;
@@ -472,6 +473,7 @@
         rec<d_radix_hist>(c, nb, 0u, k0, n, base_shift + shift, bits, hist, nb, n_dev);
         rec<d_scan_single>(c, 1u, 0u, hist, (uint32_t)((1u << bits) * nb));
         if (v0) rec<d_radix_scatter>(c, nb, 0u, k0, v0, k1, v1, n, base_shift + shift, bits, hist, nb, n_dev);
+        else if (n_dev) rec<d_radix_scatter_kn>(c, nb, 0u, k0, k1, n, base_shift + shift, bits, hist, nb, n_dev);
         else rec<d_radix_scatter_k>(c, nb, 0u, k0, k1, n, base_shift + shift, bits, hist, nb);
         std::swap(k0, k1); std::swap(v0, v1);
         shift += bits;
@@ -522,23 +524,25 @@
     const uint64_t fin = c->h_dc->n_finite;
     const uint32_t capV = (uint32_t)std::max<uint64_t>(256u, std::min<uint64_t>(fin, dcap));
     c->vox_cap = capV;
-    uint64_t *k0, *k1; uint32_t *ploc, *v0, *v1, *part, *vkey, *vcount, *seg_start, *list; uint2* bo_te; float* vf; int* pt_voxel;
+    const int toff_bits = (F3DS_VT_KEYS_ONLY && code_bits + tile_bits + VT_OFF_BITS + VT_CNT_BITS <= 64) ? VT_OFF_BITS : 0;
+    c->vox_keys_only = toff_bits != 0;
+    uint64_t *k0, *k1; uint32_t *tlist, *v0 = nullptr, *v1 = nullptr, *part, *vkey, *vcount, *seg_start, *dfirst; uint2* dd; float* vf; int* pt_voxel;
     const uint32_t nchunks = (dcap + DS_CHUNK - 1u) / DS_CHUNK;
-    ENSURE(c->pslot, n, ploc); ENSURE(c->keys0, dcap, k0); ENSURE(c->keys1, dcap, k1); ENSURE(c->vals0, dcap, v0); ENSURE(c->vals1, dcap, v1);
-    { uint32_t* w; ENSURE(c->hcnt, (size_t)ntiles * VT_TAB * 2 + 2u * nchunks, w); bo_te = reinterpret_cast<uint2*>(w); part = w + (size_t)ntiles * VT_TAB * 2; }
+    ENSURE(c->tlist, (size_t)ntiles * (VT_TILE / 2u), tlist); ENSURE(c->keys0, dcap, k0); ENSURE(c->keys1, dcap, k1);
+    if (!toff_bits) { ENSURE(c->vals0, dcap, v0); ENSURE(c->vals1, dcap, v1); }
+    ENSURE(c->hcnt, 2u * nchunks, part);
     ENSURE(c->vkey, (size_t)capV * 3, vkey); ENSURE(c->vcount, capV, vcount); ENSURE(c->vf, (size_t)capV * 12, vf);
-    ENSURE(c->seg_start, (size_t)capV + 1, seg_start); ENSURE(c->vlist, n, list); ENSURE(c->pt_voxel, n, pt_voxel);
+    ENSURE(c->seg_start, (size_t)capV + 1, seg_start); ENSURE(c->dfirst, (size_t)capV + 1, dfirst); ENSURE(c->dpos, (size_t)dcap + 1, dd); ENSURE(c->pt_voxel, n, pt_voxel);
     { uint32_t *f, *incl; ENSURE(c->flags, capV, f); ENSURE(c->incl, capV, incl); }
     c->idxbits = -1; c->ks = nullptr; c->vs = nullptr;
-    rec<d_tile_keys>(c, std::min<uint32_t>(ntiles, (uint32_t)g_grid_cap * 16u), 0u, c->d_pts, n, c->fa, c->d_grid, ploc, k0, v0, dcap, tile_bits, c->d_dc);
+    rec<d_tile_keys>(c, std::min<uint32_t>(ntiles, (uint32_t)g_grid_cap * 16u), 0u, c->d_pts, n, c->fa, c->d_grid, tlist, k0, v0, dcap, tile_bits, toff_bits, pt_voxel, c->d_dc);
     uint64_t* ks; uint32_t* vs;
-    int rc = radix_sort(c, k0, v0, k1, v1, dcap, code_bits + tile_bits, &ks, &vs, VT_CNT_BITS, &c->d_dc->seg_count);
+    int rc = radix_sort(c, k0, v0, k1, v1, dcap, code_bits + tile_bits, &ks, &vs, toff_bits + VT_CNT_BITS, &c->d_dc->seg_count);
     if (rc) return rc;
-    rec<d_desc_part>(c, nchunks, 0u, ks, dcap, tile_bits, part, c->d_dc);
-    rec<d_desc_offsets>(c, 1u, 0u, part, dcap, capV, seg_start, c->d_dc);
-    rec<d_desc_apply>(c, nchunks, 0u, ks, vs, dcap, capV, tile_bits, c->fa, c->d_grid, part, bo_te, seg_start, vkey, c->d_dc);
-    rec<d_tile_place>(c, std::min<uint32_t>(ntiles, (uint32_t)g_grid_cap * 16u), 0u, ploc, n, bo_te, list, pt_voxel, c->d_dc);
-    rec<d_voxel_list_accum>(c, std::min<uint32_t>(grid_wide(capV, 256), std::max<uint32_t>(64u, grid_wide(n / 8u, 256))), 0u, c->d_pts, list, seg_start, c->fa, vf, vcount, c->d_dc, capV);
+    rec<d_desc_part>(c, nchunks, 0u, ks, dcap, tile_bits, toff_bits, part, c->d_dc);
+    rec<d_desc_offsets>(c, 1u, 0u, part, dcap, capV, seg_start, dfirst, dd, c->d_dc);
+    rec<d_desc_apply>(c, nchunks, 0u, ks, vs, dcap, capV, tile_bits, toff_bits, c->fa, c->d_grid, part, dd, dfirst, seg_start, vkey, c->d_dc);
+    rec<d_voxel_list_accum>(c, std::min<uint32_t>(grid_wide(capV, 256), std::max<uint32_t>(64u, grid_wide(n / 8u, 256))), 0u, c->d_pts, n, reinterpret_cast<const uint16_t*>(tlist), dd, dfirst, seg_start, c->fa, vf, vcount, pt_voxel, c->d_dc, capV);
     c->vox_hashed = true;
     return F3DS_OK;
 }
@@ -1224,7 +1228,7 @@
             for (f3ds_ctx* c : b.fr) { reset_recording(c); c->vox_hashed = false; }
             hashed = false;
         } else if (rc || (rc = flush_sync(b))) return rc;
-        if (hashed && g_sw.trace_err) for (f3ds_ctx* c : b.fr) fprintf(stderr, "f3ds: tile path: most voxels in a tile %u, descriptors %u, leaves %u, lists sorted %u\n", c->h_dc->vox_max_tile, c->h_dc->seg_count, c->h_dc->n_voxels, c->h_dc->vox_disorder);
+        if (hashed && g_sw.trace_err) for (f3ds_ctx* c : b.fr) fprintf(stderr, "f3ds: tile path: most voxels in a tile %u, descriptors %u, leaves %u, lists sorted %u\nf3ds: tile path: the descriptor sort moved %s\n", c->h_dc->vox_max_tile, c->h_dc->seg_count, c->h_dc->n_voxels, c->h_dc->vox_disorder, c->vox_keys_only ? "keys only" : "(key, offset) pairs");
         if (hashed) for (f3ds_ctx* c : b.fr) if (c->h_dc->ev_overflow == 6 || c->h_dc->ev_overflow == 7) {
             if (g_sw.trace_err) fprintf(stderr, "f3ds: tile path refused a frame: %s (descriptors %u, leaves %u)\n", c->h_dc->ev_overflow == 6 ? "a voxel with too many points" : "a tile with too many voxels", c->h_dc->seg_count, c->h_dc->n_voxels);
             c->vox_dense = true; c->vox_dense_wait = c->vox_dense_penalty; c->vox_dense_penalty = std::min(2u * c->vox_dense_penalty, 1024u); hashed = false;
diff --git a/fast-3d-pointcloud-segmentation_amd/csrc/f3ds_kernels.inc b/fast-3d-pointcloud-segmentation_amd/csrc/f3ds_kernels.inc
--- a/fast-3d-pointcloud-segmentation_amd/csrc/f3ds_kernels.inc
+++ b/fast-3d-pointcloud-segmentation_amd/csrc/f3ds_kernels.inc
@@ -289,6 +289,13 @@
         }
     }
 };
+struct d_radix_scatter_kn {
+    static constexpr int BLOCK = RS_THREADS;
+    __device__ void operator()(const uint64_t* keys, uint64_t* keys_out, uint32_t n, int shift, int bits, const uint32_t* hist_scanned, uint32_t nblocks, const uint32_t* n_dev) const {
+        const uint32_t nd = *n_dev;
+        d_radix_scatter_k{}(keys, keys_out, nd < n ? nd : n, shift, bits, hist_scanned, nblocks);
+    }
+};
 
 struct FrameArgs {
     int use_transform, fold_negative_z, leaf_order;
@@ -652,6 +659,12 @@
 constexpr uint32_t VT_TAB = VT_TILE / 2;
 constexpr int VT_CNT_BITS = 14;
 static_assert(VT_TILE < (1u << VT_CNT_BITS), "a tile's point count must fit the count field");
+constexpr int VT_OFF_BITS = 12;
+static_assert(VT_TILE <= (1u << VT_OFF_BITS), "an entry's list offset must fit the offset field");
+#ifndef F3DS_VT_KEYS_ONLY
+#define F3DS_VT_KEYS_ONLY 1
+#endif
+static_assert(VT_TILE <= 65536, "the tile-local lists hold 16-bit indices");
 constexpr uint32_t VT_ENT_MAX = VT_TAB * 5 / 8;
 constexpr uint32_t VL_MAX_RUN = 256;
 constexpr uint32_t VOX_NONE = 0xFFFFFFFFu;
@@ -667,13 +680,45 @@
     const uint64_t stop = (hm | ~vm) & above;
     *head = h; *head_lane = hl; *run_len = (uint32_t)((stop ? __builtin_ctzll(stop) : 64) - hl);
 }
+struct d_tile_place {
+    __device__ void operator()(const uint32_t (&pl)[VT_TILE / 256u], const uint32_t* tab, uint16_t* lst, const uint32_t* dirty, uint32_t total, uint32_t t0, uint32_t t1,
+                               uint32_t* tlist, int* pt_voxel) const {
+        const uint32_t tid = threadIdx.x;
+    #pragma unroll
+        for (uint32_t s = 0; s < VT_TILE / 256u; ++s) {
+            const uint32_t li = s * 256u + tid;
+            if (li >= t1 - t0) continue;
+            if (pl[s] == VOX_NONE) { pt_voxel[t0 + li] = -1; continue; }
+            lst[(tab[pl[s] >> 16] >> 16) + (pl[s] & 0xFFFFu)] = (uint16_t)li;
+        }
+        __syncthreads();
+        if (dirty) {
+            for (uint32_t e = tid; e < VT_TAB; e += 256u) {
+                if (!((dirty[e >> 5] >> (e & 31u)) & 1u)) continue;
+                const uint32_t w = tab[e], cnt = w & 0xFFFFu;
+                uint16_t* const r = lst + (w >> 16);
+                for (uint32_t a = 1u; a < cnt; ++a) {
+                    const uint16_t x = r[a];
+                    uint32_t b = a;
+                    while (b > 0u && r[b - 1u] > x) { r[b] = r[b - 1u]; --b; }
+                    if (b != a) r[b] = x;
+                }
+            }
+            __syncthreads();
+        }
+        const uint32_t* const w32 = reinterpret_cast<const uint32_t*>(lst);
+        for (uint32_t w = tid; w < (total + 1u) / 2u; w += 256u) tlist[t0 / 2u + w] = w32[w];
+    }
+};
 struct d_tile_keys {
     static constexpr int BLOCK = 256;
-    __device__ void operator()(const P16* pts, uint32_t n, FrameArgs fa, const GridInfo* gp, uint32_t* ploc, uint64_t* dkeys, uint32_t* dvals,
-                               uint32_t dcap, int tile_bits, DevCounters* dc) const {
-        __shared__ unsigned long long tkey[VT_TAB];
-        __shared__ uint32_t tcnt[VT_TAB];
+    static constexpr int WAVES_PER_SIMD = 4;
+    __device__ void operator()(const P16* pts, uint32_t n, FrameArgs fa, const GridInfo* gp, uint32_t* tlist, uint64_t* dkeys, uint32_t* dvals,
+                               uint32_t dcap, int tile_bits, int toff_bits, int* pt_voxel, DevCounters* dc) const {
+        __shared__ __attribute__((aligned(16))) unsigned long long tkey[VT_TAB];
+        __shared__ __attribute__((aligned(16))) uint32_t tcnt[VT_TAB];
         __shared__ uint32_t tbits[2][VT_TAB / 32];
+        __shared__ uint32_t tdis[VT_TAB / 32];
         __shared__ uint32_t s_ent, s_base, s_over[2], s_dis;
         const GridInfo g = *gp;
         const uint64_t code_mask = (1ull << (3 * g.depth)) - 1ull;
@@ -682,14 +727,21 @@
         const uint32_t ntiles = (n + VT_TILE - 1u) / VT_TILE;
         for (uint32_t tile = BIX; tile < ntiles; tile += gridDim.x) {
             for (uint32_t e = tid; e < VT_TAB; e += 256u) { tkey[e] = HASH_EMPTY; tcnt[e] = 0u; }
-            if (tid < VT_TAB / 32u) { tbits[0][tid] = 0u; tbits[1][tid] = 0u; }
+            if (tid < VT_TAB / 32u) { tbits[0][tid] = 0u; tbits[1][tid] = 0u; tdis[tid] = 0u; }
             if (tid == 0) { s_ent = 0u; s_over[0] = 0u; s_over[1] = 0u; s_dis = 0u; }
             __syncthreads();
             const uint32_t t0 = tile * VT_TILE, t1 = n - t0 < VT_TILE ? n : t0 + VT_TILE;
             constexpr uint32_t VT_PF = 4;
+            uint32_t pl[VT_TILE / 256u];
+        #pragma unroll
+            for (uint32_t s = 0; s < VT_TILE / 256u; ++s) pl[s] = VOX_NONE;
             uint32_t it4 = 0u;
+        #pragma nounroll
             for (uint32_t base4 = t0; base4 < t1 && !s_over[(it4 + 1u) & 1u]; base4 += 256u * VT_PF, ++it4) {
               uint4 q[VT_PF];
+              uint32_t pw[VT_PF];
+        #pragma unroll
+              for (uint32_t j = 0; j < VT_PF; ++j) pw[j] = VOX_NONE;
         #pragma unroll
               for (uint32_t j = 0; j < VT_PF; ++j) { const uint32_t i = base4 + j * 256u + tid; q[j] = reinterpret_cast<const uint4*>(pts)[i < t1 ? i : t1 - 1u]; }
         #pragma unroll
@@ -719,18 +771,38 @@
                     if (ent != VOX_NONE) {
                         roff = atomicAdd(&tcnt[ent], len);
                         const uint32_t bit = 1u << (ent & 31u);
-                        if (atomicOr(&tbits[step & 1u][ent >> 5], bit) & bit) s_dis = 1u;
+                        if (atomicOr(&tbits[step & 1u][ent >> 5], bit) & bit) { s_dis = 1u; atomicOr(&tdis[ent >> 5], bit); }
                     } else s_over[it4 & 1u] = 1u;
                 }
                 if (tid < VT_TAB / 32u) tbits[(step + 1u) & 1u][tid] = 0u;
                 ent = __shfl(ent, hl, 64); roff = __shfl(roff, hl, 64);
-                if (i < t1) ploc[i] = (valid && ent != VOX_NONE) ? (ent << 16) | (roff + (uint32_t)(lane - hl)) : VOX_NONE;
+                if (valid && ent != VOX_NONE) pw[j] = (ent << 16) | (roff + (uint32_t)(lane - hl));
                 __syncthreads();
+              }
+        #pragma unroll
+              for (uint32_t k = 0; k < VT_TILE / (256u * VT_PF); ++k) {
+                if (it4 != k) continue;
+        #pragma unroll
+                for (uint32_t j = 0; j < VT_PF; ++j) pl[k * VT_PF + j] = pw[j];
               }
             }
             __syncthreads();
             if (tid == 0) { atomicMax(&dc->vox_max_tile, s_ent); if (s_dis) dc->vox_disorder = 1u; }
             if (s_over[0] | s_over[1]) { if (tid == 0) { dc->error = F3DS_ERR_UNSUPPORTED; dc->ev_overflow = 7; } return; }
+            uint32_t total;
+            {
+                uint32_t cn[8];
+                const uint4 c0 = reinterpret_cast<const uint4*>(tcnt)[tid * 2u], c1 = reinterpret_cast<const uint4*>(tcnt)[tid * 2u + 1u];
+                cn[0] = c0.x; cn[1] = c0.y; cn[2] = c0.z; cn[3] = c0.w; cn[4] = c1.x; cn[5] = c1.y; cn[6] = c1.z; cn[7] = c1.w;
+                uint32_t sum = 0;
+        #pragma unroll
+                for (uint32_t k = 0; k < 8u; ++k) sum += cn[k];
+                uint32_t run = block_incl_scan<256>(sum, &total) - sum;
+        #pragma unroll
+                for (uint32_t k = 0; k < 8u; ++k) { const uint32_t c = cn[k]; cn[k] = c | (run << 16); run += c; }
+                reinterpret_cast<uint4*>(tcnt)[tid * 2u] = make_uint4(cn[0], cn[1], cn[2], cn[3]);
+                reinterpret_cast<uint4*>(tcnt)[tid * 2u + 1u] = make_uint4(cn[4], cn[5], cn[6], cn[7]);
+            }
             if (tid == 0) s_base = s_ent ? atomicAdd(&dc->seg_count, s_ent) : 0u;
             __syncthreads();
             const uint32_t dbase = s_base;
@@ -750,27 +822,36 @@
                     if (d < dcap) {
                         uint64_t code = n_morton((unsigned)(pk >> 42) & 0x1FFFFFu, (unsigned)(pk >> 21) & 0x1FFFFFu, (unsigned)pk & 0x1FFFFFu, g.depth);
                         if (fa.leaf_order == 1) code = (~code) & code_mask;
-                        dkeys[d] = (((code << tile_bits) | (uint64_t)tile) << VT_CNT_BITS) | (uint64_t)tcnt[e];
-                        dvals[d] = tile * VT_TAB + e;
+                        const uint32_t w = tcnt[e], off = w >> 16;
+                        const uint64_t ct = (code << tile_bits) | (uint64_t)tile;
+                        dkeys[d] = (((toff_bits ? (ct << toff_bits) | (uint64_t)off : ct)) << VT_CNT_BITS) | (uint64_t)(w & 0xFFFFu);
+                        if (!toff_bits) dvals[d] = off;
                     } else { dc->error = F3DS_ERR_UNSUPPORTED; dc->ev_overflow = 7; }
                 }
             }
+            __syncthreads();
+            d_tile_place{}(pl, tcnt, reinterpret_cast<uint16_t*>(tkey), s_dis ? tdis : nullptr, total, t0, t1, tlist, pt_voxel);
             __syncthreads();
         }
     }
 };
 constexpr uint32_t DS_IT = 8;
 constexpr uint32_t DS_CHUNK = 256u * DS_IT;
-struct DescThread { uint64_t code[DS_IT]; uint32_t te[DS_IT], cnt[DS_IT]; uint32_t headmask, nheads, npts; };
-__device__ inline void desc_load(const uint64_t* dkeys, const uint32_t* dvals, uint32_t D, int tile_bits, uint32_t db, DescThread& t, bool want_te) {
-    const int sh = tile_bits + VT_CNT_BITS;
+struct DescThread { uint64_t code[DS_IT]; uint32_t src[DS_IT], cnt[DS_IT]; uint32_t headmask, nheads, npts; };
+__device__ inline void desc_load(const uint64_t* dkeys, const uint32_t* dvals, uint32_t D, int tile_bits, int toff_bits, uint32_t db, DescThread& t, bool want_src) {
+    const int sh = tile_bits + toff_bits + VT_CNT_BITS;
     uint64_t prev = (db > 0u && db - 1u < D) ? dkeys[db - 1u] >> sh : ~0ull;
 #pragma unroll
     for (uint32_t k = 0; k < DS_IT; ++k) {
         const uint32_t d = db + k;
         const uint64_t key = d < D ? dkeys[d] : 0ull;
         t.code[k] = key >> sh; t.cnt[k] = d < D ? (uint32_t)key & ((1u << VT_CNT_BITS) - 1u) : 0u;
-        t.te[k] = (want_te && d < D) ? dvals[d] : 0u;
+        t.src[k] = 0u;
+        if (want_src && d < D) {
+            const uint32_t tile = (uint32_t)(key >> (toff_bits + VT_CNT_BITS)) & ((1u << tile_bits) - 1u);
+            const uint32_t off = toff_bits ? (uint32_t)(key >> VT_CNT_BITS) & ((1u << VT_OFF_BITS) - 1u) : dvals[d];
+            t.src[k] = tile * VT_TILE + off;
+        }
     }
     t.headmask = 0u; t.nheads = 0u; t.npts = 0u;
 #pragma unroll
@@ -798,13 +879,13 @@
 }
 struct d_desc_part {
     static constexpr int BLOCK = 256;
-    __device__ void operator()(const uint64_t* dkeys, uint32_t dcap, int tile_bits, uint32_t* part, const DevCounters* dc) const {
+    __device__ void operator()(const uint64_t* dkeys, uint32_t dcap, int tile_bits, int toff_bits, uint32_t* part, const DevCounters* dc) const {
         if (dc->ev_overflow) return;
         const uint32_t D = dc->seg_count < dcap ? dc->seg_count : dcap;
         const uint32_t nchunks = (dcap + DS_CHUNK - 1u) / DS_CHUNK;
         for (uint32_t b = BIX; b < nchunks; b += gridDim.x) {
             DescThread t;
-            desc_load(dkeys, nullptr, D, tile_bits, b * DS_CHUNK + threadIdx.x * DS_IT, t, false);
+            desc_load(dkeys, nullptr, D, tile_bits, toff_bits, b * DS_CHUNK + threadIdx.x * DS_IT, t, false);
             uint32_t eh, ec, th, tc;
             block_excl_scan2(t.nheads, t.npts, &eh, &ec, &th, &tc);
             if (threadIdx.x == 0) { part[2u * b] = th; part[2u * b + 1u] = tc; }
@@ -815,7 +896,7 @@
 struct d_desc_offsets {
     static constexpr bool LATENCY_KERNEL = true;
     static constexpr int BLOCK = 256;
-    __device__ void operator()(uint32_t* part, uint32_t dcap, uint32_t capV, uint32_t* seg_start, DevCounters* dc) const {
+    __device__ void operator()(uint32_t* part, uint32_t dcap, uint32_t capV, uint32_t* seg_start, uint32_t* dfirst, uint2* dd, DevCounters* dc) const {
         if (BIX || dc->ev_overflow) return;
         const uint32_t nchunks = (dcap + DS_CHUNK - 1u) / DS_CHUNK;
         uint32_t ch = 0, cc = 0;
@@ -830,14 +911,16 @@
         }
         if (threadIdx.x == 0) {
             dc->n_voxels = ch; dc->n_valid = cc;
-            if (ch <= capV) seg_start[ch] = cc; else { dc->error = F3DS_ERR_UNSUPPORTED; dc->ev_overflow = 7; }
+            const uint32_t D = dc->seg_count < dcap ? dc->seg_count : dcap;
+            if (ch <= capV) { seg_start[ch] = cc; dfirst[ch] = D; dd[D] = make_uint2(cc, 0u); }
+            else { dc->error = F3DS_ERR_UNSUPPORTED; dc->ev_overflow = 7; }
         }
     }
 };
 struct d_desc_apply {
     static constexpr int BLOCK = 256;
-    __device__ void operator()(const uint64_t* dkeys, const uint32_t* dvals, uint32_t dcap, uint32_t capV, int tile_bits, FrameArgs fa, const GridInfo* gp,
-                               const uint32_t* part, uint2* bo_te, uint32_t* seg_start, uint32_t* vkey, const DevCounters* dc) const {
+    __device__ void operator()(const uint64_t* dkeys, const uint32_t* dvals, uint32_t dcap, uint32_t capV, int tile_bits, int toff_bits, FrameArgs fa, const GridInfo* gp,
+                               const uint32_t* part, uint2* dd, uint32_t* dfirst, uint32_t* seg_start, uint32_t* vkey, const DevCounters* dc) const {
         if (dc->ev_overflow) return;
         const uint32_t D = dc->seg_count < dcap ? dc->seg_count : dcap;
         const int depth = gp->depth;
@@ -845,7 +928,7 @@
         for (uint32_t b = BIX; b < nchunks; b += gridDim.x) {
             const uint32_t db = b * DS_CHUNK + threadIdx.x * DS_IT;
             DescThread t;
-            desc_load(dkeys, dvals, D, tile_bits, db, t, true);
+            desc_load(dkeys, dvals, D, tile_bits, toff_bits, db, t, true);
             uint32_t eh, ec, th, tc;
             block_excl_scan2(t.nheads, t.npts, &eh, &ec, &th, &tc);
             uint32_t ord = part[2u * b] + eh;
@@ -856,6 +939,7 @@
                 if (t.headmask & (1u << k)) {
                     if (ord < capV) {
                         seg_start[ord] = pos;
+                        dfirst[ord] = db + k;
                         uint64_t c2 = t.code[k];
                         if (fa.leaf_order == 1) c2 = (~c2) & ((1ull << (3 * depth)) - 1ull);
                         unsigned k3[3];
@@ -864,44 +948,10 @@
                     }
                     ord++;
                 }
-                bo_te[t.te[k]] = make_uint2(pos, ord - 1u);
+                dd[db + k] = make_uint2(pos, t.src[k]);
                 pos += t.cnt[k];
             }
             __syncthreads();
-        }
-    }
-};
-struct d_tile_place {
-    static constexpr int BLOCK = 256;
-    __device__ void operator()(const uint32_t* ploc, uint32_t n, const uint2* bo_te, uint32_t* list, int* pt_voxel, const DevCounters* dc) const {
-        __shared__ uint2 tab[VT_TAB];
-        if (dc->ev_overflow) return;
-        const uint32_t ntiles = (n + VT_TILE - 1u) / VT_TILE;
-        for (uint32_t tile = BIX; tile < ntiles; tile += gridDim.x) {
-            const uint32_t t0 = tile * VT_TILE, t1 = n - t0 < VT_TILE ? n : t0 + VT_TILE;
-            constexpr uint32_t PF = 4;
-            uint32_t pl[PF];
-    #pragma unroll
-            for (uint32_t j = 0; j < PF; ++j) { const uint32_t i = t0 + j * 256u + threadIdx.x; pl[j] = i < t1 ? ploc[i] : VOX_NONE; }
-            __syncthreads();
-            for (uint32_t e = threadIdx.x; e < VT_TAB; e += 256u) tab[e] = bo_te[(size_t)tile * VT_TAB + e];
-            __syncthreads();
-            for (uint32_t i0 = t0; i0 < t1; i0 += 256u * PF) {
-                uint32_t nx[PF];
-    #pragma unroll
-                for (uint32_t j = 0; j < PF; ++j) { const uint32_t i = i0 + (PF + j) * 256u + threadIdx.x; nx[j] = i < t1 ? ploc[i] : VOX_NONE; }
-    #pragma unroll
-                for (uint32_t j = 0; j < PF; ++j) {
-                    const uint32_t i = i0 + j * 256u + threadIdx.x;
-                    if (i >= t1) continue;
-                    if (pl[j] == VOX_NONE) { pt_voxel[i] = -1; continue; }
-                    const uint2 bo = tab[pl[j] >> 16];
-                    list[bo.x + (pl[j] & 0xFFFFu)] = i;
-                    pt_voxel[i] = (int)bo.y;
-                }
-    #pragma unroll
-                for (uint32_t j = 0; j < PF; ++j) pl[j] = nx[j];
-            }
         }
     }
 };
@@ -955,34 +1005,48 @@
 };
 struct d_voxel_list_accum {
     static constexpr int BLOCK = 256;
-    __device__ void operator()(const P16* pts, uint32_t* list, const uint32_t* seg_start, FrameArgs fa, float* vf, uint32_t* vcount, DevCounters* dc, uint32_t capV) const {
+    __device__ void operator()(const P16* pts, uint32_t n, const uint16_t* tlist, const uint2* dd, const uint32_t* dfirst, const uint32_t* seg_start, FrameArgs fa,
+                               float* vf, uint32_t* vcount, int* pt_voxel, DevCounters* dc, uint32_t capV) const {
         __shared__ __attribute__((aligned(16))) uint4 buf[VG_CHUNK];
+        __shared__ uint32_t sd[VG_CHUNK + 1], ssrc[VG_CHUNK];
+        uint32_t* const vbuf = ssrc;
         if (dc->ev_overflow) return;
         const uint32_t V = dc->n_voxels < capV ? dc->n_voxels : capV;
-        const bool disorder = dc->vox_disorder != 0u;
         const uint32_t tid = threadIdx.x;
+        const uint32_t ntl = ((n + VT_TILE - 1u) / VT_TILE) * VT_TILE;
         for (uint32_t vb = BIX * 256u; vb < V; vb += gridDim.x * 256u) {
             const uint32_t v = vb + tid;
             const bool mine = v < V;
+            const uint32_t vend = vb + 256u < V ? vb + 256u : V;
             const uint32_t s = mine ? seg_start[v] : 0u, e = mine ? seg_start[v + 1] : 0u;
-            const uint32_t p0 = seg_start[vb], p1 = seg_start[vb + 256u < V ? vb + 256u : V];
+            const uint32_t p0 = seg_start[vb], p1 = seg_start[vend];
             if (__syncthreads_or(e - s > VL_MAX_RUN)) { if (tid == 0) { dc->error = F3DS_ERR_UNSUPPORTED; dc->ev_overflow = 6; } return; }
-            if (disorder) {
-                for (uint32_t a = s + 1u; a < e; ++a) {
-                    const uint32_t x = list[a];
-                    uint32_t b = a;
-                    while (b > s && list[b - 1u] > x) { list[b] = list[b - 1u]; --b; }
-                    if (b != a) list[b] = x;
-                }
-                __threadfence_block();
+            uint32_t dcur = dfirst[vb];
+            const uint32_t d1 = dfirst[vend];
+            float sx = 0, sy = 0, sz = 0, sr = 0, sg = 0, sb = 0;
+            for (uint32_t c0 = p0; c0 < p1 && dcur < d1; c0 += VG_CHUNK) {
+                const uint32_t c1 = p1 - c0 < VG_CHUNK ? p1 : c0 + VG_CHUNK;
+                const uint32_t ndl = d1 - dcur < VG_CHUNK ? d1 - dcur : VG_CHUNK;
+                for (uint32_t t = tid; t <= ndl; t += 256u) { const uint2 x = dd[dcur + t]; sd[t] = x.x; if (t < VG_CHUNK) ssrc[t] = x.y; }
                 __syncthreads();
-            }
-            float sx = 0, sy = 0, sz = 0, sr = 0, sg = 0, sb = 0;
-            for (uint32_t c0 = p0; c0 < p1; c0 += VG_CHUNK) {
-                const uint32_t c1 = p1 - c0 < VG_CHUNK ? p1 : c0 + VG_CHUNK;
-                uint32_t idx[VG_CHUNK / 256];
+                const uint32_t top = 1u << (31 - __builtin_clz(ndl));
+                uint32_t idx[VG_CHUNK / 256], tp[VG_CHUNK / 256];
         #pragma unroll
-                for (uint32_t j = 0; j < VG_CHUNK / 256; ++j) { const uint32_t i = c0 + j * 256u + tid; idx[j] = list[i < c1 ? i : c1 - 1u]; }
+                for (uint32_t j = 0; j < VG_CHUNK / 256; ++j) {
+                    const uint32_t i = c0 + j * 256u + tid, ii = i < c1 ? i : c1 - 1u;
+                    uint32_t lo = 0u;
+                    for (uint32_t st = top; st; st >>= 1) if (lo + st < ndl && sd[lo + st] <= ii) lo += st;
+                    const uint32_t src = ssrc[lo];
+                    tp[j] = src + (ii - sd[lo]);
+                    idx[j] = src & ~(VT_TILE - 1u);
+                }
+                uint32_t nx = 0u;
+                for (uint32_t st = top; st; st >>= 1) if (nx + st <= ndl && sd[nx + st] <= c1) nx += st;
+                uint32_t li[VG_CHUNK / 256];
+        #pragma unroll
+                for (uint32_t j = 0; j < VG_CHUNK / 256; ++j) li[j] = tlist[tp[j] < ntl ? tp[j] : ntl - 1u];
+        #pragma unroll
+                for (uint32_t j = 0; j < VG_CHUNK / 256; ++j) { idx[j] += li[j]; if (idx[j] >= n) idx[j] = n - 1u; }
                 uint4 q[VG_CHUNK / 256];
         #pragma unroll
                 for (uint32_t j = 0; j < VG_CHUNK / 256; ++j) q[j] = reinterpret_cast<const uint4*>(pts)[idx[j]];
@@ -995,8 +1059,13 @@
                     float z = __uint_as_float(w.z); n_prelude(z, fa.fold_negative_z);
                     sx += __uint_as_float(w.x); sy += __uint_as_float(w.y); sz += z;
                     sr += (float)((w.w >> 16) & 255u); sg += (float)((w.w >> 8) & 255u); sb += (float)(w.w & 255u);
+                    vbuf[i - c0] = v;
                 }
                 __syncthreads();
+        #pragma unroll
+                for (uint32_t j = 0; j < VG_CHUNK / 256; ++j) { const uint32_t pp = j * 256u + tid; if (c0 + pp < c1) pt_voxel[idx[j]] = (int)vbuf[pp]; }
+                __syncthreads();
+                dcur += nx;
             }
             if (!mine) continue;
             const float c = (float)(e - s);
```
